# victorca25/traiNNer

Hardware: AMD Instinct MI355X
Metric: HR images/sec (G+D step), ESRGAN x4 128->512 (higher is better)
Workload: dtype f32 (bf16x3)

## Files before the change

### include/trainner_hip.h

```cpp
#ifndef TRAINNER_HIP_H
#define TRAINNER_HIP_H

#include <stdint.h>

#ifdef __cplusplus
extern "C" {
#endif

#define TNR_OK 0
#define TNR_EINVAL (-1)
#define TNR_ELAUNCH (-2)

enum { TNR_ACT_NONE = 0, TNR_ACT_LRELU = 1, TNR_ACT_RELU = 2 };

enum {
    TNR_CONV_3x3 = 0,
    TNR_CONV_3x3_UP2 = 1,
    TNR_CONV_4x4_S2 = 2,
    TNR_DGRAD_4x4_S2 = 3,
    TNR_CONV_1x1 = 4,
    TNR_CONV_3x3_C4 = 5,
    TNR_CONV_7x7_C4 = 6
};

// ... 36 lines not shown
    tnr_view m;  int32_t m_lo, m_hi; float m_slope;
    float *ws; int64_t ws_bytes;
    int32_t mma;
    int32_t pad_mode;
    float noise_sigma; int32_t noise_pos; uint32_t noise_key0, noise_key1, noise_pix0;
    const void *wq; int64_t wq_bytes;
    int32_t wq_form;
    int32_t shuffle;
} tnr_conv_desc;

typedef struct tnr_wgrad_desc {
    tnr_view x; int32_t N, H, W; int32_t Cin;
    tnr_view g; int32_t Ho, Wo; int32_t Cout;
    int32_t mode;
    float *dw; int32_t cin_total, cin_begin;
    float *db;
    float alpha, beta;
    float *ws; int64_t ws_bytes;
    int32_t mma;
    int32_t pad_mode;
    float *dw2; int32_t cout_split, cin_total2;
    float *db2;
} tnr_wgrad_desc;

typedef struct tnr_pack_item {
    const float *w;
    float *wp;
    int32_t Cout, Cin, kh, kw;
    int32_t kind;
    int32_t KoutP, KinP;
    int64_t n_out;
} tnr_pack_item;

typedef struct tnr_dense_pack_item {
    const float *w[5];
    float *wp;
    int32_t nf, gc;
    int32_t t;
    int32_t KoutP, KinP;
    float scale5;
    int64_t n_out;
} tnr_dense_pack_item;

const char *tnr_last_error(void);
#define TNR_ABI_VERSION 3
int tnr_version(void);

int tnr_pack_dims(int32_t Cout, int32_t Cin, int32_t kh, int32_t kw, int32_t kind,
                  int32_t *KoutP, int32_t *KinP, int64_t *n_out);
int tnr_pack_weights(const tnr_pack_item *items_dev, int32_t n, int64_t max_out, void *stream);
int tnr_pack_dense_dims(int32_t nf, int32_t gc, int32_t t, int32_t *KoutP, int32_t *KinP, int64_t *n_out);
int tnr_pack_dense_dgrad(const tnr_dense_pack_item *items_dev, int32_t n, int64_t max_out, void *stream);
int tnr_conv_forward(const tnr_conv_desc *d, void *stream);
int tnr_gauss_mult(tnr_view dst, tnr_view src, int64_t pixels, int32_t C, float sigma, uint32_t key0, uint32_t key1, uint32_t pix0,
                   void *stream);
int64_t tnr_conv_workspace_bytes(const tnr_conv_desc *d);
int64_t tnr_conv_wq_bytes(const tnr_conv_desc *d);
int tnr_conv_wq_pack(const tnr_conv_desc *d, void *image, int64_t image_bytes, void *stream);
int64_t tnr_conv_wino_bytes(const tnr_conv_desc *d);
int tnr_conv_wino_pack(const tnr_conv_desc *d, void *image, int64_t image_bytes, void *stream);
int tnr_im2col(tnr_view x, int32_t N, int32_t H, int32_t W, int32_t C, int32_t k, int32_t stride, int32_t pad,
               int32_t Ho, int32_t Wo, float *out, void *stream);
#define TNR_CHAIN_MAX 6
int64_t tnr_conv_chain_workspace_bytes(const tnr_conv_desc *stage0);
int tnr_conv_chain(const tnr_conv_desc *stages, const int32_t *fresh_from, int32_t n, uint32_t *ws, int64_t ws_bytes,
                   uint32_t epoch, void *stream);
int64_t tnr_conv_sweep_image_bytes(const tnr_conv_desc *stages, int32_t n);
int tnr_conv_sweep_pack(const tnr_conv_desc *stages, int32_t n, void *image, int64_t image_bytes, void *stream);
typedef struct tnr_sweep_pack_item { int32_t units; int32_t reserved; uint64_t opaque[15]; } tnr_sweep_pack_item;
int tnr_conv_sweep_pack_item(const tnr_conv_desc *stages, int32_t n, void *image, int64_t image_bytes, tnr_sweep_pack_item *item);
int tnr_conv_sweep_pack_batch(const tnr_sweep_pack_item *items_dev, int32_t n, int32_t max_units, void *stream);
int tnr_conv_sweep(const tnr_conv_desc *stages, int32_t n, const void *image, uint32_t *ws, int64_t ws_bytes, uint32_t epoch,
                   void *stream);
int64_t tnr_conv_thin_pack_floats(int32_t reduce_channels);
int tnr_conv_thin_pack(const float *w_oihw, float *wp, int32_t Cout, int32_t Cin, int32_t dgrad, void *stream);
int tnr_conv_thin(tnr_view x, int32_t N, int32_t H, int32_t W, int32_t Cin, const float *wp, tnr_view y, int32_t Cout,
                  const float *bias, float alpha, void *stream);
int64_t tnr_conv_thin7_pack_floats(int32_t reduce_channels);
int tnr_conv_thin7_pack(const float *w_oihw, float *wp, int32_t Cout, int32_t Cin, int32_t dgrad, void *stream);
int tnr_conv_thin7(tnr_view x, int32_t N, int32_t H, int32_t W, int32_t Cin, const float *wp, tnr_view y, int32_t Ho, int32_t Wo,
                   int32_t Cout, int32_t pad, int32_t reflect, const float *bias, float alpha, void *stream);
int64_t tnr_wgrad_workspace_bytes(const tnr_wgrad_desc *d);
int64_t tnr_wgrad_thin_workspace_bytes(int32_t N, int32_t H, int32_t Cbig);
int tnr_wgrad_thin(tnr_view big, tnr_view small, int32_t N, int32_t H, int32_t W, int32_t Cbig, int32_t Csmall, int32_t flip,
                   float *dw, float *db, float alpha, float beta, float *ws, int64_t ws_bytes, void *stream);
int64_t tnr_wgrad_thin7_workspace_bytes(int32_t N, int32_t Hbig_grid, int32_t Cbig);
int tnr_wgrad_thin7(tnr_view big, int32_t N, int32_t H, int32_t W, int32_t rpad, tnr_view small, int32_t Hs, int32_t Ws, int32_t off,
                    int32_t Cbig, int32_t Csmall, int32_t flip, float *dw, float *db, float alpha, float beta, float *ws, int64_t ws_bytes,
                    void *stream);
int tnr_conv_wgrad(const tnr_wgrad_desc *d, void *stream);
#define TNR_WGRAD_GROUP_MAX 12
int tnr_conv_wgrad_group(const tnr_wgrad_desc *descs, int32_t n, void *stream);
int tnr_wgrad_tile_class(const tnr_wgrad_desc *d, int32_t group_jobs, int32_t x3_occ, int32_t out[12]);

int tnr_gconv_fwd(tnr_view x, int32_t N, int32_t H, int32_t W, int32_t Cin, const float *w, const float *bias, tnr_view y, int32_t Ho,
                  int32_t Wo, int32_t Cout, int32_t k, int32_t stride, int32_t pad, int32_t reflect, int32_t act, float slope, void *stream);
int tnr_gconv_dgrad(tnr_view g, int32_t N, int32_t H, int32_t W, int32_t Cin, const float *w, tnr_view gx, int32_t Ho, int32_t Wo,
                    int32_t Cout, int32_t k, int32_t stride, int32_t pad, int32_t reflect, void *stream);
int64_t tnr_gconv_wgrad_workspace_bytes(int32_t Cout, int32_t Cin, int32_t k);
int tnr_gconv_wgrad(tnr_view x, int32_t N, int32_t H, int32_t W, int32_t Cin, tnr_view g, int32_t Ho, int32_t Wo, int32_t Cout, int32_t k,
                    int32_t stride, int32_t pad, int32_t reflect, float *dw, float *db, float alpha, float beta, double *ws,
                    int64_t ws_bytes, void *stream);
int tnr_bias_grad(tnr_view g, int64_t pixels, int32_t C, float *db, float alpha, float beta, double *ws, int64_t ws_bytes, void *stream);
int tnr_pad2d(tnr_view x, tnr_view y, int32_t N, int32_t H, int32_t W, int32_t C, int32_t pad, int32_t mode, void *stream);
int tnr_unpad2d(tnr_view xp, tnr_view y, int32_t N, int32_t H, int32_t W, int32_t C, int32_t pad, int32_t mode, void *stream);
int tnr_window2d(tnr_view src, int32_t Hs, int32_t Ws, tnr_view dst, int32_t N, int32_t Hd, int32_t Wd, int32_t C, int32_t oy,
// ... 19 lines not shown
                          float *dst, int32_t bgr2rgb, float data_range, int32_t normalize, void *stream);
int tnr_tensor2np_u8(const float *src, int32_t N, int32_t C, int32_t H, int32_t W, uint8_t *dst, int32_t rgb2bgr,
                     int32_t denormalize, void *stream);
int64_t tnr_metrics_workspace_bytes(int32_t N);
int tnr_psnr_ssim_u8(const uint8_t *a, const uint8_t *b, int32_t N, int32_t H, int32_t W, int32_t C, int32_t crop,
                     int32_t want_ssim, double *out, double *ws, int64_t ws_bytes, void *stream);
int tnr_lpips_stem_dims(int32_t H, int32_t W, int32_t crop, int32_t *Ho, int32_t *Wo);
int tnr_lpips_stem(const void *a, const void *b, int32_t src_kind, int32_t N, int32_t H, int32_t W, int32_t C, int32_t crop,
                   int32_t normalize, const float *shift, const float *scale, const float *w, const float *bias, tnr_view y,
                   void *stream);
int tnr_maxpool3s2_ceil_dims(int32_t H, int32_t W, int32_t *Ho, int32_t *Wo);
int tnr_maxpool3s2_ceil_fwd(tnr_view x, tnr_view y, int32_t N, int32_t H, int32_t W, int32_t C, void *stream);
int64_t tnr_lpips_workspace_bytes(int32_t N, int32_t L);
int tnr_lpips_head(tnr_view f0, tnr_view f1, int32_t N, int32_t H, int32_t W, int32_t C, const float *w, int32_t layer, int32_t L,
                   double *ws, int64_t ws_bytes, void *stream);
int tnr_lpips_finalize(int32_t N, int32_t L, const double *ws, int64_t ws_bytes, double *out, double *per_layer, void *stream);
int tnr_bilinear2x_fwd(tnr_view x, tnr_view y, int32_t N, int32_t H, int32_t W, int32_t C, void *stream);
int tnr_bilinear2x_bwd(tnr_view gy, tnr_view gx, tnr_view gz, tnr_view mask, float mslope, int32_t N, int32_t H, int32_t W,
                       int32_t C, void *stream);
int tnr_add2(tnr_view dst, tnr_view a, tnr_view b, int64_t pixels, int32_t C, void *stream);
int tnr_mask_copy(tnr_view dst, tnr_view src, tnr_view y, int64_t pixels, int32_t C, float mslope, void *stream);
int tnr_nchw_to_nhwc(const float *src, int32_t N, int32_t C, int32_t H, int32_t W, tnr_view dst,
                     int32_t Cpad, const float *scale, const float *shift, void *stream);
int tnr_nhwc_to_nchw(tnr_view src, int32_t N, int32_t C, int32_t H, int32_t W, float *dst,
                     const float *scale, int32_t accumulate, void *stream);
int tnr_upsample2x_bwd(tnr_view gup, tnr_view gx, int32_t N, int32_t H, int32_t W, int32_t C,
                       tnr_view mask, float mslope, void *stream);
int tnr_depth_to_space(tnr_view x, tnr_view y, int32_t N, int32_t H, int32_t W, int32_t Cout, void *stream);
int tnr_space_to_depth_bwd(tnr_view gy, tnr_view gx, int32_t N, int32_t H, int32_t W, int32_t Cout,
                           tnr_view mask, float mslope, void *stream);
int tnr_maxpool2_fwd(tnr_view x, tnr_view y, int32_t N, int32_t H, int32_t W, int32_t C, void *stream);
int tnr_maxpool2_bwd(tnr_view gy, tnr_view x, tnr_view gx, int32_t N, int32_t H, int32_t W, int32_t C,
                     void *stream);
int tnr_axpby(tnr_view dst, tnr_view src, int64_t pixels, int32_t C, float a, float b, void *stream);
int tnr_mask_mul(tnr_view g, tnr_view y, int64_t pixels, int32_t C, float mslope, void *stream);
int tnr_fill(float *p, int64_t n, float v, void *stream);

int64_t tnr_bn_workspace_bytes(int32_t C);
int tnr_bn_train_fwd(tnr_view z, tnr_view y, int64_t pixels, int32_t C, const float *gamma,
                     const float *beta, float *running_mean, float *running_var, int64_t *num_batches,
                     float momentum, float eps, float *save_mean, float *save_invstd, int32_t act,
                     float slope, void *ws, void *stream);
int tnr_bn_train_fwd_stats(tnr_view z, tnr_view y, int64_t pixels, int32_t C, const float *gamma, const float *beta,
                           float *running_mean, float *running_var, int64_t *num_batches, float momentum, float eps,
                           float *save_mean, float *save_invstd, double *stat64, int32_t act, float slope, void *ws, void *stream);
int tnr_bn_replay_running(float *running_mean, float *running_var, int64_t *num_batches, const double *stat64, int32_t C,
                          float momentum, void *stream);
int tnr_bn_train_bwd(tnr_view gy, tnr_view y, tnr_view z, tnr_view gz, int64_t pixels, int32_t C,
                     const float *gamma, const float *save_mean, const float *save_invstd, float mslope,
                     float *dgamma, float *dbeta, float acc_beta, void *ws, void *stream);
int tnr_bn_train_bwd_z(tnr_view gy, tnr_view z, tnr_view gz, int64_t pixels, int32_t C, const float *gamma, const float *beta,
                       const float *save_mean, const float *save_invstd, float mslope, float *dgamma, float *dbeta,
                       float acc_beta, void *ws, void *stream);
int64_t tnr_instnorm_workspace_bytes(int32_t N, int32_t C);
int tnr_instnorm_fwd(tnr_view z, tnr_view y, int32_t N, int64_t pixels_per_image, int32_t C, float eps, float *save_mean,
                     float *save_invstd, int32_t act, float slope, void *ws, void *stream);
int tnr_instnorm_bwd(tnr_view gy, tnr_view y, tnr_view z, tnr_view gz, int32_t N, int64_t pixels_per_image, int32_t C,
                     const float *save_mean, const float *save_invstd, float mslope, void *ws, void *stream);

int tnr_linear_fwd(const float *x, const float *w, const float *b, float *y, int32_t N, int32_t In,
                   int32_t Out, int32_t act, float slope, void *stream);
int tnr_linear_bwd(const float *x, const float *w, const float *gy, const float *yact, float mslope,
                   float *gx, float *dw, float *db, int32_t N, int32_t In, int32_t Out, float acc_beta,
                   float *gpre_ws, void *stream);

int64_t tnr_reduce_workspace_bytes(void);
int tnr_l1_mean_fwd(const float *a, const float *b, int64_t n, float scale, float *loss, void *ws,
                    void *stream);
int tnr_l1_mean_bwd(const float *a, const float *b, int64_t n, float scale, const float *gscale,
                    float *ga, int32_t accumulate, void *stream);
int tnr_ragan_phase_a(const float *pf, const float *pr, int32_t n, float *sums, void *ws, void *stream);
int tnr_ragan_phase_b(const float *pf, const float *pr, int32_t n, int32_t stage, float *sums, void *ws, void *stream);
int tnr_ragan_phase_c(const float *pf, const float *pr, int32_t n, int32_t stage, float weight,
                      const float *sums, float *loss_out, float *gf, float *gr, void *stream);
int tnr_scale_by(float *dst, const float *src, int64_t n, const float *gscale, void *stream);

int64_t tnr_ssim_workspace_bytes(int32_t N, int32_t C, int32_t H, int32_t W, int32_t shave, int32_t K);
int tnr_ssim_fwd(const float *x, const float *y, int32_t N, int32_t C, int32_t H, int32_t W, int32_t layout, int32_t shave,
                 const float *taps, int32_t K, float C1, float C2, double *sums, void *ws, int64_t ws_bytes, void *stream);
int tnr_ssim_bwd(const float *x, const float *y, int32_t N, int32_t C, int32_t H, int32_t W, int32_t layout, int32_t shave,
                 const float *taps, int32_t K, float C1, float C2, const float *coef, const float *gscale, float *gx,
                 int32_t accumulate, void *stream);
int tnr_avgpool2_pad_dims(int32_t H, int32_t W, int32_t shave, int32_t *Ho, int32_t *Wo);
int tnr_avgpool2_pad_fwd(const float *x, const float *y, int32_t N, int32_t C, int32_t H, int32_t W, int32_t layout, int32_t shave,
                         float *xo, float *yo, void *stream);
int tnr_avgpool2_pad_bwd(const float *gcoarse, float *gfine, int32_t N, int32_t C, int32_t H, int32_t W, int32_t layout,
                         int32_t shave, void *stream);
int tnr_msssim_combine(const double *sums, int32_t levels, int32_t N, const int64_t *counts, const float *weights, int32_t mode,
                       float *value, float *coef, void *stream);

enum { TNR_CRIT_L1 = 0, TNR_CRIT_L2 = 1, TNR_CRIT_CB = 2, TNR_CRIT_ELASTIC = 3, TNR_CRIT_CLIPL1 = 4 };
int64_t tnr_imgloss_workspace_bytes(int32_t N, int32_t C, int32_t H, int32_t W);
int tnr_filter_loss_fwd(const float *x, const float *y, int32_t N, int32_t C, int32_t H, int32_t W, int32_t layout, const float *taps,
                        int32_t K, int32_t crit, double scale, float *loss, float *dmap, void *ws, int64_t ws_bytes, void *stream);
int tnr_filter_loss_bwd(const float *dmap, int32_t N, int32_t C, int32_t H, int32_t W, int32_t layout, const float *taps, int32_t K,
                        double scale, const float *gscale, float *gx, int32_t accumulate, void *stream);
int tnr_fd_loss_fwd(const float *x, const float *y, int32_t N, int32_t C, int32_t H, int32_t W, int32_t layout, int32_t dirs,
                    int32_t crit, double scale, float *loss, void *ws, int64_t ws_bytes, void *stream);
int tnr_fd_loss_bwd(const float *x, const float *y, int32_t N, int32_t C, int32_t H, int32_t W, int32_t layout, int32_t dirs,
                    int32_t crit, double scale, const float *gscale, float *gx, int32_t accumulate, void *stream);
int tnr_pointwise_loss_fwd(const float *a, const float *b, int64_t n, int32_t crit, double scale, float *loss, void *ws, void *stream);
int tnr_pointwise_loss_bwd(const float *a, const float *b, int64_t n, int32_t crit, double scale, const float *gscale, float *ga,
                           int32_t accumulate, void *stream);

int tnr_overflow_loss_fwd(const float *x, int64_t n, double scale, float *loss, void *ws, void *stream);
int tnr_overflow_loss_bwd(const float *x, int64_t n, double scale, const float *gscale, float *gx, int32_t accumulate, void *stream);
// ... 63 lines not shown
```

### trainner_amd/csrc/conv_epilogue.h

```cpp
#pragma once
#include "conv_body.h"

namespace {

template <int MODE, int TW, int NT, int MT, bool COH, int DEPTH = 1, bool NOISE = true, int BIAS_STEP = 1, class PixFn>
__device__ __forceinline__ void conv_epilogue_dpp_map(const ConvK a, f32x16 (&acc)[MT][NT], const int cb, const int n, const int ty0,
                                                      const int tx0, const int par, const int li, const int half,
                                                      const __amdgpu_buffer_rsrc_t y_rs, PixFn &&pixfn) {
    constexpr bool DG2 = (MODE == TNR_DGRAD_4x4_S2);
    constexpr int NC = NT * 32;
    const int py = par >> 1, px = par & 1;
    TNR_STAMP(2);
#ifdef TNR_PRIO_EPI
    __builtin_amdgcn_s_setprio(TNR_PRIO_EPI);
#endif
    const int qa = li >> 2, qb = li & 3;
    const bool b0 = (qb & 1) != 0, b1 = (qb & 2) != 0;
    auto quad_transpose = [&](float &v0, float &v1, float &v2, float &v3) {
        auto xchg = [&](float &x, float &y, bool sel, int which) {
            const float send = sel ? x : y;
            const int r_ = which == 1 ? __builtin_amdgcn_mov_dpp(__builtin_bit_cast(int, send), 0xB1, 0xF, 0xF, true)
                                      : __builtin_amdgcn_mov_dpp(__builtin_bit_cast(int, send), 0x4E, 0xF, 0xF, true);
            const float recv = __builtin_bit_cast(float, r_);
            x = sel ? recv : x;
            y = sel ? y : recv;
        };
        xchg(v0, v1, b0, 1);
        xchg(v2, v3, b0, 1);
        xchg(v0, v2, b1, 2);
        xchg(v1, v3, b1, 2);
    };
    TNR_STAMP(5);
    TNR_STAMP(6);
    TNR_STAMP(7);
#ifdef TNR_ABL_NOMASK
    const bool has_r1 = a.r1 != nullptr, has_r2 = a.r2 != nullptr, has_m = false;
#else
    const bool has_r1 = a.r1 != nullptr, has_r2 = a.r2 != nullptr, has_m = a.m != nullptr;
#endif
    const bool has_noise = NOISE && a.noise_pos != 0;
    const bool all_full = (a.Cout & 3) == 0;
    const float ns = a.act == TNR_ACT_LRELU ? a.slope : (a.act == TNR_ACT_RELU ? 0.f : 1.f);
    int co_n[NT];
    bool co_ok[NT];
    f32x4 bv[NT];
    float b1f[NT], msf[NT];
    bool use_r1[NT], use_m[NT];
#pragma unroll
    for (int nn = 0; nn < NT; ++nn) {
        const int co = cb * NC + nn * 32 + qa * 4;
        co_n[nn] = co;
        co_ok[nn] = co < a.Cout;
        bv[nn] = f32x4{0.f, 0.f, 0.f, 0.f};
        if (a.bias != nullptr && co_ok[nn]) {
            if constexpr (BIAS_STEP != 1) {
#pragma unroll
                for (int k = 0; k < 4; ++k)
                    if (co + k < a.Cout) bv[nn][k] = a.bias[(co + k) * BIAS_STEP];
            } else if (co + 4 <= a.Cout) {
                bv[nn] = *reinterpret_cast<const f32x4 *>(a.bias + co);
            } else {
#pragma unroll
                for (int k = 0; k < 4; ++k)
                    if (co + k < a.Cout) bv[nn][k] = a.bias[co + k];
            }
        }
        use_r1[nn] = has_r1 && co < a.r1_ch;
        use_m[nn] = has_m && co >= a.m_lo && co < a.m_hi;
        b1f[nn] = use_r1[nn] ? a.beta1 : 0.f;
        msf[nn] = use_m[nn] ? a.m_slope : 1.f;
    }
    constexpr int UNITS = MT * 4;
    constexpr int AHEAD = DEPTH < UNITS ? DEPTH : UNITS, SETS = AHEAD + 1 < UNITS ? AHEAD + 1 : UNITS;
    bool ok[SETS];
    size_t pixi[SETS];
    f32x4 q1[SETS][NT], q2[SETS][NT], qm[SETS][NT];
    auto prep = [&](int u, int set) {
        const int mi = u >> 2, q = u & 3;
        int rr, cc;
        pixfn(mi, 8 * q + 4 * half + qb, rr, cc);
        const int sy = ty0 + rr, sx = tx0 + cc;
        ok[set] = sy < a.th_space && sx < a.tw_space;
        const int oy = DG2 ? 2 * sy + py : sy;
        const int ox = DG2 ? 2 * sx + px : sx;
        const size_t pix = ((size_t)n * a.Ho + oy) * a.Wo + ox;
        pixi[set] = pix;
        const f32x4 zero = {0.f, 0.f, 0.f, 0.f}, one = {1.f, 1.f, 1.f, 1.f};
#pragma unroll
        for (int nn = 0; nn < NT; ++nn) {
            const bool okc = ok[set] && co_ok[nn];
            if (has_r1) {
                q1[set][nn] = zero;
                if (okc && use_r1[nn]) q1[set][nn] = *reinterpret_cast<const f32x4 *>(a.r1 + pix * a.r1_ct + a.r1_co + co_n[nn]);
            }
            if (has_r2) {
                q2[set][nn] = zero;
                if (okc) q2[set][nn] = *reinterpret_cast<const f32x4 *>(a.r2 + pix * a.r2_ct + a.r2_co + co_n[nn]);
            }
            if (has_m) {
                qm[set][nn] = one;
                if (okc && use_m[nn]) qm[set][nn] = *reinterpret_cast<const f32x4 *>(a.m + pix * a.m_ct + a.m_co + co_n[nn]);
            }
        }
    };
    auto finish = [&](int u, int set) {
        const int mi = u >> 2, q = u & 3;
#pragma unroll
        for (int nn = 0; nn < NT; ++nn) {
            float v0 = acc[mi][nn][4 * q + 0], v1 = acc[mi][nn][4 * q + 1], v2 = acc[mi][nn][4 * q + 2], v3 = acc[mi][nn][4 * q + 3];
            quad_transpose(v0, v1, v2, v3);
            f32x4 v = f32x4{v0, v1, v2, v3} + bv[nn];
#pragma unroll
            for (int e = 0; e < 4; ++e) v[e] = __builtin_fmaf(ns, __builtin_fminf(v[e], 0.f), __builtin_fmaxf(v[e], 0.f)) * a.alpha;
            if (has_r1) v += b1f[nn] * q1[set][nn];
            if (has_noise) {
                const f32x4 nm = tnr_gauss_mult4(((unsigned)pixi[set] + a.noise_pix0) * (unsigned)(a.Cout >> 2) + (unsigned)(co_n[nn] >> 2),
                                                 a.noise_k0, a.noise_k1, a.noise_sigma);
                if (a.noise_pos == 1) v *= nm;
                if (has_r2) v = v * a.alpha2 + q2[set][nn];
                if (a.noise_pos != 1) v *= nm;
            } else if (has_r2) {
                v = v * a.alpha2 + q2[set][nn];
            }
            if (has_m) {
#pragma unroll
                for (int e = 0; e < 4; ++e) v[e] *= (qm[set][nn][e] > 0.f ? 1.f : msf[nn]);
            }
            if (!(ok[set] && co_ok[nn])) continue;
            const int co = co_n[nn];
#ifdef TNR_ABL_NOEPISTORE
            if (v[0] == 1.2345e30f) a.y[0] = v[1] + v[2] + v[3];
            continue;
#endif
            if (COH) {
                __builtin_amdgcn_raw_buffer_store_b128(__builtin_bit_cast(tnr_u32x4, v), y_rs,
                                                       (int)((unsigned)(pixi[set] * a.y_ct + a.y_co + co) * 4u), 0, TNR_COH_STORE_AUX);
            } else {
                float *yp = a.y + pixi[set] * a.y_ct + a.y_co + co;
                if (all_full) {
                    *reinterpret_cast<f32x4 *>(yp) = v;
                } else {
#pragma unroll
                    for (int e = 0; e < 4; ++e)
                        if (co + e < a.Cout) yp[e] = v[e];
                }
            }
        }
    };
#pragma unroll
    for (int u = 0; u < AHEAD; ++u) prep(u, u % SETS);
#pragma unroll
    for (int u = 0; u < UNITS; ++u) {
        if (u + AHEAD < UNITS) prep(u + AHEAD, (u + AHEAD) % SETS);
        finish(u, u % SETS);
    }
}

template <int MODE, int TW, int NT, int MT, bool COH, int DEPTH = 1, bool NOISE = true, int BIAS_STEP = 1>
__device__ __forceinline__ void conv_epilogue_dpp(const ConvK a, f32x16 (&acc)[MT][NT], const int cb, const int n, const int ty0,
                                                  const int tx0, const int par, const int wave, const int li, const int half,
                                                  const __amdgpu_buffer_rsrc_t y_rs) {
    conv_epilogue_dpp_map<MODE, TW, NT, MT, COH, DEPTH, NOISE, BIAS_STEP>(a, acc, cb, n, ty0, tx0, par, li, half, y_rs,
                                                                [&](int mi, int row, int &rr, int &cc) __attribute__((always_inline)) {
                                                                    const int p = (wave * MT + mi) * 32 + row;
                                                                    rr = p / TW;
                                                                    cc = p - rr * TW;
                                                                });
}

}
```

### trainner_amd/csrc/conv_sweep.hip

```cpp
#include <stddef.h>
#include <string.h>
#include <type_traits>
#include <utility>
#include "conv_body.h"
#include "conv_epilogue.h"
#include "conv_handoff.h"

namespace {

constexpr int SW_TH = 8, SW_TW = 32, SW_HT = SW_TH + 2, SW_WT = SW_TW + 2;
constexpr int SW_ROW = TNR_X3_ROW;
constexpr int SW_A_ROWS = SW_HT * SW_WT;
constexpr int SW_A_ALLOC_ROWS = 384;
constexpr int SW_A_FLOATS = SW_A_ALLOC_ROWS * SW_ROW;
constexpr int SW_UNIT_FLOATS = 32 * SW_ROW;
constexpr int SW_SLOT_UNITS = 9;
constexpr int SW_SLOT_FLOATS = SW_SLOT_UNITS * SW_UNIT_FLOATS;
constexpr int SW_RING = 3;
constexpr size_t SW_LDS_BYTES = (size_t)(2 * SW_A_FLOATS + SW_RING * SW_SLOT_FLOATS) * sizeof(float);
constexpr int SW_NPASS = 9, SW_NSTAGE = 5, SW_NTILE = 6;
constexpr int SW_A_IT = (SW_A_ROWS * 4 + 511) / 512;
constexpr int SW_B_PIECES = (SW_SLOT_UNITS * 3 + 7) / 8;
static_assert(SW_LDS_BYTES <= 160 * 1024, "one sweep workgroup per CU");

// ... 1012 lines not shown
                sw_static_for<0, 5>([&](auto kc) __attribute__((always_inline)) { item_step_buf(ic, kc, 0); });
            });
        }
        bool has_next = false;
        int e = 0;
        auto item_step = [&](auto ic, auto kc) __attribute__((always_inline)) {
            if (has_next) item_step_buf(ic, kc, (e + 1) & 1);
        };
        auto nop1 = [&](auto) __attribute__((always_inline)) {};
        auto nop0 = [&]() __attribute__((always_inline)) {};
        auto tick = [&](int, unsigned long long) __attribute__((always_inline)) {};
#pragma unroll 1
        for (int ck = 0; ck < c.nck; ++ck) {
            asm volatile("s_waitcnt lgkmcnt(0)\n\ts_barrier" ::: "memory");
            has_next = ck + 1 < c.nck;
            a_load(16 * (ck + 1), has_next);
            if constexpr (AMP) {
                auto item1 = [&](auto ic) __attribute__((always_inline)) {
                    if (has_next) a_item1(ic, (e + 1) & 1);
                };
                amp4_chunk<0, 2>(acc, s_a + (e & 1) * SW_A_FLOATS, apix0, half, item1, fbq, b_fetch1);
            } else {
                sweep4_chunk<0, 2, true>(acc, s_a + (e & 1) * SW_A_FLOATS, nullptr, apix0, half, nop1, item_step, nop0, tick, fbr, b_fetch);
            }
            ++e;
        }
        f32x16 t[2][2];
#pragma unroll
        for (int m = 0; m < 2; ++m) {
            t[m][0] = acc[m][0];
            t[m][1] = acc[m][1];
        }
        if constexpr (PS) {
            ConvK ap = a;
            const int nfb = c.ncb >> 2, sub = cb / nfb;
            ap.Cout = a.Cout >> 2;
            ap.Ho = 2 * a.Ho;
            ap.Wo = 2 * a.Wo;
            ap.bias = a.bias != nullptr ? a.bias + sub : nullptr;
            conv_epilogue_dpp<TNR_DGRAD_4x4_S2, SW_TW, 2, 2, false, (OCC == 1 ? 8 : 1), false, 4>(ap, t, cb - sub * nfb, n, ty0, tx0, sub, wave, li, half, y_rs);
        } else {
            conv_epilogue_dpp<TNR_CONV_3x3, SW_TW, 2, 2, false, (OCC == 1 ? 8 : 1)>(a, t, cb, n, ty0, tx0, 0, wave, li, half, y_rs);
        }
    }
}

constexpr int S2_TAPS = 4, S2_NU = S2_TAPS * 2, S2_RING = 4;
struct S2K {
    ConvK a;
    const float *wq;
    int wq_bytes;
    int nck;
    int tiles_x, tiles_y, ncb, tiles;
};
struct S2PackK {
    const float *wp;
    int KinP, KoutP, nck, ncb, units, dgrad;
    float *out;
};

__global__ void __launch_bounds__(256) s2_pack_kernel(const S2PackK a) {
    const int g = blockIdx.x * 256 + threadIdx.x;
    const int unit = g >> 6, r = (g >> 1) & 31, h = g & 1;
    if (unit >= a.units) return;
    const int j = unit & 1, tap = (unit >> 1) & 3;
    int rest = unit >> 3;
    const float *src;
    if (a.dgrad) {
        const int ck = rest % a.nck;
        rest /= a.nck;
        const int cb = rest % a.ncb, par = rest / a.ncb;
        src = a.wp + (((size_t)par * 4 + tap) * a.KoutP + cb * 64 + j * 32 + r) * a.KinP + 16 * ck + 8 * h;
    } else {
        const int ck = rest % a.nck;
        rest /= a.nck;
        const int pp = rest & 3, cb = rest >> 2;
        src = a.wp + ((size_t)tap * a.KoutP + cb * 64 + j * 32 + r) * (4 * a.KinP) + pp * a.KinP + 16 * ck + 8 * h;
    }
    const f32x4 q0 = *reinterpret_cast<const f32x4 *>(src), q1 = *reinterpret_cast<const f32x4 *>(src + 4);
    tnr_bf16x8 pl[3];
    tnr_split_bf16x3(q0, q1, pl);
    float *dst = a.out + (size_t)unit * SW_UNIT_FLOATS + (h * 32 + r) * 4;
#pragma unroll
    for (int k = 0; k < 3; ++k) *reinterpret_cast<tnr_bf16x8 *>(dst + k * 256) = pl[k];
}

template <bool AMP, class Item, class BFetch>
__device__ __forceinline__ void tap4_chunk(f32x16 (&acc)[2][2], const float *sa, const int (&aaddr)[2][4], Item &&item_step,
                                           tnr_bf16x8 (&fbr)[S2_RING][3], BFetch &&b_fetch) {
    constexpr int TA[6] = {0, 2, 1, 0, 1, 0}, TB[6] = {2, 0, 1, 1, 0, 0};
    tnr_bf16x8 fa[2][2][3];
    auto read_a = [&](auto tc, int m, int sp) __attribute__((always_inline)) {
        constexpr int t = decltype(tc)::value;
        fa[t & 1][m][sp] = *reinterpret_cast<const tnr_bf16x8 *>(sa + aaddr[m][t] + 8 * sp);
    };
#pragma unroll
    for (int k = 0; k < (AMP ? 2 : 6); ++k) read_a(std::integral_constant<int, 0>{}, AMP ? k : k / 3, AMP ? 0 : k % 3);
    sw_static_for<0, S2_NU>([&](auto uc) __attribute__((always_inline)) {
        constexpr int u = decltype(uc)::value, t = u >> 1, jj = u & 1;
        constexpr bool NEXT_TAP = jj == 1 && t + 1 < S2_TAPS;
        constexpr int ITEM = u - (S2_NU - 6);
        __builtin_amdgcn_sched_barrier(0);
        if constexpr (AMP) {
            sw_static_for<0, 2>([&](auto mc) __attribute__((always_inline)) {
                constexpr int m = decltype(mc)::value;
                acc[m][jj] = __builtin_amdgcn_mfma_f32_32x32x16_bf16(fa[t & 1][m][0], fbr[u % S2_RING][0], acc[m][jj], 0, 0, 0);
                if constexpr (m == 0) b_fetch(std::integral_constant<int, (u + 3) % S2_RING>{}, 0);
                if constexpr (NEXT_TAP) read_a(std::integral_constant<int, (t + 1 < S2_TAPS ? t + 1 : t)>{}, m, 0);
                if constexpr (m == 1 && ITEM >= 0) item_step(std::integral_constant<int, (ITEM >= 0 ? ITEM : 0)>{}, std::integral_constant<int, -1>{});
                __builtin_amdgcn_sched_barrier(0);
            });
        } else {
            sw_static_for<0, 12>([&](auto ic) __attribute__((always_inline)) {
                constexpr int i = decltype(ic)::value, p = i / 2, m = i % 2;
                acc[m][jj] = __builtin_amdgcn_mfma_f32_32x32x16_bf16(fa[t & 1][m][TA[p]], fbr[u % S2_RING][TB[p]], acc[m][jj], 0, 0, 0);
                if constexpr (i < 3) b_fetch(std::integral_constant<int, (u + 3) % S2_RING>{}, i);
                if constexpr (NEXT_TAP && i >= 3 && i < 9) read_a(std::integral_constant<int, (t + 1 < S2_TAPS ? t + 1 : t)>{}, (i - 3) / 3, (i - 3) % 3);
                if constexpr (ITEM >= 0 && i >= 4 && i < 9) item_step(std::integral_constant<int, (ITEM >= 0 ? ITEM : 0)>{}, std::integral_constant<int, (i >= 4 && i < 9 ? i - 4 : 0)>{});
                __builtin_amdgcn_sched_barrier(0);
            });
        }
    });
}

template <int MODE, bool AMP>
__global__ void __launch_bounds__(256, 2) conv_s2_d4_kernel(const S2K c) {
    constexpr bool DG = MODE == TNR_DGRAD_4x4_S2;
    constexpr int HT = DG ? SW_HT : SW_TH + 1, WT = DG ? SW_WT : SW_TW + 1, ROWS = HT * WT;
    constexpr int A_IT = (ROWS * 4 + 255) / 256;
    static_assert(A_IT <= 6 && A_IT * 256 <= SW_A_ALLOC_ROWS * 4, "staging plan");
    extern __shared__ __attribute__((aligned(16))) float smem[];
    float *s_a = smem;
    const int tid = threadIdx.x;
    const int wave = __builtin_amdgcn_readfirstlane(tid >> 6), lane = tid & 63, li = lane & 31, half = lane >> 5;
    const ConvK &a = c.a;
    const __amdgpu_buffer_rsrc_t x_rs =
        __builtin_amdgcn_make_buffer_rsrc(const_cast<float *>(a.x), 0, (int)((unsigned)a.N * a.H * a.W * a.x_ct * 4u), 0x00020000);
    const __amdgpu_buffer_rsrc_t w_rs = __builtin_amdgcn_make_buffer_rsrc(const_cast<float *>(c.wq), 0, c.wq_bytes, 0x00020000);
    const __amdgpu_buffer_rsrc_t y_rs =
        __builtin_amdgcn_make_buffer_rsrc(a.y, 0, (int)((unsigned)a.N * a.Ho * a.Wo * a.y_ct * 4u), 0x00020000);
    const int nchunks = DG ? c.nck : 4 * c.nck;

    for (int tile = blockIdx.x; tile < c.tiles; tile += gridDim.x) {
        int rest = tile;
        const int cb = rest % c.ncb;
        rest /= c.ncb;
        int par = 0;
        if constexpr (DG) {
            par = rest & 3;
            rest >>= 2;
        }
        const int tx = rest % c.tiles_x;
        rest /= c.tiles_x;
        const int ty = rest % c.tiles_y, n = rest / c.tiles_y;
        const int ty0 = ty * SW_TH, tx0 = tx * SW_TW;
        const int py = par >> 1, px = par & 1;
        int aaddr[2][4];
#pragma unroll
        for (int m = 0; m < 2; ++m)
#pragma unroll
            for (int t = 0; t < 4; ++t) {
                const int pos_y = DG ? 1 + py - (t >> 1) : (t >> 1), pos_x = DG ? 1 + px - (t & 1) : (t & 1);
                const int pp = (2 * wave + m + pos_y) * WT + li + pos_x;
                aaddr[m][t] = pp * SW_ROW + 4 * (half ^ ((pp >> TNR_X3_SWZ) & 1));
            }
        int in_off[A_IT], a_dst[A_IT];
        auto plan = [&](int pp) __attribute__((always_inline)) {
#pragma unroll
            for (int it = 0; it < A_IT; ++it) {
                const int i = tid + it * 256, row = i >> 2, q = i & 3;
                const int hr = row / WT, hc = row - hr * WT;
                const int Y = DG ? ty0 + hr - 1 : 2 * (ty0 + hr) - 1 + (pp >> 1), X = DG ? tx0 + hc - 1 : 2 * (tx0 + hc) - 1 + (pp & 1);
                const bool in = (row < ROWS) & (Y >= 0) & (Y < a.H) & (X >= 0) & (X < a.W);
                in_off[it] = in ? (((n * a.H + Y) * a.W + X) * a.x_ct + a.x_co + q * 4) : -1;
                a_dst[it] = row * SW_ROW + 4 * ((q >> 1) ^ ((row >> TNR_X3_SWZ) & 1)) + 2 * (q & 1);
            }
        };
        plan(0);
        f32x4 rin[A_IT];
// ... 33 lines not shown
        for (int m = 0; m < 2; ++m)
#pragma unroll
            for (int j = 0; j < 2; ++j)
#pragma unroll
                for (int r = 0; r < 16; ++r) acc[m][j][r] = 0.f;

        a_load(0, true);
        __syncthreads();
        tnr_bf16x8 fbr[S2_RING][3];
        int bq = (DG ? (par * c.ncb + cb) * c.nck : cb * 4 * c.nck) * S2_NU;
        auto b_fetch = [&](auto rc, int sp) __attribute__((always_inline)) {
            constexpr int r = decltype(rc)::value;
            if constexpr (AMP) {
                fbr[r][0] = __builtin_bit_cast(tnr_bf16x8, __builtin_amdgcn_raw_buffer_load_b128(w_rs, lane * 16, bq * 3072, 0));
                ++bq;
            } else {
                fbr[r][sp] = __builtin_bit_cast(tnr_bf16x8, __builtin_amdgcn_raw_buffer_load_b128(w_rs, lane * 16, (bq * 3 + sp) * 1024, 0));
                if (sp == 2) ++bq;
            }
        };
        sw_static_for<0, 3>([&](auto rc) __attribute__((always_inline)) {
#pragma unroll
            for (int sp = 0; sp < (AMP ? 1 : 3); ++sp) b_fetch(rc, sp);
        });
        sw_static_for<0, 6>([&](auto ic) __attribute__((always_inline)) {
            if constexpr (AMP) item_step_buf(ic, std::integral_constant<int, -1>{}, 0);
            else sw_static_for<0, 5>([&](auto kc) __attribute__((always_inline)) { item_step_buf(ic, kc, 0); });
        });
        bool has_next = false;
        int e = 0;
        auto item_step = [&](auto ic, auto kc) __attribute__((always_inline)) {
            if (has_next) item_step_buf(ic, kc, (e + 1) & 1);
        };
#pragma unroll 1
        for (int ck = 0; ck < nchunks; ++ck) {
            asm volatile("s_waitcnt lgkmcnt(0)\n\ts_barrier" ::: "memory");
            has_next = ck + 1 < nchunks;
            int ch_next = 16 * (ck + 1);
            if constexpr (!DG) {
                const int nx = ck + 1, ppn = nx / c.nck;
                ch_next = 16 * (nx - ppn * c.nck);
                if (has_next && ppn != ck / c.nck) plan(ppn);
            }
            a_load(ch_next, has_next);
            tap4_chunk<AMP>(acc, s_a + (e & 1) * SW_A_FLOATS, aaddr, item_step, fbr, b_fetch);
            ++e;
        }
        f32x16 t2[2][2];
#pragma unroll
        for (int m = 0; m < 2; ++m) {
            t2[m][0] = acc[m][0];
            t2[m][1] = acc[m][1];
        }
        conv_epilogue_dpp<MODE, SW_TW, 2, 2, false, 1>(a, t2, cb, n, ty0, tx0, par, wave, li, half, y_rs);
    }
}

bool s2_ok(const tnr_conv_desc *d) {
    if (d->mode != TNR_CONV_4x4_S2 && d->mode != TNR_DGRAD_4x4_S2) return false;
    const bool dg = d->mode == TNR_DGRAD_4x4_S2;
    const int tw = dg ? d->W : d->Wo, th = dg ? d->H : d->Ho;
    return (d->mma == TNR_MMA_BF16X3 || d->mma == TNR_MMA_BF16) && d->pad_mode == 0 && d->shuffle == 0 && (d->Cout % 64) == 0 && d->KoutP == d->Cout &&
           d->Cin == d->KinP && (d->Cin % 16) == 0 && d->Cin >= 32 && tw >= 32 && th >= 8 &&
           (dg ? (d->Ho == 2 * d->H && d->Wo == 2 * d->W) : (d->H == 2 * d->Ho && d->W == 2 * d->Wo)) &&
           buffers_addressable(*d) &&
           (int64_t)(d->Cout / 64) * (d->Cin / 16) * 4 * S2_NU * SW_UNIT_FLOATS * (int64_t)sizeof(float) < (1LL << 31);
}

bool d4_ok(const tnr_conv_desc *d) {
    if (d->shuffle != 0 && !(d->shuffle == 2 && (d->Cout % 256) == 0 && d->r1.ptr == nullptr && d->r2.ptr == nullptr && d->m.ptr == nullptr &&
                             d->noise_pos == 0 && d->pad_mode == 0 && (d->y.ctot % 4) == 0 &&
                             (int64_t)d->N * d->H * d->W * 4 * d->y.ctot < (1LL << 30)))
        return false;
    return d->mode == TNR_CONV_3x3 && (d->mma == TNR_MMA_BF16X3 || d->mma == TNR_MMA_BF16) && (d->pad_mode == 0 || (d->pad_mode == 1 && d->H >= 2 && d->W >= 2)) &&
           (d->Cout % 64) == 0 && d->KoutP == d->Cout &&
           d->Cin == d->KinP && (d->Cin % 16) == 0 && d->Cin >= 32 && d->Ho == d->H && d->Wo == d->W && d->W >= 32 && d->H >= 8 &&
           buffers_addressable(*d) &&
           (int64_t)(d->Cout / 64) * (d->Cin / 16) * 18 * SW_UNIT_FLOATS * (int64_t)sizeof(float) < (1LL << 31);
}

bool sweep_pattern(const tnr_conv_desc *st, int n, const char **why) {
    auto no = [&](const char *w) { if (why) *why = w; return false; };
    if (st == nullptr || (n != SW_NSTAGE && n != SW4_NSTAGE)) return no("not 5 (or 4) stages");
    if (n == SW4_NSTAGE && st[0].mma != TNR_MMA_BF16X3) return no("the four-stage form exists in bf16x3 only");
    const tnr_conv_desc &d0 = st[0];
    if (d0.Cin < 32 || (d0.Cin % 16) != 0) return no("block input channels must be a multiple of 16, >= 32");
    for (int i = 0; i < n; ++i) {
        const tnr_conv_desc &d = st[i];
        if (d.mode != TNR_CONV_3x3 || (d.mma != TNR_MMA_BF16X3 && d.mma != TNR_MMA_BF16) || d.mma != d0.mma || d.pad_mode != 0)
            return no("stage is not a zero-padded 3x3 in bf16x3 (or all stages with bf16 operands)");
        if (d.N != d0.N || d.H != d0.H || d.W != d0.W || d.Ho != d0.H || d.Wo != d0.W) return no("pixel grids differ");
        if (d.x.ptr != d0.x.ptr || d.x.ctot != d0.x.ctot || d.x.coff != d0.x.coff) return no("stages read different buffers");
        if (d.Cin != d0.Cin + 32 * i || d.KinP != d.Cin) return no("input channels do not grow by 32 per stage");
        if (d.Cout != (i < 4 ? 32 : 64) || d.KoutP != d.Cout) return no("output channels are not 32, 32, 32, 32, 64");
        if (i < 4 && (d.y.ptr != d0.x.ptr || d.y.ctot != d0.x.ctot || d.y.coff != d0.x.coff + d.Cin)) return no("stage output is not the next channel group");
        if (!views_aligned(d)) return no("x / y / r1 / r2 / mask views must be 4-channel aligned");
        if (d.noise_pos < 0 || d.noise_pos > 2 || (i < 4 && d.noise_pos != 0)) return no("the noise multiplier belongs to the last stage");
        if (!buffers_addressable(d)) return no("buffer above 4 GiB");
        if (!d.x.ptr || !d.y.ptr || !d.wp) return no("null pointer");
    }
    const tnr_conv_desc &dl = st[n - 1];
    if (n == SW_NSTAGE && dl.y.ptr == d0.x.ptr && dl.y.coff < d0.x.coff + dl.Cin && dl.y.coff + dl.Cout > d0.x.coff) return no("last stage overwrites its own input");
    return true;
}

int sweep_form() {
    static const int form = [] {
// ... 116 lines not shown
    c.wq_bytes = sw_total_units(c.nck0, n) * SW_UNIT_FLOATS * (int)sizeof(float);
    for (int i = 0; i < SW_NSTAGE; ++i) {
        const tnr_conv_desc *d = &stages[i < n ? i : n - 1];
        ConvK &k = c.st[i] = conv_k_from_desc(*d);
        k.tiles_x = c.tiles_x; k.tiles_y = c.tiles_y; k.ncb = d->KoutP / 32;
    }
    const int per_round = (cus / c.tpi) * c.tpi;
    const int grid = c.tiles < per_round ? c.tiles : per_round;
    const int form = sweep_form();
    if (n == SW4_NSTAGE) {
        TNR_REQUIRE(form == 5, "conv_sweep: four stages run in the direct four-wave form only");
        hipLaunchKernelGGL((conv_sweep4_kernel<true, false, SwPlan4>), dim3((unsigned)grid), dim3(256), S4D_LDS_BYTES, (hipStream_t)stream, c);
        return tnr_check_launch("conv_sweep");
    }
    if (stages[0].mma == TNR_MMA_BF16) {
        TNR_REQUIRE(form == 5, "conv_sweep: bf16 operands (use_amp) run in the direct four-wave form only");
        hipLaunchKernelGGL((conv_sweep4_kernel<true, true>), dim3((unsigned)grid), dim3(256), S4D_LDS_BYTES, (hipStream_t)stream, c);
        return tnr_check_launch("conv_sweep");
    }
    if (form == 8) hipLaunchKernelGGL(conv_sweep_kernel, dim3((unsigned)grid), dim3(512), SW_LDS_BYTES, (hipStream_t)stream, c);
    else if (form == 4) hipLaunchKernelGGL(conv_sweep4_kernel<false>, dim3((unsigned)grid), dim3(256), SW_LDS_BYTES, (hipStream_t)stream, c);
    else hipLaunchKernelGGL(conv_sweep4_kernel<true>, dim3((unsigned)grid), dim3(256), S4D_LDS_BYTES, (hipStream_t)stream, c);
    return tnr_check_launch("conv_sweep");
}

extern "C" int64_t tnr_conv_wq_bytes(const tnr_conv_desc *d) {
    if (d != nullptr && s2_ok(d)) return (int64_t)(d->Cout / 64) * (d->Cin / 16) * 4 * S2_NU * SW_UNIT_FLOATS * (int64_t)sizeof(float);
    if (d == nullptr || !d4_ok(d)) return 0;
    return (int64_t)(d->Cout / 64) * (d->Cin / 16) * 18 * SW_UNIT_FLOATS * (int64_t)sizeof(float);
}

extern "C" int tnr_conv_wq_pack(const tnr_conv_desc *d, void *image, int64_t image_bytes, void *stream) {
    if (d != nullptr && image != nullptr && d->wp != nullptr && s2_ok(d)) {
        S2PackK a;
        a.wp = d->wp; a.KinP = d->KinP; a.KoutP = d->KoutP; a.nck = d->Cin / 16; a.ncb = d->Cout / 64;
        a.dgrad = d->mode == TNR_DGRAD_4x4_S2;
        a.units = a.ncb * 4 * a.nck * S2_NU;
        TNR_REQUIRE((int64_t)a.units * SW_UNIT_FLOATS * (int64_t)sizeof(float) <= image_bytes, "conv_wq_pack: image buffer too small");
        a.out = static_cast<float *>(image);
        hipLaunchKernelGGL(s2_pack_kernel, dim3((unsigned)tnr_cdiv(a.units * 64, 256)), dim3(256), 0, (hipStream_t)stream, a);
        return tnr_check_launch("conv_wq_pack (four-tap form)");
    }
    TNR_REQUIRE(d != nullptr && image != nullptr && d->wp != nullptr && d4_ok(d), "conv_wq_pack: the launch cannot use a pre-split weight stream");
    D4PackK a;
    a.wp = d->wp; a.KinP = d->KinP; a.KoutP = d->KoutP; a.nck = d->Cin / 16; a.ncb = d->Cout / 64;
    a.units = a.ncb * a.nck * 18;
    a.shuffle = d->shuffle;
    TNR_REQUIRE((int64_t)a.units * SW_UNIT_FLOATS * (int64_t)sizeof(float) <= image_bytes, "conv_wq_pack: image buffer too small");
    a.out = static_cast<float *>(image);
    hipLaunchKernelGGL(d4_pack_kernel, dim3((unsigned)tnr_cdiv(a.units * 64, 256)), dim3(256), 0, (hipStream_t)stream, a);
    return tnr_check_launch("conv_wq_pack");
}

int tnr_launch_conv_s2_d4(const tnr_conv_desc *d, void *stream) {
    if (!s2_ok(d) || d->wq == nullptr || d->wq_bytes < tnr_conv_wq_bytes(d) || d->noise_pos != 0) return 1;
    static int cus = 0;
    if (const int rc = tnr_kernel_setup(&cus, "conv_s2_d4", {{conv_s2_d4_kernel<TNR_CONV_4x4_S2, false>, S4D_LDS_BYTES}, {conv_s2_d4_kernel<TNR_CONV_4x4_S2, true>, S4D_LDS_BYTES},
                                                             {conv_s2_d4_kernel<TNR_DGRAD_4x4_S2, false>, S4D_LDS_BYTES}, {conv_s2_d4_kernel<TNR_DGRAD_4x4_S2, true>, S4D_LDS_BYTES}}))
        return rc;
    const bool dg = d->mode == TNR_DGRAD_4x4_S2;
    S2K c;
    if (!stream_k_from_desc(c, *d, tnr_conv_wq_bytes(d), SW_TW, SW_TH, dg ? 4 : 1)) return 1;
    const unsigned grid = (unsigned)(c.tiles < 2 * cus ? c.tiles : 2 * cus);
    const bool amp = d->mma == TNR_MMA_BF16;
    if (dg) {
        if (amp) hipLaunchKernelGGL((conv_s2_d4_kernel<TNR_DGRAD_4x4_S2, true>), dim3(grid), dim3(256), S4D_LDS_BYTES, (hipStream_t)stream, c);
        else hipLaunchKernelGGL((conv_s2_d4_kernel<TNR_DGRAD_4x4_S2, false>), dim3(grid), dim3(256), S4D_LDS_BYTES, (hipStream_t)stream, c);
    } else {
        if (amp) hipLaunchKernelGGL((conv_s2_d4_kernel<TNR_CONV_4x4_S2, true>), dim3(grid), dim3(256), S4D_LDS_BYTES, (hipStream_t)stream, c);
        else hipLaunchKernelGGL((conv_s2_d4_kernel<TNR_CONV_4x4_S2, false>), dim3(grid), dim3(256), S4D_LDS_BYTES, (hipStream_t)stream, c);
    }
    return tnr_check_launch("conv_s2_d4");
}

int tnr_launch_conv3x3_d4(const tnr_conv_desc *d, void *stream) {
    if (!d4_ok(d) || d->wq == nullptr || d->wq_bytes < tnr_conv_wq_bytes(d) || d->noise_pos < 0 || d->noise_pos > 2) return 1;
    static int occ = [] { const char *e = getenv("TNR_D4_OCC"); return e ? atoi(e) : 2; }();
    static int cus = 0;
    if (const int rc = tnr_kernel_setup(&cus, "conv3x3_d4", {{conv3x3_d4_kernel<1>, S4D_LDS_BYTES}, {conv3x3_d4_kernel<2>, S4D_LDS_BYTES}, {conv3x3_d4_kernel<2, true>, S4D_LDS_BYTES},
                                                             {conv3x3_d4_kernel<2, false, true>, S4D_LDS_BYTES}, {conv3x3_d4_kernel<2, true, true>, S4D_LDS_BYTES}}))
        return rc;
    D4K c;
    if (!stream_k_from_desc(c, *d, tnr_conv_wq_bytes(d), SW_TW, SW_TH, 1)) return 1;
    const int slots = cus * (occ == 1 ? 1 : 2);
    const int grid = c.tiles < slots ? c.tiles : slots;
    if (d->shuffle == 2) {
        const unsigned g2 = (unsigned)(c.tiles < 2 * cus ? c.tiles : 2 * cus);
        if (d->mma == TNR_MMA_BF16) hipLaunchKernelGGL((conv3x3_d4_kernel<2, true, true>), dim3(g2), dim3(256), S4D_LDS_BYTES, (hipStream_t)stream, c);
        else hipLaunchKernelGGL((conv3x3_d4_kernel<2, false, true>), dim3(g2), dim3(256), S4D_LDS_BYTES, (hipStream_t)stream, c);
        return tnr_check_launch("conv3x3_d4 (pixel-shuffle store)");
    }
    if (d->mma == TNR_MMA_BF16) hipLaunchKernelGGL((conv3x3_d4_kernel<2, true>), dim3((unsigned)(c.tiles < 2 * cus ? c.tiles : 2 * cus)), dim3(256), S4D_LDS_BYTES, (hipStream_t)stream, c);
    else if (occ == 1) hipLaunchKernelGGL(conv3x3_d4_kernel<1>, dim3((unsigned)grid), dim3(256), S4D_LDS_BYTES, (hipStream_t)stream, c);
    else hipLaunchKernelGGL(conv3x3_d4_kernel<2>, dim3((unsigned)grid), dim3(256), S4D_LDS_BYTES, (hipStream_t)stream, c);
    return tnr_check_launch("conv3x3_d4");
}
```

### trainner_amd/csrc/conv_tile.hip

```cpp
#include "conv_body.h"
#include "conv_x3w8.h"
#include <cstdlib>
#ifdef TNR_CONV_DL_EXPERIMENT
#include "conv_body_dl.h"
#endif

namespace {

template <int MODE, int TW, int NT, int MT, int BF>
__global__ void __launch_bounds__(256, 2) conv_tile_kernel(const ConvK a) {
    TNR_STAMP_CALL(0);
    extern __shared__ __attribute__((aligned(16))) float smem[];
    int bid = blockIdx.x;
    const int split = bid % a.ksplit;
    bid /= a.ksplit;
    const int cb = bid % a.ncb;
    bid /= a.ncb;
    const int tx = bid % a.tiles_x;
    bid /= a.tiles_x;
    const int ty = bid % a.tiles_y;
    bid /= a.tiles_y;
    int par = 0;
    if (MODE == TNR_DGRAD_4x4_S2) {
        par = bid & 3;
// ... 64 lines not shown
    if (tw == 32) return nt == 2 ? launch_conv<MODE, 32, 2>(k, tiles, s) : launch_conv<MODE, 32, 1>(k, tiles, s);
    if (tw == 16) return nt == 2 ? launch_conv<MODE, 16, 2>(k, tiles, s) : launch_conv<MODE, 16, 1>(k, tiles, s);
    return nt == 2 ? launch_conv<MODE, 8, 2>(k, tiles, s) : launch_conv<MODE, 8, 1>(k, tiles, s);
}

int conv_pick_tw(int sw, int sh) {
    int best = 0;
    int64_t best_area = 0;
    for (int tw = 32; tw >= 8; tw >>= 1) {
        if (tw > 8 && sw < tw) continue;
        const int th = 256 / tw;
        const int64_t area = (int64_t)tnr_cdiv(sw, tw) * tw * tnr_cdiv(sh, th) * th;
        if (best == 0 || area < best_area) { best = tw; best_area = area; }
    }
    return best;
}

struct ConvTileGeom {
    int tw, th, nt;
    bool big_m;
    int tiles_x, tiles_y, ncb;
    int64_t tiles;
};
ConvTileGeom conv_tile_geom(const tnr_conv_desc *d) {
    const bool dg = d->mode == TNR_DGRAD_4x4_S2;
    const int sh = dg ? d->H : d->Ho, sw = dg ? d->W : d->Wo;
    ConvTileGeom g;
    g.tw = conv_pick_tw(sw, sh);
    g.nt = d->Cout > 32 ? 2 : 1;
    g.big_m = (d->mode == TNR_CONV_3x3) && g.nt == 1 && g.tw == 32 && sh >= 16;
    g.th = (g.big_m ? 512 : 256) / g.tw;
    g.tiles_x = tnr_cdiv(sw, g.tw);
    g.tiles_y = tnr_cdiv(sh, g.th);
    g.ncb = tnr_cdiv(d->Cout, g.nt * 32);
    g.tiles = (int64_t)g.tiles_x * g.tiles_y * g.ncb * d->N * (dg ? 4 : 1);
    return g;
}

int conv_ksplit(const tnr_conv_desc *d, int64_t tiles) {
    if (d->r1.ptr || d->r2.ptr || d->m.ptr || d->noise_pos || (d->Cout % 4) != 0 || d->mode == TNR_DGRAD_4x4_S2) return 1;
    const int nchunks = (d->KinP / TNR_CK) * (d->mode == TNR_CONV_4x4_S2 ? 4 : 1);
    if (tiles >= 192 || nchunks < 32) return 1;
    int want = (int)((512 + tiles - 1) / tiles);
    const int max_split = nchunks / 8;
    if (want > max_split) want = max_split;
    if (want < 2) return 1;
    const int per = (nchunks + want - 1) / want;
    return (nchunks + per - 1) / per;
}

}

int tnr_launch_conv3x3_d4(const tnr_conv_desc *d, void *stream);
int tnr_launch_conv3x3_wino(const tnr_conv_desc *d, void *stream);
int tnr_launch_conv_s2_d4(const tnr_conv_desc *d, void *stream);

extern "C" int tnr_conv_forward(const tnr_conv_desc *d, void *stream) {
    TNR_REQUIRE(d != nullptr && d->x.ptr && d->y.ptr && d->wp, "conv: null pointer");
    TNR_REQUIRE(d->mode >= TNR_CONV_3x3 && d->mode <= TNR_CONV_7x7_C4, "conv: bad mode %d", d->mode);
    if (d->mode == TNR_CONV_3x3_C4)
        TNR_REQUIRE(d->x.ctot == 4 && d->x.coff == 0 && d->Cin == 4 && d->KinP == 48, "conv3x3_c4: needs an NHWC4 input view and a C4 packing");
    if (d->mode == TNR_CONV_7x7_C4)
        TNR_REQUIRE(d->x.ctot == 4 && d->x.coff == 0 && d->Cin == 4 && d->KinP == 208 && d->wq == nullptr && d->ws == nullptr && d->shuffle == 0,
                    "conv7x7_c4: needs an NHWC4 input view and a 7x7 C4 packing (no weight stream, no split-K)");
    TNR_REQUIRE(views_aligned(*d) && (d->Cin % 4) == 0,
                "conv: x / y / r1 (+ r1_ch) / r2 / mask (+ range) views and Cin must be 4-channel aligned (x: ctot %d coff %d Cin %d)", d->x.ctot, d->x.coff, d->Cin);
    TNR_REQUIRE((d->KinP % TNR_CK) == 0 && (d->KoutP % 32) == 0, "conv: bad packed dims %d %d", d->KinP, d->KoutP);
    TNR_REQUIRE(d->Cin <= d->KinP && d->Cout <= d->KoutP, "conv: Cin/Cout exceed the packing");
    TNR_REQUIRE((int64_t)d->N * d->H * d->W * d->x.ctot < (1LL << 31), "conv: input buffer above 2^31 elements needs 64-bit offsets");
    TNR_REQUIRE(d->Cout % 4 == 0 || (d->r1.ptr == nullptr && d->r2.ptr == nullptr && d->m.ptr == nullptr && d->noise_pos == 0),
                "conv: residual / mask / noise epilogues need Cout %% 4 == 0");
    TNR_REQUIRE(d->noise_pos >= 0 && d->noise_pos <= 2, "conv: bad noise_pos %d", d->noise_pos);
    switch (d->mode) {
        case TNR_CONV_3x3:
        case TNR_CONV_1x1:
        case TNR_CONV_3x3_C4:
        case TNR_CONV_7x7_C4:
            TNR_REQUIRE(d->Ho == d->H && d->Wo == d->W, "conv3x3 / conv1x1 / conv7x7_c4: output must match input size");
            break;
        case TNR_CONV_3x3_UP2:
            TNR_REQUIRE(d->Ho == 2 * d->H && d->Wo == 2 * d->W, "conv3x3_up2: output must be 2x input");
            break;
        case TNR_CONV_4x4_S2:
            TNR_REQUIRE(2 * d->Ho == d->H && 2 * d->Wo == d->W, "conv4x4s2: output must be input/2");
            break;
        default:
            TNR_REQUIRE(d->Ho == 2 * d->H && d->Wo == 2 * d->W, "dgrad4x4s2: output must be 2x gout size");
            break;
    }
    ConvK k = conv_k_from_desc(*d);
    const ConvTileGeom g = conv_tile_geom(d);
    const int tw = g.tw, nt = g.nt, sh = k.th_space;
    const bool big_m = g.big_m;
    k.tiles_x = g.tiles_x; k.tiles_y = g.tiles_y; k.ncb = g.ncb;
    int64_t tiles = g.tiles;
    TNR_REQUIRE(tiles > 0 && tiles < (1LL << 31), "conv: grid too large");
    hipStream_t s = (hipStream_t)stream;
    const int ksplit = conv_ksplit(d, tiles);
    TNR_REQUIRE(d->mma >= TNR_MMA_F32 && d->mma <= TNR_MMA_BF16X3, "conv: bad mma %d", d->mma);
    TNR_REQUIRE(d->pad_mode == 0 || (d->pad_mode == 1 && d->mode == TNR_CONV_3x3 && d->H >= 2 && d->W >= 2) ||
                (d->pad_mode == 1 && d->mode == TNR_CONV_7x7_C4 && d->H >= 4 && d->W >= 4), "conv: pad_mode 1 (reflection) is for TNR_CONV_3x3 and TNR_CONV_7x7_C4");
    SplitRedK red;
    if (ksplit > 1 && d->ws != nullptr) {
        const int64_t plane = (int64_t)d->N * d->Ho * d->Wo * k.KoutP;
        TNR_REQUIRE(plane * ksplit * (int64_t)sizeof(float) <= d->ws_bytes, "conv: split-K workspace too small");
        red.ws = d->ws; red.split_stride = (size_t)plane; red.ksplit = ksplit;
        red.y = k.y; red.y_ct = k.y_ct; red.y_co = k.y_co; red.Cout = k.Cout; red.CoutP = k.KoutP;
        red.pixels = (long long)d->N * d->Ho * d->Wo;
        red.bias = k.bias; red.act = k.act; red.slope = k.slope; red.alpha = k.alpha;
        k.y = d->ws; k.y_ct = k.KoutP; k.y_co = 0; k.Cout = k.KoutP;
        k.bias = nullptr; k.act = TNR_ACT_NONE; k.alpha = 1.f;
        k.ksplit = ksplit; k.split_stride = (size_t)plane;
        tiles *= ksplit;
    }
    int rc;
    if (d->wq != nullptr && d->wq_form == 1) {
        TNR_REQUIRE(k.ksplit == 1, "conv: a Winograd weight stream cannot be combined with a split-K workspace");
        rc = tnr_launch_conv3x3_wino(d, (void *)s);
        TNR_REQUIRE(rc != 1, "conv: wq_form = 1 but the launch does not qualify for the Winograd kernel (tnr_conv_wino_bytes() == 0)");
        return rc;
    }
    if (d->wq != nullptr && k.ksplit == 1) {
        static const bool d4 = [] { const char *e = std::getenv("TNR_X3_D4"); return e == nullptr || e[0] != '0'; }();
        if (d4 || d->shuffle != 0) {
            rc = (d->mode == TNR_CONV_4x4_S2 || d->mode == TNR_DGRAD_4x4_S2) ? tnr_launch_conv_s2_d4(d, (void *)s) : tnr_launch_conv3x3_d4(d, (void *)s);
            if (rc <= 0) return rc;
        }
    }
    TNR_REQUIRE(d->shuffle == 0, "conv: a pixel-shuffle store (shuffle = %d) exists in the weight-stream kernel only (tnr_conv_wq_bytes() == 0 for this launch)", d->shuffle);
    {
        static const bool w8 = [] { const char *e = std::getenv("TNR_X3_W8"); return e == nullptr || e[0] != '0'; }();
        if (w8 && d->mode == TNR_CONV_3x3 && nt == 2 && tw == 32 && sh >= 16 && conv3x3_x3w8_ok(k)) return launch_conv3x3_x3w8(k, s);
    }
#ifdef TNR_CONV_DL_EXPERIMENT
    const char *dl_env = std::getenv("TNR_CONV_DL");
    const int dl = dl_env != nullptr ? dl_env[0] - '0' : 0;
    if (dl == 1 && d->mode == TNR_CONV_3x3 && nt == 2 && tw == 32 && sh >= 16 && conv3x3_dl_ok(k)) return launch_conv3x3_dl<0>(k, s);
    if (dl == 4 && d->mode == TNR_CONV_3x3 && nt == 2 && tw == 32 && sh >= 16 && conv3x3_dl_ok(k)) return launch_conv3x3_dl<2>(k, s);
    if (dl == 5 && d->mode == TNR_CONV_3x3 && nt == 2 && tw == 32 && sh >= 16 && conv3x3_dl_ok(k)) return launch_conv3x3_dl<4>(k, s);
    if (dl == 2 && d->mode == TNR_CONV_3x3 && tw == 32 && conv3x3_dl_ok(k)) {
        if (big_m) return launch_conv3x3_dk8<1, 4>(k, tiles, s);
        if (nt == 2) return launch_conv3x3_dk8<2, 2>(k, tiles, s);
    }
#endif
    if (big_m) {
        rc = launch_conv<TNR_CONV_3x3, 32, 1, 4>(k, (int)tiles, s);
    } else {
        switch (d->mode) {
            case TNR_CONV_3x3: rc = dispatch_conv<TNR_CONV_3x3>(k, tw, nt, (int)tiles, s); break;
            case TNR_CONV_3x3_UP2: rc = dispatch_conv<TNR_CONV_3x3_UP2>(k, tw, nt, (int)tiles, s); break;
            case TNR_CONV_4x4_S2: rc = dispatch_conv<TNR_CONV_4x4_S2>(k, tw, nt, (int)tiles, s); break;
            case TNR_CONV_1x1: rc = dispatch_conv<TNR_CONV_1x1>(k, tw, nt, (int)tiles, s); break;
            case TNR_CONV_3x3_C4: rc = dispatch_conv<TNR_CONV_3x3_C4>(k, tw, nt, (int)tiles, s); break;
            case TNR_CONV_7x7_C4: rc = dispatch_conv<TNR_CONV_7x7_C4>(k, tw, nt, (int)tiles, s); break;
            default: rc = dispatch_conv<TNR_DGRAD_4x4_S2>(k, tw, nt, (int)tiles, s); break;
        }
    }
    if (rc != TNR_OK || k.ksplit == 1) return rc;
    const long long work = red.pixels * (red.CoutP >> 2);
    long long blocks = (work + 255) / 256;
    if (blocks > 4096) blocks = 4096;
    hipLaunchKernelGGL(conv_splitk_reduce_kernel, dim3((unsigned)blocks), dim3(256), 0, s, red);
    return tnr_check_launch("conv_splitk_reduce");
}

extern "C" int64_t tnr_conv_workspace_bytes(const tnr_conv_desc *d) {
    if (d == nullptr) return 0;
    const int ks = conv_ksplit(d, conv_tile_geom(d).tiles);
    return ks > 1 ? (int64_t)ks * d->N * d->Ho * d->Wo * tnr_round_up(d->Cout, 32) * (int64_t)sizeof(float) : 0;
}
```

### trainner_amd/csrc/conv_wino.hip

```cpp
#include <stddef.h>
#include <stdlib.h>
#include <type_traits>
#include <utility>
#include "conv_body.h"
#include "conv_epilogue.h"

namespace {

constexpr int WN_T = 16;
constexpr int WN_PT = WN_T / 2;
constexpr int WN_NP = WN_PT * WN_PT;
constexpr int WN_RAW_W = WN_T + 2;
constexpr int WN_RAW_PIX = WN_RAW_W * WN_RAW_W;
constexpr int WN_RAW_STRIDE = 24;
constexpr int WN_RAW_FLOATS = WN_RAW_PIX * WN_RAW_STRIDE;
constexpr int WN_ROW = TNR_X3_ROW;
constexpr int WN_VH_ROWS = 8 * WN_NP;
constexpr int WN_VH_FLOATS = WN_VH_ROWS * WN_ROW;
constexpr size_t WN_LDS_BYTES = (size_t)(2 * WN_VH_FLOATS + 2 * WN_RAW_FLOATS) * sizeof(float);
constexpr int WN_UNIT_FLOATS = 32 * WN_ROW;
constexpr int WN_STAGE_ITEMS = WN_RAW_PIX * 4;
constexpr int WN_STAGE_IT = (WN_STAGE_ITEMS / 2 + 255) / 256;
static_assert(WN_LDS_BYTES <= 160 * 1024, "one Winograd workgroup per CU");
static_assert(8 * 4 * 16 * 64 * sizeof(float) <= WN_LDS_BYTES, "the inverse transform's exchange fits the LDS");
static_assert(WN_STAGE_IT * 256 * 2 >= WN_STAGE_ITEMS, "staging plan covers the patch");

#ifndef WN_PRIO
#define WN_PRIO 3
#endif
#ifdef WN_TIMELINE
__device__ unsigned long long wn_tl[2][16];
#define WN_T(v) const unsigned long long v = __builtin_amdgcn_s_memtime()
#define WN_ADD(i, d) do { if (lane == 0 && (wave & 3) == 0) tl[i] += (d); } while (0)
#else
#define WN_T(v) do { } while (0)
#define WN_ADD(i, d) do { } while (0)
#endif

struct WinoK {
    ConvK a;
    const float *wq;
    int wq_bytes;
    int nck;
    int tiles_x, tiles_y, ncb, tiles;
};

struct WinoPackK {
    const float *wp;
    int KinP, KoutP, nck, ncb, units;
    float *out;
};

__global__ void __launch_bounds__(256) wino_pack_kernel(const WinoPackK a) {
    const int g = blockIdx.x * 256 + threadIdx.x;
    const int unit = g >> 6, r = (g >> 1) & 31, oh = g & 1;
    if (unit >= a.units) return;
    const int j = unit & 3;
    int rest = unit >> 2;
    const int ck = rest % a.nck;
    rest /= a.nck;
    const int i = rest & 3, nt = (rest >> 2) & 1, cb = rest >> 3;
    const int co = cb * 64 + nt * 32 + r;
    const double G[4][3] = {{1.0, 0.0, 0.0}, {0.5, 0.5, 0.5}, {0.5, -0.5, 0.5}, {0.0, 0.0, 1.0}};
    f32x4 q[2];
#pragma unroll
    for (int e = 0; e < 8; ++e) {
        const int ch = 16 * ck + 8 * oh + e;
        double u = 0.0;
#pragma unroll
        for (int ky = 0; ky < 3; ++ky)
#pragma unroll
            for (int kx = 0; kx < 3; ++kx)
                u += G[i][ky] * G[j][kx] * (double)a.wp[((size_t)(ky * 3 + kx) * a.KoutP + co) * a.KinP + ch];
        q[e >> 2][e & 3] = (float)u;
    }
    tnr_bf16x8 pl[3];
    tnr_split_bf16x3(q[0], q[1], pl);
    float *dst = a.out + (size_t)unit * WN_UNIT_FLOATS + (oh * 32 + r) * 4;
#pragma unroll
    for (int k = 0; k < 3; ++k) *reinterpret_cast<tnr_bf16x8 *>(dst + k * 256) = pl[k];
}

template <int B, class F, int... I>
__device__ __forceinline__ void wn_static_for_seq(F &f, std::integer_sequence<int, I...>) {
    (f(std::integral_constant<int, B + I>{}), ...);
}
template <int B, int E, class F>
__device__ __forceinline__ void wn_static_for(F &&f) {
    wn_static_for_seq<B>(f, std::make_integer_sequence<int, (E > B ? E - B : 0)>{});
}

__global__ void __launch_bounds__(512, 2) conv3x3_wino_kernel(const WinoK c) {
    extern __shared__ __attribute__((aligned(16))) float smem[];
    float *s_v = smem;
    float *s_raw = smem + 2 * WN_VH_FLOATS;
    const int tid = threadIdx.x;
    const int wave = __builtin_amdgcn_readfirstlane(tid >> 6), lane = tid & 63, li = lane & 31, half = lane >> 5;
    const int wil = wave & 1, wn = (wave >> 1) & 1, wh = wave >> 2;
    const int wi = 2 * wh + wil;
    const int tt = tid & 255;
    const ConvK &a = c.a;
    const __amdgpu_buffer_rsrc_t x_rs =
        __builtin_amdgcn_make_buffer_rsrc(const_cast<float *>(a.x), 0, (int)((unsigned)a.N * a.H * a.W * a.x_ct * 4u), 0x00020000);
    const __amdgpu_buffer_rsrc_t w_rs = __builtin_amdgcn_make_buffer_rsrc(const_cast<float *>(c.wq), 0, c.wq_bytes, 0x00020000);
    const __amdgpu_buffer_rsrc_t y_rs =
        __builtin_amdgcn_make_buffer_rsrc(a.y, 0, (int)((unsigned)a.N * a.Ho * a.Wo * a.y_ct * 4u), 0x00020000);
    float *s_vh = s_v + wh * WN_VH_FLOATS;

    const int tp = tt >> 2, tq = tt & 3;
    const int tpy = tp >> 3, tpx = tp & 7;
    const int raw_off = ((2 * tpy + wh) * WN_RAW_W + 2 * tpx) * WN_RAW_STRIDE + 4 * tq;
    static_assert(TNR_X3_SWZ < 4, "the swizzle bit must not depend on the transform position or the M-tile");
    const int v_dst0 = tp * WN_ROW + 4 * ((tq >> 1) ^ ((tp >> TNR_X3_SWZ) & 1)) + 2 * (tq & 1);
    const int a_src0 = (wil * 4 * WN_NP + li) * WN_ROW + 4 * (half ^ ((li >> TNR_X3_SWZ) & 1));
    constexpr int XL_STRIDE = WN_NP * WN_ROW;

#ifdef WN_TIMELINE
    unsigned long long tl[16] = {0, 0, 0, 0, 0, 0, 0, 0, 0, 0, 0, 0, 0, 0, 0, 0};
    const unsigned long long tl_begin = __builtin_amdgcn_s_memtime();
#endif
    for (int tile = blockIdx.x; tile < c.tiles; tile += gridDim.x) {
        const int cb = tile % c.ncb;
        int rest = tile / c.ncb;
        const int tx = rest % c.tiles_x;
        rest /= c.tiles_x;
        const int ty = rest % c.tiles_y, n = rest / c.tiles_y;
        const int ty0 = ty * WN_T, tx0 = tx * WN_T;
        int in_off[WN_STAGE_IT], r_dst[WN_STAGE_IT];
#pragma unroll
        for (int it = 0; it < WN_STAGE_IT; ++it) {
            const int il = tt + it * 256;
            const int i = wh * (WN_STAGE_ITEMS / 2) + il, pix = i >> 2, q = i & 3;
            const int pr = pix / WN_RAW_W, pc = pix - pr * WN_RAW_W;
            int Y = ty0 + pr - 1, X = tx0 + pc - 1;
            if (a.reflect) {
                Y = Y == -1 ? 1 : (Y == a.H ? a.H - 2 : Y);
                X = X == -1 ? 1 : (X == a.W ? a.W - 2 : X);
            }
            const bool mine = il < WN_STAGE_ITEMS / 2;
            const bool in = mine & (Y >= 0) & (Y < a.H) & (X >= 0) & (X < a.W);
            in_off[it] = in ? (((n * a.H + Y) * a.W + X) * a.x_ct + a.x_co + q * 4) : -1;
            r_dst[it] = mine ? pix * WN_RAW_STRIDE + 4 * q : -1;
        }
        f32x4 rin[WN_STAGE_IT];
// ... 200 lines not shown
            WN_T(t1);
            __syncthreads();
            WN_T(t2);
#ifndef WN_X_NOB
            b_fetch(ck, std::integral_constant<int, 2>{});
#endif
#ifndef WN_X_NORAW
            raw_load(16 * (ck + 2), ck + 2 < c.nck);
#endif
#ifndef WN_X_NOM
            multiply();
#endif
            WN_T(t3);
            __syncthreads();
            WN_T(t4);
            WN_ADD(0, t1 - t0); WN_ADD(1, t2 - t1); WN_ADD(2, t3 - t2); WN_ADD(3, t4 - t3); WN_ADD(7, 1ull);
        }
        if (wh == 0) __syncthreads();
        WN_T(t_loop1);
        WN_ADD(4, t_loop1 - t_loop0);

#ifdef WN_X_NOEPI
        if (a.alpha == 1.2345e30f)
#endif
        {
        {
            float *xch = smem + wave * (4 * 16 * 64);
#pragma unroll
            for (int l = 0; l < 2; ++l)
#pragma unroll
                for (int m = 0; m < 2; ++m) {
                    const f32x16 rr = l == 0 ? (acc[0][m] + acc[1][m]) + acc[2][m] : (acc[1][m] - acc[2][m]) - acc[3][m];
#pragma unroll
                    for (int r = 0; r < 16; ++r) xch[((l * 2 + m) * 16 + r) * 64 + lane] = rr[r];
                }
        }
        __syncthreads();
        f32x16 keep[2][1];
        {
            const int k = wil, m = wh;
            auto slot = [&](int ip, int l) __attribute__((always_inline)) {
                return smem + (((ip >> 1) * 4 + wn * 2 + (ip & 1)) * 4 + l * 2 + m) * (16 * 64) + lane;
            };
#pragma unroll
            for (int l = 0; l < 2; ++l) {
                const float *p0 = slot(k, l), *p1 = slot(k + 1, l), *p2 = slot(k + 2, l);
#pragma unroll
                for (int r = 0; r < 16; ++r) {
                    const float x0 = p0[r * 64], x1 = p1[r * 64], x2 = p2[r * 64];
                    keep[l][0][r] = k == 0 ? (x0 + x1) + x2 : (x0 - x1) - x2;
                }
            }
        }
        conv_epilogue_dpp_map<TNR_CONV_3x3, WN_T, 1, 2, false, 1>(a, keep, cb * 2 + wn, n, ty0, tx0, 0, li, half, y_rs,
                                                                  [&](int mi, int row, int &rr, int &cc) __attribute__((always_inline)) {
                                                                      const int p = 32 * wh + row;
                                                                      rr = 2 * (p >> 3) + wil;
                                                                      cc = 2 * (p & 7) + mi;
                                                                  });
        }
    }
#ifdef WN_TIMELINE
    if (lane == 0 && (wave & 3) == 0) {
        tl[5] = __builtin_amdgcn_s_memtime() - tl_begin;
        for (int i = 0; i < 16; ++i) atomicAdd(&wn_tl[wh][i], tl[i]);
    }
#endif
}

constexpr int W16_STAGE_IT = (WN_STAGE_ITEMS / 2 + 511) / 512;

__global__ void __launch_bounds__(1024, 4) conv3x3_wino16_kernel(const WinoK c) {
    extern __shared__ __attribute__((aligned(16))) float smem[];
    float *s_v = smem;
    float *s_raw = smem + 2 * WN_VH_FLOATS;
    const int tid = threadIdx.x;
    const int wave = __builtin_amdgcn_readfirstlane(tid >> 6), lane = tid & 63, li = lane & 31, half = lane >> 5;
    const int wh = (wave >> 2) & 1, role = (wave & 3) | ((wave >> 3) << 2);
    const int wil = role & 1, wn = (role >> 1) & 1, wjp = role >> 2;
    const int wi = 2 * wh + wil;
    const int tt = role * 64 + lane;
    const ConvK &a = c.a;
    const __amdgpu_buffer_rsrc_t x_rs =
        __builtin_amdgcn_make_buffer_rsrc(const_cast<float *>(a.x), 0, (int)((unsigned)a.N * a.H * a.W * a.x_ct * 4u), 0x00020000);
    const __amdgpu_buffer_rsrc_t w_rs = __builtin_amdgcn_make_buffer_rsrc(const_cast<float *>(c.wq), 0, c.wq_bytes, 0x00020000);
    const __amdgpu_buffer_rsrc_t y_rs =
        __builtin_amdgcn_make_buffer_rsrc(a.y, 0, (int)((unsigned)a.N * a.Ho * a.Wo * a.y_ct * 4u), 0x00020000);
    float *s_vh = s_v + wh * WN_VH_FLOATS;

    const int tp = (tt >> 2) & 63, tq = tt & 3, rs = tt >> 8;
    const int tpy = tp >> 3, tpx = tp & 7;
    const int it_ = 2 * wh + rs;
    const int pa = it_ == 0 ? 0 : (it_ == 2 ? 2 : 1), pb = it_ == 0 ? 2 : (it_ == 1 ? 2 : (it_ == 2 ? 1 : 3));
    const bool plus = it_ == 1;
    const int raw_a = ((2 * tpy + pa) * WN_RAW_W + 2 * tpx) * WN_RAW_STRIDE + 4 * tq;
    const int raw_b = ((2 * tpy + pb) * WN_RAW_W + 2 * tpx) * WN_RAW_STRIDE + 4 * tq;
    static_assert(TNR_X3_SWZ < 4, "the swizzle bit must not depend on the transform position or the M-tile");
    const int v_dst0 = (rs * 4 * WN_NP + tp) * WN_ROW + 4 * ((tq >> 1) ^ ((tp >> TNR_X3_SWZ) & 1)) + 2 * (tq & 1);
    const int a_src0 = ((wil * 4 + 2 * wjp) * WN_NP + li) * WN_ROW + 4 * (half ^ ((li >> TNR_X3_SWZ) & 1));
    constexpr int XL_STRIDE = WN_NP * WN_ROW;

    for (int tile = blockIdx.x; tile < c.tiles; tile += gridDim.x) {
        const int cb = tile % c.ncb;
        int rest = tile / c.ncb;
        const int tx = rest % c.tiles_x;
        rest /= c.tiles_x;
        const int ty = rest % c.tiles_y, n = rest / c.tiles_y;
        const int ty0 = ty * WN_T, tx0 = tx * WN_T;
        int in_off[W16_STAGE_IT], r_dst[W16_STAGE_IT];
#pragma unroll
        for (int it = 0; it < W16_STAGE_IT; ++it) {
            const int il = tt + it * 512;
// ... 157 lines not shown
            };
            const float *p0 = slot(k), *p1 = slot(k + 1), *p2 = slot(k + 2);
#pragma unroll
            for (int r = 0; r < 16; ++r) {
                const float x0 = p0[r * 64], x1 = p1[r * 64], x2 = p2[r * 64];
                keep[0][0][r] = k == 0 ? (x0 + x1) + x2 : (x0 - x1) - x2;
            }
        }
        conv_epilogue_dpp_map<TNR_CONV_3x3, WN_T, 1, 1, false, 1>(a, keep, cb * 2 + wn, n, ty0, tx0, 0, li, half, y_rs,
                                                                  [&](int, int row, int &rr, int &cc) __attribute__((always_inline)) {
                                                                      const int p = 32 * wh + row;
                                                                      rr = 2 * (p >> 3) + wil;
                                                                      cc = 2 * (p & 7) + wjp;
                                                                  });
    }
}

bool wino_ok(const tnr_conv_desc *d) {
    return d->mode == TNR_CONV_3x3 && d->mma == TNR_MMA_BF16X3 && (d->pad_mode == 0 || (d->pad_mode == 1 && d->H >= 2 && d->W >= 2)) &&
           (d->Cout % 64) == 0 && d->KoutP == d->Cout && d->Cin == d->KinP && (d->Cin % 16) == 0 && d->Cin >= 32 && d->Ho == d->H &&
           d->Wo == d->W && d->W >= 8 && d->H >= 8 && buffers_addressable(*d) &&
           (int64_t)(d->Cout / 64) * (d->Cin / 16) * 32 * WN_UNIT_FLOATS * (int64_t)sizeof(float) < (1LL << 31);
}

}

#ifdef WN_TIMELINE
extern "C" int tnr_debug_wino_timeline(unsigned long long *out16, int reset) {
    if (out16 != nullptr && hipMemcpyFromSymbol(out16, HIP_SYMBOL(wn_tl), sizeof(wn_tl)) != hipSuccess) return TNR_ELAUNCH;
    if (reset) {
        unsigned long long z[32] = {0};
        if (hipMemcpyToSymbol(HIP_SYMBOL(wn_tl), z, sizeof(z)) != hipSuccess) return TNR_ELAUNCH;
    }
    return TNR_OK;
}
#endif

extern "C" int64_t tnr_conv_wino_bytes(const tnr_conv_desc *d) {
    if (d == nullptr || !wino_ok(d)) return 0;
    return (int64_t)(d->Cout / 64) * (d->Cin / 16) * 32 * WN_UNIT_FLOATS * (int64_t)sizeof(float);
}

extern "C" int tnr_conv_wino_pack(const tnr_conv_desc *d, void *image, int64_t image_bytes, void *stream) {
    TNR_REQUIRE(d != nullptr && image != nullptr && d->wp != nullptr && wino_ok(d), "conv_wino_pack: the launch cannot run in the Winograd form");
    WinoPackK a;
    a.wp = d->wp; a.KinP = d->KinP; a.KoutP = d->KoutP; a.nck = d->Cin / 16; a.ncb = d->Cout / 64;
    a.units = a.ncb * a.nck * 32;
    TNR_REQUIRE((int64_t)a.units * WN_UNIT_FLOATS * (int64_t)sizeof(float) <= image_bytes, "conv_wino_pack: image buffer too small");
    a.out = static_cast<float *>(image);
    hipLaunchKernelGGL(wino_pack_kernel, dim3((unsigned)tnr_cdiv(a.units * 64, 256)), dim3(256), 0, (hipStream_t)stream, a);
    return tnr_check_launch("conv_wino_pack");
}

int tnr_launch_conv3x3_wino(const tnr_conv_desc *d, void *stream) {
    if (!wino_ok(d) || d->wq == nullptr || d->wq_bytes < tnr_conv_wino_bytes(d) || d->noise_pos < 0 || d->noise_pos > 2) return 1;
    static int cus = 0;
    if (const int rc = tnr_kernel_setup(&cus, "conv3x3_wino", {{conv3x3_wino_kernel, WN_LDS_BYTES}, {conv3x3_wino16_kernel, WN_LDS_BYTES}})) return rc;
    WinoK c;
    if (!stream_k_from_desc(c, *d, tnr_conv_wino_bytes(d), WN_T, WN_T, 1)) return 1;
    const int grid = c.tiles < cus ? c.tiles : cus;
    static const bool w16 = [] { const char *e = getenv("TNR_WINO_WAVES"); return e != nullptr && atoi(e) == 16; }();
    if (w16) {
        hipLaunchKernelGGL(conv3x3_wino16_kernel, dim3((unsigned)grid), dim3(1024), WN_LDS_BYTES, (hipStream_t)stream, c);
        return tnr_check_launch("conv3x3_wino16");
    }
    hipLaunchKernelGGL(conv3x3_wino_kernel, dim3((unsigned)grid), dim3(512), WN_LDS_BYTES, (hipStream_t)stream, c);
    return tnr_check_launch("conv3x3_wino");
}
```

### trainner_amd/csrc/norm_loss_optim.hip

```cpp
#include "common.h"

namespace {

constexpr int RED_BLOCKS = 512;

struct BnMaskK { const float *invstd, *gamma, *beta; };
template <int MODE>
__global__ void bn_partial_kernel(const float *z, int z_ct, int z_co, const float *gy, int g_ct, int g_co, const float *y,
                                  int y_ct, int y_co, const float *mean, float mslope, int64_t pixels, int C,
                                  int64_t pix_per_block, double *partial, BnMaskK mk = BnMaskK{nullptr, nullptr, nullptr}) {
    extern __shared__ double sh_d[];
    {
        const size_t go = (size_t)blockIdx.y * (size_t)pixels;
        z += go * z_ct;
        if (MODE >= 1) {
            gy += go * g_ct;
            if (MODE == 1) y += go * y_ct;
            mean += (size_t)blockIdx.y * C;
        }
        partial += (size_t)blockIdx.y * gridDim.x * C * 2;
    }
    const int G = C / 4;
    const int lanes = 256 / G;
    const int tid = threadIdx.x;
// ... 581 lines not shown
}
}

extern "C" int tnr_bn_replay_running(float *running_mean, float *running_var, int64_t *num_batches, const double *stat64, int32_t C,
                                     float momentum, void *stream) {
    TNR_REQUIRE(running_mean && running_var && stat64 && C > 0, "bn_replay_running: bad arguments");
    hipLaunchKernelGGL(bn_replay_kernel, dim3(tnr_cdiv(C, 256)), dim3(256), 0, (hipStream_t)stream, running_mean, running_var, num_batches,
                       stat64, C, momentum);
    return tnr_check_launch("bn_replay_running");
}

extern "C" int tnr_bn_train_bwd(tnr_view gy, tnr_view y, tnr_view z, tnr_view gz, int64_t pixels, int32_t C,
                                const float *gamma, const float *save_mean, const float *save_invstd, float mslope,
                                float *dgamma, float *dbeta, float acc_beta, void *ws, void *stream) {
    TNR_REQUIRE(gy.ptr && y.ptr && z.ptr && gz.ptr && gamma && save_mean && save_invstd && ws, "bn_bwd: null pointer");
    TNR_REQUIRE((C % 4) == 0 && C / 4 <= 256, "bn_bwd: unsupported C %d", C);
    TNR_REQUIRE((dgamma == nullptr) == (dbeta == nullptr), "bn_bwd: dgamma and dbeta go together");
    int nblocks; int64_t ppb; size_t lds;
    bn_plan(pixels, C, nblocks, ppb, lds);
    hipStream_t s = (hipStream_t)stream;
    double *partial = (double *)ws;
    double *sums = partial + (size_t)RED_BLOCKS * C * 2;
    hipLaunchKernelGGL(bn_partial_kernel<1>, dim3(nblocks), dim3(256), lds, s, z.ptr, z.ctot, z.coff, gy.ptr, gy.ctot, gy.coff,
                       y.ptr, y.ctot, y.coff, save_mean, mslope, pixels, C, ppb, partial);
    hipLaunchKernelGGL(bn_bwd_finalize_kernel, dim3(tnr_cdiv(C, 32)), dim3(256), 0, s, partial, nblocks, C, save_invstd, sums,
                       dgamma, dbeta, acc_beta);
    hipLaunchKernelGGL(bn_bwd_apply_kernel<false>, dim3(grid_for(pixels * (C / 4))), dim3(256), 0, s, gy.ptr, gy.ctot, gy.coff, y.ptr,
                       y.ctot, y.coff, z.ptr, z.ctot, z.coff, gz.ptr, gz.ctot, gz.coff, pixels, C, gamma, save_mean,
                       save_invstd, sums, mslope, (const float *)nullptr);
    return tnr_check_launch("bn_train_bwd");
}

extern "C" int tnr_bn_train_bwd_z(tnr_view gy, tnr_view z, tnr_view gz, int64_t pixels, int32_t C, const float *gamma, const float *beta,
                                  const float *save_mean, const float *save_invstd, float mslope, float *dgamma, float *dbeta,
                                  float acc_beta, void *ws, void *stream) {
    TNR_REQUIRE(gy.ptr && z.ptr && gz.ptr && gamma && beta && save_mean && save_invstd && ws, "bn_bwd_z: null pointer");
    TNR_REQUIRE((C % 4) == 0 && C / 4 <= 256, "bn_bwd_z: unsupported C %d", C);
    TNR_REQUIRE((dgamma == nullptr) == (dbeta == nullptr), "bn_bwd_z: dgamma and dbeta go together");
    int nblocks; int64_t ppb; size_t lds;
    bn_plan(pixels, C, nblocks, ppb, lds);
    hipStream_t s = (hipStream_t)stream;
    double *partial = (double *)ws;
    double *sums = partial + (size_t)RED_BLOCKS * C * 2;
    hipLaunchKernelGGL(bn_partial_kernel<2>, dim3(nblocks), dim3(256), lds, s, z.ptr, z.ctot, z.coff, gy.ptr, gy.ctot, gy.coff,
                       (const float *)nullptr, 0, 0, save_mean, mslope, pixels, C, ppb, partial, BnMaskK{save_invstd, gamma, beta});
    hipLaunchKernelGGL(bn_bwd_finalize_kernel, dim3(tnr_cdiv(C, 32)), dim3(256), 0, s, partial, nblocks, C, save_invstd, sums,
                       dgamma, dbeta, acc_beta);
    hipLaunchKernelGGL(bn_bwd_apply_kernel<true>, dim3(grid_for(pixels * (C / 4))), dim3(256), 0, s, gy.ptr, gy.ctot, gy.coff,
                       (const float *)nullptr, 0, 0, z.ptr, z.ctot, z.coff, gz.ptr, gz.ctot, gz.coff, pixels, C, gamma, save_mean,
                       save_invstd, sums, mslope, beta);
    return tnr_check_launch("bn_train_bwd_z");
}

extern "C" int64_t tnr_instnorm_workspace_bytes(int32_t N, int32_t C) {
    return (int64_t)N * ((int64_t)RED_BLOCKS * C * 2 + 2 * (int64_t)C) * (int64_t)sizeof(double);
}

extern "C" int tnr_instnorm_fwd(tnr_view z, tnr_view y, int32_t N, int64_t pixels, int32_t C, float eps, float *save_mean,
                                float *save_invstd, int32_t act, float slope, void *ws, void *stream) {
    TNR_REQUIRE(z.ptr && y.ptr && save_mean && save_invstd && ws && N > 0 && N <= 65535 && pixels > 0, "instnorm_fwd: bad arguments");
    TNR_REQUIRE((C % 4) == 0 && C / 4 <= 256, "instnorm_fwd: unsupported C %d", C);
    int nblocks; int64_t ppb; size_t lds;
    bn_plan(pixels, C, nblocks, ppb, lds);
    hipStream_t s = (hipStream_t)stream;
    double *partial = (double *)ws;
    hipLaunchKernelGGL(bn_partial_kernel<0>, dim3(nblocks, N), dim3(256), lds, s, z.ptr, z.ctot, z.coff, nullptr, 0, 0, nullptr, 0,
                       0, nullptr, 0.f, pixels, C, ppb, partial);
    hipLaunchKernelGGL(bn_fwd_finalize_kernel, dim3(tnr_cdiv(C, 32), N), dim3(256), 0, s, partial, nblocks, C, pixels,
                       nullptr, nullptr, nullptr, 0.f, eps, save_mean, save_invstd, nullptr);
    int64_t gx = tnr_cdiv64(pixels * (C / 4), 256);
    if (gx > 4096) gx = 4096;
    hipLaunchKernelGGL(bn_fwd_apply_kernel, dim3((unsigned)gx, N), dim3(256), 0, s, z.ptr, z.ctot, z.coff, y.ptr,
                       y.ctot, y.coff, pixels, C, nullptr, nullptr, save_mean, save_invstd, act, slope);
    return tnr_check_launch("instnorm_fwd");
}

extern "C" int tnr_instnorm_bwd(tnr_view gy, tnr_view y, tnr_view z, tnr_view gz, int32_t N, int64_t pixels, int32_t C,
                                const float *save_mean, const float *save_invstd, float mslope, void *ws, void *stream) {
    TNR_REQUIRE(gy.ptr && y.ptr && z.ptr && gz.ptr && save_mean && save_invstd && ws && N > 0 && N <= 65535 && pixels > 0,
                "instnorm_bwd: bad arguments");
    TNR_REQUIRE((C % 4) == 0 && C / 4 <= 256, "instnorm_bwd: unsupported C %d", C);
    int nblocks; int64_t ppb; size_t lds;
    bn_plan(pixels, C, nblocks, ppb, lds);
    hipStream_t s = (hipStream_t)stream;
    double *partial = (double *)ws;
    double *sums = partial + (size_t)N * RED_BLOCKS * C * 2;
    hipLaunchKernelGGL(bn_partial_kernel<1>, dim3(nblocks, N), dim3(256), lds, s, z.ptr, z.ctot, z.coff, gy.ptr, gy.ctot, gy.coff,
                       y.ptr, y.ctot, y.coff, save_mean, mslope, pixels, C, ppb, partial);
    hipLaunchKernelGGL(bn_bwd_finalize_kernel, dim3(tnr_cdiv(C, 32), N), dim3(256), 0, s, partial, nblocks, C, save_invstd, sums,
                       nullptr, nullptr, 0.f);
    int64_t gx = tnr_cdiv64(pixels * (C / 4), 256);
    if (gx > 4096) gx = 4096;
    hipLaunchKernelGGL(bn_bwd_apply_kernel<false>, dim3((unsigned)gx, N), dim3(256), 0, s, gy.ptr, gy.ctot, gy.coff, y.ptr,
                       y.ctot, y.coff, z.ptr, z.ctot, z.coff, gz.ptr, gz.ctot, gz.coff, pixels, C, nullptr, save_mean,
                       save_invstd, sums, mslope, (const float *)nullptr);
    return tnr_check_launch("instnorm_bwd");
}

extern "C" int tnr_linear_fwd(const float *x, const float *w, const float *b, float *y, int32_t N, int32_t In, int32_t Out,
                              int32_t act, float slope, void *stream) {
    TNR_REQUIRE(x && w && y && N > 0 && In > 0 && Out > 0, "linear_fwd: bad arguments");
    hipLaunchKernelGGL(linear_fwd_kernel, dim3(N * Out), dim3(256), 0, (hipStream_t)stream, x, w, b, y, N, In, Out, act, slope);
    return tnr_check_launch("linear_fwd");
}

extern "C" int tnr_linear_bwd(const float *x, const float *w, const float *gy, const float *yact, float mslope, float *gx,
// ... 108 lines not shown
```

### trainner_amd/engine.py

```python
import torch

from . import hip, ops
from .flat import FlatParams


class ConvOp:

    def __init__(self, mod, packer, need_dgrad=True, ups=False):
        self.mod, self.packer = mod, packer
        k, s = mod.kernel_size, mod.stride
        if k == 3 and s == 1:
            self.mode_f = ops.CONV_3x3_UP2 if ups else ops.CONV_3x3
            self.mode_d = ops.CONV_3x3
            pf, pd = ops.PACK_FWD, ops.PACK_DGRAD_3x3
        elif k == 4 and s == 2 and not ups:
            self.mode_f, self.mode_d = ops.CONV_4x4_S2, ops.DGRAD_4x4_S2
            pf, pd = ops.PACK_FWD_S2D, ops.PACK_DGRAD_S2
        else:
            raise NotImplementedError("conv k=%d s=%d is not on the SR hot path" % (k, s))
        self.i_f = packer.add(mod.weight, pf)
        self.i_d = packer.add(mod.weight, pd) if need_dgrad else None
        deep = mod.in_channels * k * k >= 2048 and not ups
        i_fc = packer.add(mod.weight, ops.PACK_COL_FWD) if deep else None
        i_dc = packer.add(mod.weight, ops.PACK_COL_DGRAD3) if (deep and need_dgrad and k == 3) else None
        img = k == 3 and s == 1 and not ups
        self.thin = img
        i_f4 = packer.add(mod.weight, ops.PACK_C4_FWD) if (img and mod.in_channels <= 4) else None
        i_d4 = packer.add(mod.weight, ops.PACK_C4_DGRAD3) if (img and need_dgrad and mod.out_channels <= 4) else None
        cin, cout = mod.in_channels, mod.out_channels
        self.dirs = {False: (self.mode_f, ops.ConvLayer(k, s, cin, cout, False, ups, direct=self.i_f, c4=i_f4, col=i_fc)),
                     True: (self.mode_d, ops.ConvLayer(k, s, cin, cout, True, ups, direct=self.i_d, c4=i_d4, col=i_dc))}

    def _run(self, dgrad, x, y, epi):
        mode, layer = self.dirs[dgrad]
        wp = self.packer.get(layer.direct)
        form = ops.conv_plan(x, wp, y, mode, epi, layer=layer)[0]
        if form == "thin":
            ops.conv_thin(x, self.mod.weight, y, bias=None if dgrad else self.mod.bias, alpha=epi.get("alpha", 1.0), dgrad=dgrad)
        elif form == "c4":
            ops.conv(x if x.C == 4 else ops.View(x.buf), self.packer.get(layer.c4), y, mode=ops.CONV_3x3_C4, **epi)
        elif form == "im2col":
            ops.conv_small(x, self.packer.get(layer.col), y, layer.k, layer.stride, **epi)
        else:
            ops.conv(x, wp, y, mode=mode, **epi)

    def fwd(self, x, y, **epi):
        epi["bias"] = self.mod.bias
        self._run(False, x, y, epi)

    def fwd_shuffle2(self, x, y, **epi):
        return ops.conv_shuffle2(x, self.packer.get(self.i_f), y, layer=self.dirs[False][1], bias=self.mod.bias, **epi)

    def dgrad(self, g, gx, **epi):
        self._run(True, g, gx, epi)

    def fwd_stage(self, x, y, fresh_from=None, **epi):
        return dict(x=x, wp=self.packer.get(self.i_f), y=y, mode=self.mode_f, bias=self.mod.bias, fresh_from=fresh_from, **epi)

    def wgrad_item(self, x, g, alpha=1.0, cin_begin=0, with_bias=True, reflect=False):
        w = self.mod.weight
        db = self.mod.bias.grad if (with_bias and self.mod.bias is not None and cin_begin == 0) else None
        return dict(x=x, g=g, dw=w.grad, db=db, cin_begin=cin_begin, alpha=alpha, beta=1.0, reflect=reflect)

    def wgrad(self, x, g, alpha=1.0, cin_begin=0, with_bias=True, reflect=False):
        if reflect:
            ops.wgrad_group([self.wgrad_item(x, g, alpha, cin_begin, with_bias, reflect=True)], mode=self.mode_f)
            return
        if self.thin and ops.IMAGE_C4 and cin_begin == 0 and x.N == g.N and (x.H, x.W) == (g.H, g.W):
            m = self.mod
            db = m.bias.grad if (with_bias and m.bias is not None) else None
            if m.in_channels <= 3 and x.ctot == 4 and x.coff == 0 and g.C in (16, 32, 64):
                ops.wgrad_thin(g, ops.View(x.buf), m.weight.grad, db, flip=False, alpha=alpha)
                return
            if m.out_channels <= 3 and g.ctot == 4 and g.coff == 0 and x.C in (16, 32, 64):
                ops.wgrad_thin(x, ops.View(g.buf), m.weight.grad, db, flip=True, alpha=alpha)
                return
        ops.wgrad_group([self.wgrad_item(x, g, alpha, cin_begin, with_bias)], mode=self.mode_f)


class _NetFn(torch.autograd.Function):

    @staticmethod
    def forward(ctx, net, x, *params):
        need_param_grad = any(ctx.needs_input_grad[2:])
        need_graph = ctx.needs_input_grad[1] or need_param_grad
        memo = net._memo_lookup(x) if (net.memoize and net.training) else None
        if memo is not None and memo[1] is not None:
            out, saved = memo
            net.replay_forward_side_effects(saved)
            out = out.detach()
        else:
            out, saved = net.engine_forward(x, save=need_graph or (net.memoize and net.training))
            if net.memoize and net.training:
                net._memo_store(x, out, saved)
        ctx.net, ctx.saved, ctx.need_param_grad = net, (saved if need_graph else None), need_param_grad
        return out

    @staticmethod
    def backward(ctx, gout):
        saved = ctx.saved
        if saved is None:
            raise RuntimeError("HIP engine: backward through a forward that saved no activations")
        ctx.saved = None
        sched = getattr(ctx.net, "_bucket_schedule", None)
        if sched is not None and ctx.need_param_grad:
            sched.begin_pass()
        gx = ctx.net.engine_backward(saved, gout, need_input_grad=ctx.needs_input_grad[1],
# ... 74 lines not shown
```

### trainner_amd/hip.py

```python
import ctypes as C
import os

import torch

from . import build as _build

c_f = C.c_float
c_i = C.c_int32
c_l = C.c_int64
c_p = C.c_void_p

ACT_NONE, ACT_LRELU, ACT_RELU = 0, 1, 2
MMA_F32, MMA_BF16, MMA_BF16X3 = 0, 1, 2
CONV_3x3, CONV_3x3_UP2, CONV_4x4_S2, DGRAD_4x4_S2, CONV_1x1, CONV_3x3_C4, CONV_7x7_C4 = 0, 1, 2, 3, 4, 5, 6
PACK_FWD, PACK_DGRAD_3x3, PACK_FWD_S2D, PACK_DGRAD_S2, PACK_COL_FWD, PACK_COL_DGRAD3 = 0, 1, 2, 3, 4, 5
PACK_C4_FWD, PACK_C4_DGRAD3 = 6, 7
PACK_DENSE_DGRAD = 16


class CView(C.Structure):
    _fields_ = [("ptr", c_p), ("ctot", c_i), ("coff", c_i)]


class ConvDesc(C.Structure):
    _fields_ = [
        ("x", CView), ("N", c_i), ("H", c_i), ("W", c_i), ("Cin", c_i),
        ("wp", c_p), ("KinP", c_i), ("KoutP", c_i),
        ("y", CView), ("Ho", c_i), ("Wo", c_i), ("Cout", c_i),
        ("mode", c_i), ("bias", c_p), ("act", c_i), ("slope", c_f), ("alpha", c_f),
        ("r1", CView), ("r1_ch", c_i), ("beta1", c_f),
        ("r2", CView), ("alpha2", c_f),
        ("m", CView), ("m_lo", c_i), ("m_hi", c_i), ("m_slope", c_f),
        ("ws", c_p), ("ws_bytes", c_l), ("mma", c_i), ("pad_mode", c_i),
        ("noise_sigma", c_f), ("noise_pos", c_i), ("noise_key0", C.c_uint32), ("noise_key1", C.c_uint32), ("noise_pix0", C.c_uint32),
        ("wq", c_p), ("wq_bytes", c_l), ("wq_form", c_i), ("shuffle", c_i),
    ]


class WgradDesc(C.Structure):
    _fields_ = [
        ("x", CView), ("N", c_i), ("H", c_i), ("W", c_i), ("Cin", c_i),
        ("g", CView), ("Ho", c_i), ("Wo", c_i), ("Cout", c_i),
        ("mode", c_i),
        ("dw", c_p), ("cin_total", c_i), ("cin_begin", c_i),
        ("db", c_p), ("alpha", c_f), ("beta", c_f),
        ("ws", c_p), ("ws_bytes", c_l), ("mma", c_i), ("pad_mode", c_i),
        ("dw2", c_p), ("cout_split", c_i), ("cin_total2", c_i), ("db2", c_p),
    ]


class SweepPackItem(C.Structure):
    _fields_ = [("units", c_i), ("reserved", c_i), ("opaque", C.c_uint64 * 15)]


class PackItem(C.Structure):
    _fields_ = [("w", c_p), ("wp", c_p), ("Cout", c_i), ("Cin", c_i), ("kh", c_i), ("kw", c_i),
                ("kind", c_i), ("KoutP", c_i), ("KinP", c_i), ("n_out", c_l)]


class DensePackItem(C.Structure):
    _fields_ = [("w", c_p * 5), ("wp", c_p), ("nf", c_i), ("gc", c_i), ("t", c_i), ("KoutP", c_i), ("KinP", c_i),
                ("scale5", c_f), ("n_out", c_l)]


_SIGS = {
    "tnr_last_error": (C.c_char_p, []),
    "tnr_version": (c_i, []),
    "tnr_pack_dims": (c_i, [c_i, c_i, c_i, c_i, c_i, C.POINTER(c_i), C.POINTER(c_i), C.POINTER(c_l)]),
    "tnr_pack_weights": (c_i, [c_p, c_i, c_l, c_p]),
    "tnr_pack_dense_dims": (c_i, [c_i, c_i, c_i, C.POINTER(c_i), C.POINTER(c_i), C.POINTER(c_l)]),
    "tnr_pack_dense_dgrad": (c_i, [c_p, c_i, c_l, c_p]),
    "tnr_conv_forward": (c_i, [C.POINTER(ConvDesc), c_p]),
    "tnr_conv_workspace_bytes": (c_l, [C.POINTER(ConvDesc)]),
    "tnr_conv_wq_bytes": (c_l, [C.POINTER(ConvDesc)]),
    "tnr_conv_wq_pack": (c_i, [C.POINTER(ConvDesc), c_p, c_l, c_p]),
    "tnr_conv_wino_bytes": (c_l, [C.POINTER(ConvDesc)]),
    "tnr_conv_wino_pack": (c_i, [C.POINTER(ConvDesc), c_p, c_l, c_p]),
    "tnr_gauss_mult": (c_i, [CView, CView, c_l, c_i, c_f, C.c_uint32, C.c_uint32, C.c_uint32, c_p]),
    "tnr_im2col": (c_i, [CView, c_i, c_i, c_i, c_i, c_i, c_i, c_i, c_i, c_i, c_p, c_p]),
    "tnr_conv_chain_workspace_bytes": (c_l, [C.POINTER(ConvDesc)]),
    "tnr_conv_chain": (c_i, [C.POINTER(ConvDesc), C.POINTER(C.c_int32), c_i, c_p, c_l, C.c_uint32, c_p]),
    "tnr_conv_sweep_image_bytes": (c_l, [C.POINTER(ConvDesc), c_i]),
    "tnr_conv_sweep_pack_item": (c_i, [C.POINTER(ConvDesc), c_i, c_p, c_l, C.POINTER(SweepPackItem)]),
    "tnr_conv_sweep_pack_batch": (c_i, [c_p, c_i, c_i, c_p]),
    "tnr_conv_sweep_pack": (c_i, [C.POINTER(ConvDesc), c_i, c_p, c_l, c_p]),
    "tnr_conv_sweep": (c_i, [C.POINTER(ConvDesc), c_i, c_p, c_p, c_l, C.c_uint32, c_p]),
    "tnr_conv_thin_pack_floats": (c_l, [c_i]),
    "tnr_conv_thin_pack": (c_i, [c_p, c_p, c_i, c_i, c_i, c_p]),
    "tnr_conv_thin": (c_i, [CView, c_i, c_i, c_i, c_i, c_p, CView, c_i, c_p, c_f, c_p]),
    "tnr_wgrad_workspace_bytes": (c_l, [C.POINTER(WgradDesc)]),
    "tnr_conv_thin7_pack_floats": (c_l, [c_i]),
    "tnr_conv_thin7_pack": (c_i, [c_p, c_p, c_i, c_i, c_i, c_p]),
    "tnr_conv_thin7": (c_i, [CView, c_i, c_i, c_i, c_i, c_p, CView, c_i, c_i, c_i, c_i, c_i, c_p, c_f, c_p]),
    "tnr_wgrad_thin7_workspace_bytes": (c_l, [c_i, c_i, c_i]),
    "tnr_wgrad_thin7": (c_i, [CView, c_i, c_i, c_i, c_i, CView, c_i, c_i, c_i, c_i, c_i, c_i, c_p, c_p, c_f, c_f, c_p, c_l, c_p]),
    "tnr_wgrad_thin_workspace_bytes": (c_l, [c_i, c_i, c_i]),
    "tnr_wgrad_thin": (c_i, [CView, CView, c_i, c_i, c_i, c_i, c_i, c_i, c_p, c_p, c_f, c_f, c_p, c_l, c_p]),
    "tnr_conv_wgrad": (c_i, [C.POINTER(WgradDesc), c_p]),
    "tnr_conv_wgrad_group": (c_i, [C.POINTER(WgradDesc), c_i, c_p]),
    "tnr_wgrad_tile_class": (c_i, [C.POINTER(WgradDesc), c_i, c_i, C.POINTER(c_i * 12)]),
    "tnr_nchw_to_nhwc": (c_i, [c_p, c_i, c_i, c_i, c_i, CView, c_i, c_p, c_p, c_p]),
    "tnr_nhwc_to_nchw": (c_i, [CView, c_i, c_i, c_i, c_i, c_p, c_p, c_i, c_p]),
    "tnr_upsample2x_bwd": (c_i, [CView, CView, c_i, c_i, c_i, c_i, CView, c_f, c_p]),
    "tnr_depth_to_space": (c_i, [CView, CView, c_i, c_i, c_i, c_i, c_p]),
    "tnr_space_to_depth_bwd": (c_i, [CView, CView, c_i, c_i, c_i, c_i, CView, c_f, c_p]),
    "tnr_maxpool2_fwd": (c_i, [CView, CView, c_i, c_i, c_i, c_i, c_p]),
    "tnr_maxpool2_bwd": (c_i, [CView, CView, CView, c_i, c_i, c_i, c_i, c_p]),
    "tnr_gconv_fwd": (c_i, [CView, c_i, c_i, c_i, c_i, c_p, c_p, CView, c_i, c_i, c_i, c_i, c_i, c_i, c_i, c_i, c_f, c_p]),
    "tnr_gconv_dgrad": (c_i, [CView, c_i, c_i, c_i, c_i, c_p, CView, c_i, c_i, c_i, c_i, c_i, c_i, c_i, c_p]),
    "tnr_gconv_wgrad_workspace_bytes": (c_l, [c_i, c_i, c_i]),
    "tnr_gconv_wgrad": (c_i, [CView, c_i, c_i, c_i, c_i, CView, c_i, c_i, c_i, c_i, c_i, c_i, c_i, c_p, c_p, c_f, c_f, c_p, c_l, c_p]),
    "tnr_bias_grad": (c_i, [CView, c_l, c_i, c_p, c_f, c_f, c_p, c_l, c_p]),
    "tnr_pad2d": (c_i, [CView, CView, c_i, c_i, c_i, c_i, c_i, c_i, c_p]),
    "tnr_unpad2d": (c_i, [CView, CView, c_i, c_i, c_i, c_i, c_i, c_i, c_p]),
    "tnr_window2d": (c_i, [CView, c_i, c_i, CView, c_i, c_i, c_i, c_i, c_i, c_i, c_i, c_p]),
    "tnr_tanh_fwd": (c_i, [c_p, c_p, c_l, c_p]),
    "tnr_tanh_bwd": (c_i, [c_p, c_p, c_p, c_l, c_p]),
    "tnr_gan_loss": (c_i, [c_p, c_l, c_i, c_f, c_p, c_p, c_p]),
    "tnr_dp_unique_id": (c_i, [c_p]),
    "tnr_dp_init": (c_i, [c_p, c_i, c_i, C.POINTER(c_p)]),
    "tnr_dp_allreduce_bucket": (c_i, [c_p, c_p, c_l, c_i, c_p]),
    "tnr_dp_broadcast": (c_i, [c_p, c_p, c_l, c_i, c_p]),
    "tnr_dp_comm_count": (c_i, [c_p, C.POINTER(c_i)]),
    "tnr_dp_finalize": (c_i, [c_p]),
    "tnr_filter2d": (c_i, [c_p, c_p, c_p, c_i, c_i, c_i, c_i, c_p]),
    "tnr_resize": (c_i, [c_p, c_p, c_i, c_i, c_i, c_i, c_i, c_i, c_p]),
    "tnr_noise_gaussian": (c_i, [c_p, c_i, c_i, c_i, c_i, c_p, c_p, C.c_uint64, c_i, c_p]),
    "tnr_noise_poisson": (c_i, [c_p, c_i, c_i, c_i, c_i, c_p, c_p, c_p, C.c_uint64, c_i, c_p]),
    "tnr_jpeg_workspace_bytes": (c_l, [c_i, c_i, c_i]),
    "tnr_jpeg_sim": (c_i, [c_p, c_i, c_i, c_i, c_p, c_p, c_l, c_p]),
    "tnr_feed_u8_to_tensor": (c_i, [c_p, c_i, c_i, c_i, c_i, c_p, c_i, c_p, c_i, c_f, c_i, c_p]),
    "tnr_tensor2np_u8": (c_i, [c_p, c_i, c_i, c_i, c_i, c_p, c_i, c_i, c_p]),
    "tnr_metrics_workspace_bytes": (c_l, [c_i]),
    "tnr_psnr_ssim_u8": (c_i, [c_p, c_p, c_i, c_i, c_i, c_i, c_i, c_i, c_p, c_p, c_l, c_p]),
    "tnr_lpips_stem_dims": (c_i, [c_i, c_i, c_i, C.POINTER(c_i), C.POINTER(c_i)]),
    "tnr_lpips_stem": (c_i, [c_p, c_p, c_i, c_i, c_i, c_i, c_i, c_i, c_i, c_p, c_p, c_p, c_p, CView, c_p]),
    "tnr_maxpool3s2_ceil_dims": (c_i, [c_i, c_i, C.POINTER(c_i), C.POINTER(c_i)]),
    "tnr_maxpool3s2_ceil_fwd": (c_i, [CView, CView, c_i, c_i, c_i, c_i, c_p]),
    "tnr_lpips_workspace_bytes": (c_l, [c_i, c_i]),
    "tnr_lpips_head": (c_i, [CView, CView, c_i, c_i, c_i, c_i, c_p, c_i, c_i, c_p, c_l, c_p]),
    "tnr_lpips_finalize": (c_i, [c_i, c_i, c_p, c_l, c_p, c_p, c_p]),
    "tnr_bilinear2x_fwd": (c_i, [CView, CView, c_i, c_i, c_i, c_i, c_p]),
    "tnr_bilinear2x_bwd": (c_i, [CView, CView, CView, CView, c_f, c_i, c_i, c_i, c_i, c_p]),
    "tnr_add2": (c_i, [CView, CView, CView, c_l, c_i, c_p]),
    "tnr_mask_copy": (c_i, [CView, CView, CView, c_l, c_i, c_f, c_p]),
    "tnr_axpby": (c_i, [CView, CView, c_l, c_i, c_f, c_f, c_p]),
    "tnr_mask_mul": (c_i, [CView, CView, c_l, c_i, c_f, c_p]),
    "tnr_fill": (c_i, [c_p, c_l, c_f, c_p]),
    "tnr_bn_workspace_bytes": (c_l, [c_i]),
    "tnr_bn_train_fwd": (c_i, [CView, CView, c_l, c_i, c_p, c_p, c_p, c_p, c_p, c_f, c_f, c_p, c_p, c_i, c_f, c_p, c_p]),
    "tnr_bn_train_fwd_stats": (c_i, [CView, CView, c_l, c_i, c_p, c_p, c_p, c_p, c_p, c_f, c_f, c_p, c_p, c_p, c_i, c_f, c_p, c_p]),
    "tnr_bn_replay_running": (c_i, [c_p, c_p, c_p, c_p, c_i, c_f, c_p]),
    "tnr_bn_train_bwd": (c_i, [CView, CView, CView, CView, c_l, c_i, c_p, c_p, c_p, c_f, c_p, c_p, c_f, c_p, c_p]),
    "tnr_bn_train_bwd_z": (c_i, [CView, CView, CView, c_l, c_i, c_p, c_p, c_p, c_p, c_f, c_p, c_p, c_f, c_p, c_p]),
    "tnr_instnorm_workspace_bytes": (c_l, [c_i, c_i]),
    "tnr_instnorm_fwd": (c_i, [CView, CView, c_i, c_l, c_i, c_f, c_p, c_p, c_i, c_f, c_p, c_p]),
    "tnr_instnorm_bwd": (c_i, [CView, CView, CView, CView, c_i, c_l, c_i, c_p, c_p, c_f, c_p, c_p]),
    "tnr_linear_fwd": (c_i, [c_p, c_p, c_p, c_p, c_i, c_i, c_i, c_i, c_f, c_p]),
    "tnr_linear_bwd": (c_i, [c_p, c_p, c_p, c_p, c_f, c_p, c_p, c_p, c_i, c_i, c_i, c_f, c_p, c_p]),
    "tnr_reduce_workspace_bytes": (c_l, []),
    "tnr_l1_mean_fwd": (c_i, [c_p, c_p, c_l, c_f, c_p, c_p, c_p]),
    "tnr_l1_mean_bwd": (c_i, [c_p, c_p, c_l, c_f, c_p, c_p, c_i, c_p]),
    "tnr_ragan_phase_a": (c_i, [c_p, c_p, c_i, c_p, c_p, c_p]),
    "tnr_ragan_phase_b": (c_i, [c_p, c_p, c_i, c_i, c_p, c_p, c_p]),
    "tnr_ragan_phase_c": (c_i, [c_p, c_p, c_i, c_i, c_f, c_p, c_p, c_p, c_p, c_p]),
    "tnr_scale_by": (c_i, [c_p, c_p, c_l, c_p, c_p]),
    "tnr_ssim_workspace_bytes": (c_l, [c_i, c_i, c_i, c_i, c_i, c_i]),
    "tnr_ssim_fwd": (c_i, [c_p, c_p, c_i, c_i, c_i, c_i, c_i, c_i, C.POINTER(c_f), c_i, c_f, c_f, c_p, c_p, c_l, c_p]),
    "tnr_ssim_bwd": (c_i, [c_p, c_p, c_i, c_i, c_i, c_i, c_i, c_i, C.POINTER(c_f), c_i, c_f, c_f, c_p, c_p, c_p, c_i, c_p]),
    "tnr_avgpool2_pad_dims": (c_i, [c_i, c_i, c_i, C.POINTER(c_i), C.POINTER(c_i)]),
    "tnr_avgpool2_pad_fwd": (c_i, [c_p, c_p, c_i, c_i, c_i, c_i, c_i, c_i, c_p, c_p, c_p]),
    "tnr_avgpool2_pad_bwd": (c_i, [c_p, c_p, c_i, c_i, c_i, c_i, c_i, c_i, c_p]),
    "tnr_msssim_combine": (c_i, [c_p, c_i, c_i, C.POINTER(c_l), C.POINTER(c_f), c_i, c_p, c_p, c_p]),
    "tnr_imgloss_workspace_bytes": (c_l, [c_i, c_i, c_i, c_i]),
    "tnr_filter_loss_fwd": (c_i, [c_p, c_p, c_i, c_i, c_i, c_i, c_i, C.POINTER(c_f), c_i, c_i, C.c_double, c_p, c_p, c_p, c_l, c_p]),
    "tnr_filter_loss_bwd": (c_i, [c_p, c_i, c_i, c_i, c_i, c_i, C.POINTER(c_f), c_i, C.c_double, c_p, c_p, c_i, c_p]),
    "tnr_fd_loss_fwd": (c_i, [c_p, c_p, c_i, c_i, c_i, c_i, c_i, c_i, c_i, C.c_double, c_p, c_p, c_l, c_p]),
    "tnr_fd_loss_bwd": (c_i, [c_p, c_p, c_i, c_i, c_i, c_i, c_i, c_i, c_i, C.c_double, c_p, c_p, c_i, c_p]),
    "tnr_pointwise_loss_fwd": (c_i, [c_p, c_p, c_l, c_i, C.c_double, c_p, c_p, c_p]),
    "tnr_pointwise_loss_bwd": (c_i, [c_p, c_p, c_l, c_i, C.c_double, c_p, c_p, c_i, c_p]),
    "tnr_overflow_loss_fwd": (c_i, [c_p, c_l, C.c_double, c_p, c_p, c_p]),
    "tnr_overflow_loss_bwd": (c_i, [c_p, c_l, C.c_double, c_p, c_p, c_i, c_p]),
    "tnr_spl_workspace_bytes": (c_l, [c_i, c_i, c_i, c_i, c_i]),
    "tnr_spl_coef_bytes": (c_l, [c_i, c_i, c_i, c_i, c_i]),
    "tnr_spl_loss_fwd": (c_i, [c_p, c_p, c_i, c_i, c_i, c_i, c_i, c_i, c_i, c_p, c_p, c_p, c_l, c_p]),
    "tnr_spl_loss_bwd": (c_i, [c_p, c_p, c_i, c_i, c_i, c_i, c_i, c_i, c_i, c_p, c_p, c_p, c_i, c_p]),
    "tnr_freqsep_low": (c_i, [c_p, c_i, c_i, c_i, c_i, c_i, C.POINTER(c_f), c_p, c_p, c_i, c_p]),
    "tnr_freqsep_high_fwd": (c_i, [c_p, c_i, c_i, c_i, c_i, c_i, C.POINTER(c_f), c_p, c_p]),
    "tnr_freqsep_high_bwd": (c_i, [c_p, c_p, c_i, c_i, c_i, c_i, c_i, C.POINTER(c_f), c_p, c_p, c_i, c_p]),
    "tnr_diffaug_workspace_bytes": (c_l, [c_i]),
    "tnr_diffaug_mean": (c_i, [c_p, c_i, c_i, c_i, c_i, c_i, c_p, C.POINTER(c_i), c_i, c_p, c_l, c_p]),
    "tnr_diffaug_fwd": (c_i, [c_p, c_i, c_i, c_i, c_i, c_i, c_p, C.POINTER(c_i), c_p, c_p, c_p]),
    "tnr_diffaug_bwd": (c_i, [c_p, c_i, c_i, c_i, c_i, c_i, c_p, C.POINTER(c_i), c_p, c_p, c_p]),
    "tnr_batchaug_mix": (c_i, [c_p, c_p, c_p, c_p, c_i, c_i, c_i, c_i, c_i, C.POINTER(c_i), c_f, c_f, c_p, c_p]),
    "tnr_batchaug_mask": (c_i, [c_p, c_p, c_i, c_i, c_i, c_i, c_i, c_i, c_p, c_p]),
    "tnr_gram_workspace_bytes": (c_l, [c_i, c_i, c_i, c_i]),
    "tnr_gram_fwd": (c_i, [CView, c_i, c_i, c_i, c_i, c_f, c_i, c_p, c_p, c_l, c_p]),
    "tnr_gram_bwd": (c_i, [CView, c_p, c_i, c_i, c_i, c_i, c_f, c_i, CView, c_i, c_p]),
    "tnr_cx_sums_workspace_bytes": (c_l, [c_i, c_i, c_i]),
    "tnr_cx_sums": (c_i, [CView, c_i, c_i, c_i, c_i, c_p, c_i, c_p, c_p, c_l, c_p]),
    "tnr_cx_prepare": (c_i, [CView, c_i, c_i, c_i, c_i, c_p, c_i, c_p, c_p, c_p, c_p]),
    "tnr_cx_matrix_bytes": (c_l, [c_i, c_i]),
    "tnr_cx_distance": (c_i, [c_p, c_p, c_i, c_i, c_i, c_i, c_p, c_p]),
    "tnr_cx_rows": (c_i, [c_p, c_i, c_i, c_f, c_f, c_p, c_p, c_p, c_p, c_p]),
    "tnr_cx_finalize": (c_i, [c_p, c_i, c_i, c_p, c_p, c_p, c_p, c_p, c_p]),
    "tnr_cx_grad_rows": (c_i, [c_p, c_p, c_p, c_i, c_i, c_i, c_f, c_p, c_p, c_p, c_p, c_p, c_p, c_p]),
    "tnr_cx_grad_gemm": (c_i, [c_p, c_p, c_i, c_i, c_i, c_i, c_p, c_p]),
# ... 75 lines not shown
```

### trainner_amd/models/modules/architectures/discriminators.py

```python
import torch
import torch.nn as nn

from .... import ops
from ....engine import ConvOp, HipNet
from ....ops import View, new_act
from . import block as B


class Discriminator_VGG(HipNet):
    def __init__(self, size, in_nc, base_nf, norm_type="batch", act_type="leakyrelu", mode="CNA", convtype="Conv2D",
                 arch="ESRGAN"):
        super().__init__()
        if norm_type != "batch" or mode != "CNA" or convtype != "Conv2D":
            raise NotImplementedError("Discriminator_VGG option outside the ESRGAN recipe is not implemented by the HIP engine")
        if in_nc > 4 or base_nf % 4:
            raise NotImplementedError("HIP Discriminator_VGG needs <= 4 image channels and base_nf %% 4 == 0")
        self.size, self.in_nc = size, in_nc
        self.act, self.slope = B.act_code(act_type)
        blocks = [B.conv_block(in_nc, base_nf, 3, 1, None, act_type), B.conv_block(base_nf, base_nf, 4, 2, "batch", act_type)]
        cur, nc = size // 2, base_nf
        while cur > 4:
            out = nc * 2 if nc < 512 else nc
            blocks.append(B.conv_block(nc, out, 3, 1, "batch", act_type))
            blocks.append(B.conv_block(out, out, 4, 2, "batch", act_type))
            nc, cur = out, cur // 2
        self.features = B.flat_sequential(*blocks)
        self.final_nc, self.final_size = nc, cur
        hidden = 128 if arch == "PPON" else 100
        self.classifier = nn.Sequential(B.LinearHIP(nc * cur * cur, hidden), B.Marker("act:leakyrelu"), B.LinearHIP(hidden, 1))
        self._init_engine()

    def _build_ops(self, packer):
        layers = []
        mods = list(self.features)
        i = 0
        while i < len(mods):
            conv = mods[i]
            bn = mods[i + 1] if isinstance(mods[i + 1], B.BatchNorm2dHIP) else None
            layers.append((ConvOp(conv, packer, need_dgrad=True), bn))
            i += 3 if bn is not None else 2
        self._ops = layers

    def engine_forward(self, x, save):
        N, Cc, S, _ = x.shape
        if S != self.size or x.shape[3] != self.size:
            raise ValueError("Discriminator_VGG built for %dx%d inputs, got %s" % (self.size, self.size, tuple(x.shape)))
        dev, sl, act = x.device, self.slope, self.act
        x4 = View(new_act(N, S, S, 4, dev))
        ops.nchw_to_nhwc(x, x4, Cpad=4)
        cur, acts, bn_stats = x4, [], []
        for conv, bn in self._ops:
            m = conv.mod
            Ho = cur.H // m.stride
            if bn is None:
                y = View(new_act(N, Ho, Ho, m.out_channels, dev))
                conv.fwd(cur, y, act=act, slope=sl)
                acts.append((cur, None, y, None, None))
            else:
                z = View(new_act(N, Ho, Ho, m.out_channels, dev))
                conv.fwd(cur, z)
                y = View(new_act(N, Ho, Ho, m.out_channels, dev))
                mean = torch.empty(m.out_channels, dtype=torch.float32, device=dev)
                invstd = torch.empty(m.out_channels, dtype=torch.float32, device=dev)
                st = torch.empty(2 * m.out_channels, dtype=torch.float64, device=dev) if (save and self.memoize) else None
                ops.bn_train_fwd(z, y, bn.weight, bn.bias, bn.running_mean, bn.running_var, bn.num_batches_tracked,
                                 mean, invstd, momentum=bn.momentum, eps=bn.eps, act=act, slope=sl, stat64=st)
                acts.append((cur, z, y, mean, invstd))
                bn_stats.append((bn, st))
            cur = y
        feat = torch.empty((N, self.final_nc, cur.H, cur.W), dtype=torch.float32, device=dev)
        ops.nhwc_to_nchw(cur, feat)
        l0, l1 = self.classifier[0], self.classifier[2]
        hid = torch.empty((N, l0.out_features), dtype=torch.float32, device=dev)
        ops.linear_fwd(feat.view(N, -1), l0.weight, l0.bias, hid, act=ops.ACT_LRELU, slope=0.2)
        out = torch.empty((N, 1), dtype=torch.float32, device=dev)
        ops.linear_fwd(hid, l1.weight, l1.bias, out)
        saved = dict(acts=acts, feat=feat, hid=hid, last=cur, bn_stats=bn_stats) if save else None
        return out, saved

    def replay_forward_side_effects(self, saved):
        for bn, st in saved["bn_stats"]:
            if st is None:
                raise RuntimeError("memoized forward without recorded BatchNorm statistics")
            ops.bn_replay_running(bn.running_mean, bn.running_var, bn.num_batches_tracked, st, momentum=bn.momentum)

    def engine_backward(self, sv, gout, need_input_grad, need_param_grad):
        W, sl = need_param_grad, self.slope
        gout = gout.contiguous()
        dev = gout.device
        acts, feat, hid, last = sv["acts"], sv["feat"], sv["hid"], sv["last"]
        N = feat.shape[0]
        l0, l1 = self.classifier[0], self.classifier[2]
        ghid = torch.empty_like(hid)
        ops.linear_bwd(hid, l1.weight, gout, None, gx=ghid, dw=l1.weight.grad if W else None,
                       db=l1.bias.grad if W else None)
        gfeat = torch.empty_like(feat)
        ops.linear_bwd(feat.view(N, -1), l0.weight, ghid, hid, gx=gfeat.view(N, -1), dw=l0.weight.grad if W else None,
                       db=l0.bias.grad if W else None, mslope=0.2)
        gy = View(new_act(N, last.H, last.W, last.C, dev))
        ops.nchw_to_nhwc(gfeat, gy, Cpad=last.C)
        sched = getattr(self, "_bucket_schedule", None) if W else None
        if sched is not None:
            sched.mark_done(l0.weight)
        for li in range(len(self._ops) - 1, -1, -1):
            conv, bn = self._ops[li]
            xin, z, y, mean, invstd = acts[li]
            if bn is not None:
                gz = View(new_act(N, y.H, y.W, y.C, dev))
                ops.bn_train_bwd(gy, y, z, gz, bn.weight, mean, invstd, dgamma=bn.weight.grad if W else None,
                                 dbeta=bn.bias.grad if W else None, mslope=sl, beta=bn.bias)
            else:
                gz = gy
            if W:
                conv.wgrad(View(xin.buf, 0, conv.mod.in_channels) if li == 0 else xin, gz)
                if sched is not None:
                    sched.mark_done(conv.mod.weight)
            if li == 0:
                if not need_input_grad:
                    return None
                gx4 = View(new_act(N, xin.H, xin.W, 4, dev))
                conv.dgrad(gz, gx4)
                gx = torch.empty((N, self.in_nc, xin.H, xin.W), dtype=torch.float32, device=dev)
                ops.nhwc_to_nchw(View(gx4.buf, 0, self.in_nc), gx)
                return gx
            prev_bn = self._ops[li - 1][1]
            gprev = View(new_act(N, xin.H, xin.W, xin.C, dev))
            if prev_bn is None:
                conv.dgrad(gz, gprev, mask=xin, m_slope=sl)
            else:
                conv.dgrad(gz, gprev)
            gy = gprev
        return None


class UNetDiscriminator(HipNet):

    def __init__(self, input_nc, nf=64, skip_connection=True, spectral_norm=False):
        super().__init__()
        if spectral_norm:
            raise NotImplementedError("spectral norm in UNetDiscriminator is not implemented by the HIP engine")
        if input_nc > 4 or nf % 4:
            raise NotImplementedError("HIP UNetDiscriminator needs <= 4 image channels and nf %% 4 == 0")
        self.input_nc, self.nf, self.skip_connection = input_nc, nf, bool(skip_connection)
        self.slope = 0.2
        C = B.Conv2dHIP
        self.conv0 = C(input_nc, nf, 3, 1)
        self.conv1 = C(nf, nf * 2, 4, 2, bias=False)
        self.conv2 = C(nf * 2, nf * 4, 4, 2, bias=False)
        self.conv3 = C(nf * 4, nf * 8, 4, 2, bias=False)
        self.conv4 = C(nf * 8, nf * 4, 3, 1, bias=False)
        self.conv5 = C(nf * 4, nf * 2, 3, 1, bias=False)
        self.conv6 = C(nf * 2, nf, 3, 1, bias=False)
        self.conv7 = C(nf, nf, 3, 1, bias=False)
        self.conv8 = C(nf, nf, 3, 1, bias=False)
        self.conv9 = C(nf, 1, 3, 1)
        self._init_engine()

    def _build_ops(self, packer):
        self._ops = [ConvOp(getattr(self, "conv%d" % i), packer, need_dgrad=True) for i in range(10)]

    def engine_forward(self, x, save):
        N, Cc, H, W = x.shape
        if H % 8 or W % 8:
            raise ValueError("UNetDiscriminator needs input sizes divisible by 8, got %s" % (tuple(x.shape),))
        dev, sl, o, nf = x.device, self.slope, self._ops, self.nf
        act = dict(act=ops.ACT_LRELU, slope=sl)
        x4 = View(new_act(N, H, W, 4, dev))
        ops.nchw_to_nhwc(x, x4, Cpad=4)
        x0 = View(new_act(N, H, W, nf, dev))
        o[0].fwd(x4, x0, **act)
        x1 = View(new_act(N, H // 2, W // 2, nf * 2, dev))
        o[1].fwd(x0, x1, **act)
        x2 = View(new_act(N, H // 4, W // 4, nf * 4, dev))
        o[2].fwd(x1, x2, **act)
        x3 = View(new_act(N, H // 8, W // 8, nf * 8, dev))
        o[3].fwd(x2, x3, **act)
        ups, ys, xs = [], [], []
        prev = x3
        for conv, skip in ((o[4], x2), (o[5], x1), (o[6], x0)):
            up = View(new_act(N, prev.H * 2, prev.W * 2, prev.C, dev))
            ops.bilinear2x_fwd(prev, up)
# ... 314 lines not shown
```

### trainner_amd/ops.py

```python
import collections
import ctypes as C

import os

import torch

from . import hip
from .hip import (ACT_LRELU, ACT_NONE, ACT_RELU, CONV_1x1, CONV_3x3, CONV_3x3_C4, CONV_3x3_UP2, CONV_4x4_S2, CONV_7x7_C4, DGRAD_4x4_S2,
                  PACK_C4_DGRAD3, PACK_C4_FWD, PACK_COL_DGRAD3, PACK_COL_FWD, PACK_DENSE_DGRAD, PACK_DGRAD_3x3, PACK_DGRAD_S2, PACK_FWD, PACK_FWD_S2D, CView,
                  ConvDesc,
                  DensePackItem, PackItem, WgradDesc)


def round_up(a, b):
    return (a + b - 1) // b * b


class View:
    __slots__ = ("buf", "coff", "C")

    def __init__(self, buf, coff=0, C=None):
        assert buf.dim() == 4 and buf.dtype == torch.float32 and buf.is_contiguous()
        self.buf, self.coff = buf, coff
        self.C = buf.shape[3] - coff if C is None else C
# ... 315 lines not shown
def conv_plan(x, wp, y, mode=CONV_3x3, epi=None, shuffle=0, layer=None, wino=None, mma=_LIVE, splitk=True, wino_ok=True, stream_ok=True):
    mma = MMA if mma is _LIVE else mma
    epi = epi or {}
    if shuffle:
        no = ((not (SHUFFLE_FOLD and X3_D4 and x.buf.is_cuda) and "switch")
              or (mma not in _STREAM_MMA and "arithmetic")
              or (layer is not None and (layer.k != 3 or layer.stride != 1 or layer.ups or layer.cout != 4 * y.C) and "shape")
              or ((wp.KoutP != 4 * y.C or y.H != 2 * x.H or y.W != 2 * x.W) and "shape")
              or (not stream_ok and "declined"))
        return ("tile", no) if no else ("stream", None)
    why = None
    if layer is not None:
        if layer.k == 3 and layer.stride == 1 and not layer.ups and (layer.cin if layer.dgrad else layer.cout) <= 4 and y.C <= 4:
            why = ((not IMAGE_C4 and "switch")
                   or ((any(epi.get(n) is not None for n in _FUSED) or epi.get("act", ACT_NONE) != ACT_NONE) and "epilogue"))
            if not why:
                return "thin", None
        if layer.c4 is not None and x.ctot == 4 and x.coff == 0:
            if IMAGE_C4:
                return "c4", why
            why = why or "switch"
        if layer.col is not None:
            no = ((not SMALL_GEMM and "switch")
                  or ((y.pixels > 4096 or y.pixels % 8 or x.C % 4) and "shape")
                  or ((any(epi.get(n) is not None for n in _FUSED) or epi.get("reflect")) and "epilogue"))
            if not no:
                return "im2col", why
            why = why or no
    if splitk and wp.KinP >= 512 and y.pixels <= 16384:
        return "tile", "splitk"
    if mode in (CONV_3x3_C4, CONV_7x7_C4):
        return "c4", why
    if mode == CONV_3x3:
        no = ((wino is False and "forbidden")
              or (wino is None and not WINO and "switch")
              or (wino is None and (x.C < WINO_MIN_CIN or y.pixels < WINO_MIN_PIXELS) and "shape")
              or (mma != hip.MMA_BF16X3 and "arithmetic")
              or (y.C % 64 and "shape")
              or (not wino_ok and "declined"))
        if not no:
            return "wino", why or ("forced" if wino else None)
        why = why or no
    if mode in (CONV_3x3, CONV_4x4_S2, DGRAD_4x4_S2):
        no = ((not (X3_D4 and (S2_D4 or mode == CONV_3x3)) and "switch")
              or (mma not in _STREAM_MMA and "arithmetic")
              or (y.C % 64 and "shape")
              or (not stream_ok and "declined"))
        if not no:
            return "stream", why
        why = why or no
    return "tile", why


def _conv_launch(x, wp, y, mode, wino, shuffle, epi, layer=None):
    d, said = None, {}
    while True:
        form, why = conv_plan(x, wp, y, mode, epi, shuffle, layer, wino, **said)
        if shuffle and form != "stream":
            return None
        if d is None:
            lib, d = hip.load(), ConvDesc()
            _conv_desc(d, x, wp, y, mode, **epi)
            if shuffle:
                d.Ho, d.Wo, d.Cout, d.shuffle, d.m_hi = x.H, x.W, 4 * y.C, shuffle, 0
        if why == "splitk":
            need = lib.tnr_conv_workspace_bytes(C.byref(d))
            if need > 0:
                ws = WS.get("splitk@%x" % hip.stream(), need, x.buf.device)
                d.ws, d.ws_bytes = ws.data_ptr(), ws.numel() * 8
                break
            said["splitk"] = False
        elif form == "wino":
            img = _wino_image(lib, d, wp, x.buf.device)
            if img is not None:
                d.wq, d.wq_bytes, d.wq_form = img.data_ptr(), img.numel() * 4, 1
                break
            assert wino is not True, "this launch cannot run in the Winograd form"
            said["wino_ok"] = False
        elif form == "stream":
            img = _wq_image(lib, d, wp, x.buf.device, tag="shuffle2" if shuffle else None)
            if img is not None:
                d.wq, d.wq_bytes = img.data_ptr(), img.numel() * 4
                break
            said["stream_ok"] = False
        else:
            break
    t0 = PROFILE.begin() if PROFILE is not None else None
    hip.check(lib.tnr_conv_forward(C.byref(d), hip.stream()), "conv_forward")
    if PROFILE is not None:
        fam, taps = _CONV_FAMILY[mode]
        PROFILE.end("conv_wino_3x3" if form == "wino" else fam, 2.0 * d.N * d.Ho * d.Wo * taps * min(x.C, wp.KinP) * d.Cout, t0, (x.C, d.Cout, d.Ho, wp.kind))
    return form


def conv_shuffle2(x, wp, y, layer=None, **epi):
    return _conv_launch(x, wp, y, CONV_3x3, None, 2, epi, layer) is not None


def conv(x, wp, y, mode=CONV_3x3, wino=None, **epi):
    _conv_launch(x, wp, y, mode, wino, 0, epi)


CHAIN_MAX = 6
CONV_CHAIN = os.environ.get("TNR_CONV_CHAIN", "1") != "0"
CONV_SWEEP = os.environ.get("TNR_CONV_SWEEP", "1") != "0"
CHAIN_X3 = os.environ.get("TNR_CHAIN_X3", "1") == "1"
AMP_SWEEP = os.environ.get("TNR_AMP_SWEEP", "1") != "0"
SWEEP_DISPENSED = os.environ.get("TNR_SWEEP_WAVES", "4") != "8"
CHAIN_WITH_COLLECTIVES = os.environ.get("TNR_CHAIN_WITH_COLLECTIVES", "0") == "1"
SWEEP_AUTO = os.environ.get("TNR_SWEEP_AUTO", "1") != "0"
SWEEP_AUTO_STATE = {"choice": None, "sweep_us": None, "layers_us": None}
DENSE_SPLIT = os.environ.get("TNR_DENSE_SPLIT", "1") != "0"
_SWEEP_FORM_DMA = os.environ.get("TNR_SWEEP_FORM", "")[:2] == "dm"
COLLECTIVES_IN_FLIGHT = False
COUNTERS = {"one_launch_next_to_collectives": 0, "per_layer_next_to_collectives": 0}
_cu_counts = {}


def _cus(dev):
    if dev not in _cu_counts:
        _cu_counts[dev] = torch.cuda.get_device_properties(dev).multi_processor_count
    return _cu_counts[dev]


def _on_device(buf):
    return buf.is_cuda


def _crowded(in_flight):
    return in_flight and not CHAIN_WITH_COLLECTIVES


def _chain_mma(mma):
    return hip.MMA_F32 if mma == hip.MMA_BF16X3 and not CHAIN_X3 else mma


def _eligible(stages):
    return all(st.get("mode", CONV_3x3) == CONV_3x3 and st["y"].C % 32 == 0 and st["wp"].KoutP == st["y"].C for st in stages)


def _split_shape(stages):
    x0 = stages[0]["x"]
    if not all(st.get("mode", CONV_3x3) == CONV_3x3 and not st.get("reflect") and st["wp"].KoutP == st["y"].C and st["wp"].KinP == st["x"].C for st in stages) \
            or stages[4]["y"].C != 64 or any(st["y"].C != 32 for st in stages[:4]) or x0.C % 16 or x0.C < 32 or stages[4]["x"].C != x0.C + 128:
        return False
    return x0.H >= 8 and x0.W >= 8 and -(-x0.W // 32) * -(-x0.H // 8) <= _cus(x0.buf.device)


def dense_block_plan(stages, crowded=_LIVE, mma=_LIVE, choice=_LIVE, sweepable=True):
    n = 5 if stages is None else len(stages)
    mma = _chain_mma(MMA if mma is _LIVE else mma)
    x3 = mma == hip.MMA_BF16X3
    if not CONV_CHAIN:
# ... 427 lines not shown


def bias_grad(g, db, alpha=1.0, beta=1.0):
    ws = WS.get("bias_grad@%x" % hip.stream(), 512 * g.C * 8, g.buf.device)
    hip.check(hip.load().tnr_bias_grad(g.c(), g.pixels, g.C, db.data_ptr(), alpha, beta, ws.data_ptr(), ws.numel() * 8, hip.stream()), "bias_grad")


def pad2d(x, y, pad, reflect):
    hip.check(hip.load().tnr_pad2d(x.c(), y.c(), x.N, x.H, x.W, x.C, pad, int(reflect), hip.stream()), "pad2d")


def unpad2d(xp, y, pad, fold):
    hip.check(hip.load().tnr_unpad2d(xp.c(), y.c(), y.N, y.H, y.W, y.C, pad, int(fold), hip.stream()), "unpad2d")


def window2d(src, dst, oy, ox, acc=False):
    hip.check(hip.load().tnr_window2d(src.c(), src.H, src.W, dst.c(), dst.N, dst.H, dst.W, dst.C, oy, ox, int(acc), hip.stream()), "window2d")


def tanh_fwd(x, y):
    hip.check(hip.load().tnr_tanh_fwd(x.data_ptr(), y.data_ptr(), x.numel(), hip.stream()), "tanh_fwd")


def tanh_bwd(g, y, gx):
    hip.check(hip.load().tnr_tanh_bwd(g.data_ptr(), y.data_ptr(), gx.data_ptr(), g.numel(), hip.stream()), "tanh_bwd")


def gan_loss(pred, kind, target, out, grad=None):
    hip.check(hip.load().tnr_gan_loss(pred.data_ptr(), pred.numel(), kind, float(target), out.data_ptr(), hip.ptr(grad), hip.stream()), "gan_loss")


def axpby(dst, src, a=1.0, b=1.0):
    hip.check(hip.load().tnr_axpby(dst.c(), src.c(), dst.pixels, dst.C, a, b, hip.stream()), "axpby")


def mask_mul(g, y, mslope=0.2):
    hip.check(hip.load().tnr_mask_mul(g.c(), y.c(), g.pixels, g.C, mslope, hip.stream()), "mask_mul")


def fill(t, value=0.0):
    hip.check(hip.load().tnr_fill(t.data_ptr(), t.numel(), value, hip.stream()), "fill")


def bn_train_fwd(z, y, gamma, beta, running_mean, running_var, num_batches, save_mean, save_invstd,
                 momentum=0.1, eps=1e-5, act=ACT_LRELU, slope=0.2, stat64=None):
    lib = hip.load()
    ws = WS.get("bn", lib.tnr_bn_workspace_bytes(z.C), z.buf.device)
    hip.check(lib.tnr_bn_train_fwd_stats(z.c(), y.c(), z.pixels, z.C, gamma.data_ptr(), beta.data_ptr(),
                                         hip.ptr(running_mean), hip.ptr(running_var), hip.ptr(num_batches), momentum, eps,
                                         save_mean.data_ptr(), save_invstd.data_ptr(), hip.ptr(stat64), act, slope, ws.data_ptr(),
                                         hip.stream()), "bn_train_fwd")


def bn_replay_running(running_mean, running_var, num_batches, stat64, momentum=0.1):
    hip.check(hip.load().tnr_bn_replay_running(running_mean.data_ptr(), running_var.data_ptr(), hip.ptr(num_batches), stat64.data_ptr(),
                                               running_mean.numel(), momentum, hip.stream()), "bn_replay_running")


BN_MASK_FROM_Z = os.environ.get("TNR_BN_MASK_FROM_Z", "1") != "0"


def bn_train_bwd(gy, y, z, gz, gamma, save_mean, save_invstd, dgamma=None, dbeta=None, acc_beta=1.0, mslope=0.2, beta=None):
    lib = hip.load()
    ws = WS.get("bn", lib.tnr_bn_workspace_bytes(z.C), z.buf.device)
    if beta is not None and BN_MASK_FROM_Z:
        hip.check(lib.tnr_bn_train_bwd_z(gy.c(), z.c(), gz.c(), z.pixels, z.C, gamma.data_ptr(), beta.data_ptr(), save_mean.data_ptr(),
                                         save_invstd.data_ptr(), mslope, hip.ptr(dgamma), hip.ptr(dbeta), acc_beta, ws.data_ptr(),
                                         hip.stream()), "bn_train_bwd_z")
        return
    hip.check(lib.tnr_bn_train_bwd(gy.c(), y.c(), z.c(), gz.c(), z.pixels, z.C, gamma.data_ptr(),
                                   save_mean.data_ptr(), save_invstd.data_ptr(), mslope, hip.ptr(dgamma),
                                   hip.ptr(dbeta), acc_beta, ws.data_ptr(), hip.stream()), "bn_train_bwd")


def instnorm_fwd(z, y, save_mean, save_invstd, eps=1e-5, act=ACT_NONE, slope=0.0):
    lib = hip.load()
    ws = WS.get("instnorm", lib.tnr_instnorm_workspace_bytes(z.N, z.C), z.buf.device)
    hip.check(lib.tnr_instnorm_fwd(z.c(), y.c(), z.N, z.H * z.W, z.C, eps, save_mean.data_ptr(), save_invstd.data_ptr(), act, slope,
                                   ws.data_ptr(), hip.stream()), "instnorm_fwd")


def instnorm_bwd(gy, y, z, gz, save_mean, save_invstd, mslope=1.0):
    lib = hip.load()
    ws = WS.get("instnorm", lib.tnr_instnorm_workspace_bytes(z.N, z.C), z.buf.device)
    hip.check(lib.tnr_instnorm_bwd(gy.c(), y.c(), z.c(), gz.c(), z.N, z.H * z.W, z.C, save_mean.data_ptr(), save_invstd.data_ptr(),
                                   mslope, ws.data_ptr(), hip.stream()), "instnorm_bwd")


def linear_fwd(x, w, b, y, act=ACT_NONE, slope=0.2):
    N, In = x.shape
    Out = w.shape[0]
    hip.check(hip.load().tnr_linear_fwd(x.data_ptr(), w.data_ptr(), hip.ptr(b), y.data_ptr(), N, In, Out, act, slope,
                                        hip.stream()), "linear_fwd")


def linear_bwd(x, w, gy, yact=None, gx=None, dw=None, db=None, acc_beta=1.0, mslope=0.2):
    N, In = x.shape
    Out = w.shape[0]
    gpre = WS.get("lin", N * Out * 4, x.device)
    hip.check(hip.load().tnr_linear_bwd(x.data_ptr(), w.data_ptr(), gy.data_ptr(), hip.ptr(yact), mslope, hip.ptr(gx),
                                        hip.ptr(dw), hip.ptr(db), N, In, Out, acc_beta, gpre.data_ptr(), hip.stream()),
              "linear_bwd")


def _reduce_ws(dev):
    return WS.get("reduce@%x" % hip.stream(), hip.load().tnr_reduce_workspace_bytes(), dev)


def _floats(seq, n=None):
    return (C.c_float * (len(seq) if n is None else n))(*seq)


def l1_mean_fwd(a, b, scale, out):
    hip.check(hip.load().tnr_l1_mean_fwd(a.data_ptr(), b.data_ptr(), a.numel(), scale, out.data_ptr(),
                                         _reduce_ws(a.device).data_ptr(), hip.stream()), "l1_mean_fwd")


def l1_mean_bwd(a, b, scale, gscale, ga, accumulate=False):
    hip.check(hip.load().tnr_l1_mean_bwd(a.data_ptr(), b.data_ptr(), a.numel(), scale, hip.ptr(gscale), ga.data_ptr(),
                                         int(accumulate), hip.stream()), "l1_mean_bwd")


def ssim_fwd(x, y, layout, shave, taps, C1, C2, sums):
    lib = hip.load()
    N, Ch, H, W = x.shape
# ... 283 lines not shown
```

Baseline: 74.50.

## Fuse BatchNorm statistics reduction into discriminator conv epilogues

Adds a statistics hook to the conv epilogue. In forward mode it accumulates per-channel sum and sum-of-squares. In backward mode it accumulates the BN gradient reductions (sum of masked gy and gy times centered z) and writes per-tile double partials. New BN forward and backward entry points consume these partials instead of re-reading the activation tensor to reduce it, which removes a full pass over z per BN layer in the VGG-style discriminator. In exchange the epilogue does extra register-heavy double accumulation, DPP shuffles and an LDS reduction, which may lower occupancy or slow the conv kernels.

```diff
diff --git a/include/trainner_hip.h b/include/trainner_hip.h
--- a/include/trainner_hip.h
+++ b/include/trainner_hip.h
@@ -112,6 +112,18 @@
 int tnr_pack_dense_dims(int32_t nf, int32_t gc, int32_t t, int32_t *KoutP, int32_t *KinP, int64_t *n_out);
 int tnr_pack_dense_dgrad(const tnr_dense_pack_item *items_dev, int32_t n, int64_t max_out, void *stream);
 int tnr_conv_forward(const tnr_conv_desc *d, void *stream);
+#define TNR_STATS_FWD 1
+#define TNR_STATS_BWD 2
+typedef struct tnr_conv_stats {
+    int32_t mode;
+    int32_t slots;
+    double *partial;
+    tnr_view z;
+    const float *mean, *invstd, *gamma, *beta;
+    float slope;
+} tnr_conv_stats;
+int32_t tnr_conv_stats_slots(const tnr_conv_desc *d, int32_t mode);
+int tnr_conv_forward_stats(const tnr_conv_desc *d, const tnr_conv_stats *st, void *stream);
 int tnr_gauss_mult(tnr_view dst, tnr_view src, int64_t pixels, int32_t C, float sigma, uint32_t key0, uint32_t key1, uint32_t pix0,
                    void *stream);
 int64_t tnr_conv_workspace_bytes(const tnr_conv_desc *d);
@@ -237,6 +249,12 @@
 int tnr_bn_train_bwd_z(tnr_view gy, tnr_view z, tnr_view gz, int64_t pixels, int32_t C, const float *gamma, const float *beta,
                        const float *save_mean, const float *save_invstd, float mslope, float *dgamma, float *dbeta,
                        float acc_beta, void *ws, void *stream);
+int tnr_bn_train_fwd_partials(const double *partial, int32_t slots, tnr_view z, tnr_view y, int64_t pixels, int32_t C, const float *gamma,
+                              const float *beta, float *running_mean, float *running_var, int64_t *num_batches, float momentum, float eps,
+                              float *save_mean, float *save_invstd, double *stat64, int32_t act, float slope, void *ws, void *stream);
+int tnr_bn_train_bwd_z_partials(const double *partial, int32_t slots, tnr_view gy, tnr_view z, tnr_view gz, int64_t pixels, int32_t C,
+                                const float *gamma, const float *beta, const float *save_mean, const float *save_invstd, float mslope,
+                                float *dgamma, float *dbeta, float acc_beta, void *ws, void *stream);
 int64_t tnr_instnorm_workspace_bytes(int32_t N, int32_t C);
 int tnr_instnorm_fwd(tnr_view z, tnr_view y, int32_t N, int64_t pixels_per_image, int32_t C, float eps, float *save_mean,
                      float *save_invstd, int32_t act, float slope, void *ws, void *stream);
diff --git a/trainner_amd/csrc/conv_epilogue.h b/trainner_amd/csrc/conv_epilogue.h
--- a/trainner_amd/csrc/conv_epilogue.h
+++ b/trainner_amd/csrc/conv_epilogue.h
@@ -3,10 +3,20 @@
 
 namespace {
 
-template <int MODE, int TW, int NT, int MT, bool COH, int DEPTH = 1, bool NOISE = true, int BIAS_STEP = 1, class PixFn>
+struct ConvStatK {
+    double *partial;
+    const float *z; int z_ct, z_co;
+    const float *mean, *invstd, *gamma, *beta;
+    float slope;
+};
+inline ConvStatK conv_stat_k(const tnr_conv_stats &s) {
+    return ConvStatK{s.partial, s.z.ptr, s.z.ctot, s.z.coff, s.mean, s.invstd, s.gamma, s.beta, s.slope};
+}
+template <int MODE, int TW, int NT, int MT, bool COH, int DEPTH = 1, bool NOISE = true, int BIAS_STEP = 1, int STAT = 0, class PixFn>
 __device__ __forceinline__ void conv_epilogue_dpp_map(const ConvK a, f32x16 (&acc)[MT][NT], const int cb, const int n, const int ty0,
                                                       const int tx0, const int par, const int li, const int half,
-                                                      const __amdgpu_buffer_rsrc_t y_rs, PixFn &&pixfn) {
+                                                      const __amdgpu_buffer_rsrc_t y_rs, PixFn &&pixfn, double (*st)[4][2] = nullptr,
+                                                      const ConvStatK *sk = nullptr) {
     constexpr bool DG2 = (MODE == TNR_DGRAD_4x4_S2);
     constexpr int NC = NT * 32;
     const int py = par >> 1, px = par & 1;
@@ -70,11 +80,23 @@
         b1f[nn] = use_r1[nn] ? a.beta1 : 0.f;
         msf[nn] = use_m[nn] ? a.m_slope : 1.f;
     }
+    constexpr int SNT = STAT == 2 ? NT : 1;
+    f32x4 s_mu[SNT], s_is[SNT], s_ga[SNT], s_be[SNT];
+    if constexpr (STAT == 2) {
+#pragma unroll
+        for (int nn = 0; nn < NT; ++nn) {
+            const int co = co_ok[nn] ? co_n[nn] : 0;
+            s_mu[nn] = *reinterpret_cast<const f32x4 *>(sk->mean + co);
+            s_is[nn] = *reinterpret_cast<const f32x4 *>(sk->invstd + co);
+            s_ga[nn] = *reinterpret_cast<const f32x4 *>(sk->gamma + co);
+            s_be[nn] = *reinterpret_cast<const f32x4 *>(sk->beta + co);
+        }
+    }
     constexpr int UNITS = MT * 4;
     constexpr int AHEAD = DEPTH < UNITS ? DEPTH : UNITS, SETS = AHEAD + 1 < UNITS ? AHEAD + 1 : UNITS;
     bool ok[SETS];
     size_t pixi[SETS];
-    f32x4 q1[SETS][NT], q2[SETS][NT], qm[SETS][NT];
+    f32x4 q1[SETS][NT], q2[SETS][NT], qm[SETS][NT], qz[SETS][SNT];
     auto prep = [&](int u, int set) {
         const int mi = u >> 2, q = u & 3;
         int rr, cc;
@@ -101,6 +123,10 @@
                 qm[set][nn] = one;
                 if (okc && use_m[nn]) qm[set][nn] = *reinterpret_cast<const f32x4 *>(a.m + pix * a.m_ct + a.m_co + co_n[nn]);
             }
+            if constexpr (STAT == 2) {
+                qz[set][nn] = zero;
+                if (okc) qz[set][nn] = *reinterpret_cast<const f32x4 *>(sk->z + pix * sk->z_ct + sk->z_co + co_n[nn]);
+            }
         }
     };
     auto finish = [&](int u, int set) {
@@ -128,6 +154,22 @@
             }
             if (!(ok[set] && co_ok[nn])) continue;
             const int co = co_n[nn];
+            if constexpr (STAT == 1) {
+#pragma unroll
+                for (int e = 0; e < 4; ++e) {
+                    st[nn][e][0] += (double)v[e];
+                    st[nn][e][1] += (double)v[e] * (double)v[e];
+                }
+            } else if constexpr (STAT == 2) {
+#pragma unroll
+                for (int e = 0; e < 4; ++e) {
+                    const float zc = qz[set][nn][e] - s_mu[nn][e];
+                    const float yv = ((qz[set][nn][e] - s_mu[nn][e]) * s_is[nn][e]) * s_ga[nn][e] + s_be[nn][e];
+                    const float gm = v[e] * (yv > 0.f ? 1.f : sk->slope);
+                    st[nn][e][0] += (double)gm;
+                    st[nn][e][1] += (double)gm * (double)zc;
+                }
+            }
 #ifdef TNR_ABL_NOEPISTORE
             if (v[0] == 1.2345e30f) a.y[0] = v[1] + v[2] + v[3];
             continue;
@@ -156,16 +198,47 @@
     }
 }
 
-template <int MODE, int TW, int NT, int MT, bool COH, int DEPTH = 1, bool NOISE = true, int BIAS_STEP = 1>
+template <int MODE, int TW, int NT, int MT, bool COH, int DEPTH = 1, bool NOISE = true, int BIAS_STEP = 1, int STAT = 0>
 __device__ __forceinline__ void conv_epilogue_dpp(const ConvK a, f32x16 (&acc)[MT][NT], const int cb, const int n, const int ty0,
                                                   const int tx0, const int par, const int wave, const int li, const int half,
-                                                  const __amdgpu_buffer_rsrc_t y_rs) {
-    conv_epilogue_dpp_map<MODE, TW, NT, MT, COH, DEPTH, NOISE, BIAS_STEP>(a, acc, cb, n, ty0, tx0, par, li, half, y_rs,
+                                                  const __amdgpu_buffer_rsrc_t y_rs, double (*st)[4][2] = nullptr,
+                                                  const ConvStatK *sk = nullptr) {
+    conv_epilogue_dpp_map<MODE, TW, NT, MT, COH, DEPTH, NOISE, BIAS_STEP, STAT>(a, acc, cb, n, ty0, tx0, par, li, half, y_rs,
                                                                 [&](int mi, int row, int &rr, int &cc) __attribute__((always_inline)) {
                                                                     const int p = (wave * MT + mi) * 32 + row;
                                                                     rr = p / TW;
                                                                     cc = p - rr * TW;
-                                                                });
-}
-
-}
+                                                                }, st, sk);
+}
+
+constexpr int CONV_STATS_WAVE_DOUBLES(int NT) { return 2 * NT * 8 * 4 * 2; }
+template <int CTRL>
+__device__ __forceinline__ double conv_stats_dpp(const double x) {
+    const unsigned long long b = __builtin_bit_cast(unsigned long long, x);
+    const unsigned lo = (unsigned)__builtin_amdgcn_mov_dpp((int)(unsigned)b, CTRL, 0xF, 0xF, true);
+    const unsigned hi = (unsigned)__builtin_amdgcn_mov_dpp((int)(unsigned)(b >> 32), CTRL, 0xF, 0xF, true);
+    return __builtin_bit_cast(double, ((unsigned long long)hi << 32) | lo);
+}
+template <int NT>
+__device__ __forceinline__ void conv_stats_to_lds(double (&st)[NT][4][2], double *sh, const int wave, const int li, const int half) {
+    double *row = sh + ((size_t)(wave * 2 + half) * NT * 8 + (li >> 2)) * 8;
+#pragma unroll
+    for (int nn = 0; nn < NT; ++nn)
+#pragma unroll
+        for (int e = 0; e < 4; ++e)
+#pragma unroll
+            for (int k = 0; k < 2; ++k) {
+                double s = st[nn][e][k];
+                s += conv_stats_dpp<0xB1>(s);
+                s += conv_stats_dpp<0x4E>(s);
+                if ((li & 3) == 0) row[nn * 64 + e * 2 + k] = s;
+            }
+}
+template <int NT>
+__device__ __forceinline__ void conv_stats_add(const double *sh, const int wave, const int half, const int ch, double &s0, double &s1) {
+    const double *p = sh + ((size_t)((wave * 2 + half) * NT + (ch >> 5)) * 8 + ((ch & 31) >> 2)) * 8 + (ch & 3) * 2;
+    s0 += p[0];
+    s1 += p[1];
+}
+
+}
diff --git a/trainner_amd/csrc/conv_sweep.hip b/trainner_amd/csrc/conv_sweep.hip
--- a/trainner_amd/csrc/conv_sweep.hip
+++ b/trainner_amd/csrc/conv_sweep.hip
@@ -1088,6 +1088,7 @@
     int wq_bytes;
     int nck;
     int tiles_x, tiles_y, ncb, tiles;
+    ConvStatK st;
 };
 struct S2PackK {
     const float *wp;
@@ -1159,8 +1160,9 @@
     });
 }
 
-template <int MODE, bool AMP>
+template <int MODE, bool AMP, int STAT = 0>
 __global__ void __launch_bounds__(256, 2) conv_s2_d4_kernel(const S2K c) {
+    static_assert(STAT == 0 || (STAT == 1 && MODE == TNR_CONV_4x4_S2 && !AMP), "the statistics hook exists for the fp32 forward layer only");
     constexpr bool DG = MODE == TNR_DGRAD_4x4_S2;
     constexpr int HT = DG ? SW_HT : SW_TH + 1, WT = DG ? SW_WT : SW_TW + 1, ROWS = HT * WT;
     constexpr int A_IT = (ROWS * 4 + 255) / 256;
@@ -1300,7 +1302,24 @@
             t2[m][0] = acc[m][0];
             t2[m][1] = acc[m][1];
         }
-        conv_epilogue_dpp<MODE, SW_TW, 2, 2, false, 1>(a, t2, cb, n, ty0, tx0, par, wave, li, half, y_rs);
+        double st[2][4][2] = {{{0.0, 0.0}, {0.0, 0.0}, {0.0, 0.0}, {0.0, 0.0}}, {{0.0, 0.0}, {0.0, 0.0}, {0.0, 0.0}, {0.0, 0.0}}};
+        conv_epilogue_dpp<MODE, SW_TW, 2, 2, false, 1, true, 1, STAT>(a, t2, cb, n, ty0, tx0, par, wave, li, half, y_rs, st, &c.st);
+        if constexpr (STAT != 0) {
+            double *sh = reinterpret_cast<double *>(s_a + (nchunks & 1) * SW_A_FLOATS);
+            static_assert(4 * CONV_STATS_WAVE_DOUBLES(2) * sizeof(double) <= SW_A_FLOATS * sizeof(float), "statistics rows fit an input buffer");
+            conv_stats_to_lds<2>(st, sh, wave, li, half);
+            __syncthreads();
+            if (tid < 64) {
+                double s0 = 0.0, s1 = 0.0;
+#pragma unroll
+                for (int w = 0; w < 4; ++w)
+#pragma unroll
+                    for (int hh = 0; hh < 2; ++hh) conv_stats_add<2>(sh, w, hh, tid, s0, s1);
+                double *dst = c.st.partial + ((size_t)((n * c.tiles_y + ty) * c.tiles_x + tx) * a.Cout + cb * 64 + tid) * 2;
+                dst[0] = s0;
+                dst[1] = s1;
+            }
+        }
     }
 }
 
@@ -1523,17 +1542,32 @@
     return tnr_check_launch("conv_wq_pack");
 }
 
-int tnr_launch_conv_s2_d4(const tnr_conv_desc *d, void *stream) {
+int tnr_conv_s2_d4_stats_slots(const tnr_conv_desc *d, int mode) {
+    if (!s2_ok(d) || d->wq == nullptr || d->wq_bytes < tnr_conv_wq_bytes(d) || d->noise_pos != 0 || d->mma != TNR_MMA_BF16X3) return 0;
+    if (d->mode != TNR_CONV_4x4_S2 || mode != TNR_STATS_FWD) return 0;
+    const int64_t slots = (int64_t)d->N * tnr_cdiv(d->Ho, SW_TH) * tnr_cdiv(d->Wo, SW_TW);
+    return slots < (1LL << 31) / d->Cout ? (int)slots : 0;
+}
+
+int tnr_launch_conv_s2_d4(const tnr_conv_desc *d, void *stream, const tnr_conv_stats *st) {
     if (!s2_ok(d) || d->wq == nullptr || d->wq_bytes < tnr_conv_wq_bytes(d) || d->noise_pos != 0) return 1;
     static int cus = 0;
     if (const int rc = tnr_kernel_setup(&cus, "conv_s2_d4", {{conv_s2_d4_kernel<TNR_CONV_4x4_S2, false>, S4D_LDS_BYTES}, {conv_s2_d4_kernel<TNR_CONV_4x4_S2, true>, S4D_LDS_BYTES},
-                                                             {conv_s2_d4_kernel<TNR_DGRAD_4x4_S2, false>, S4D_LDS_BYTES}, {conv_s2_d4_kernel<TNR_DGRAD_4x4_S2, true>, S4D_LDS_BYTES}}))
+                                                             {conv_s2_d4_kernel<TNR_DGRAD_4x4_S2, false>, S4D_LDS_BYTES}, {conv_s2_d4_kernel<TNR_DGRAD_4x4_S2, true>, S4D_LDS_BYTES},
+                                                             {conv_s2_d4_kernel<TNR_CONV_4x4_S2, false, 1>, S4D_LDS_BYTES}}))
         return rc;
     const bool dg = d->mode == TNR_DGRAD_4x4_S2;
     S2K c;
     if (!stream_k_from_desc(c, *d, tnr_conv_wq_bytes(d), SW_TW, SW_TH, dg ? 4 : 1)) return 1;
     const unsigned grid = (unsigned)(c.tiles < 2 * cus ? c.tiles : 2 * cus);
     const bool amp = d->mma == TNR_MMA_BF16;
+    c.st = ConvStatK{};
+    if (st != nullptr) {
+        if (tnr_conv_s2_d4_stats_slots(d, st->mode) <= 0) return 1;
+        c.st = conv_stat_k(*st);
+        hipLaunchKernelGGL((conv_s2_d4_kernel<TNR_CONV_4x4_S2, false, 1>), dim3(grid), dim3(256), S4D_LDS_BYTES, (hipStream_t)stream, c);
+        return tnr_check_launch("conv_s2_d4 (statistics)");
+    }
     if (dg) {
         if (amp) hipLaunchKernelGGL((conv_s2_d4_kernel<TNR_DGRAD_4x4_S2, true>), dim3(grid), dim3(256), S4D_LDS_BYTES, (hipStream_t)stream, c);
         else hipLaunchKernelGGL((conv_s2_d4_kernel<TNR_DGRAD_4x4_S2, false>), dim3(grid), dim3(256), S4D_LDS_BYTES, (hipStream_t)stream, c);
diff --git a/trainner_amd/csrc/conv_tile.hip b/trainner_amd/csrc/conv_tile.hip
--- a/trainner_amd/csrc/conv_tile.hip
+++ b/trainner_amd/csrc/conv_tile.hip
@@ -140,10 +140,44 @@
 }
 
 int tnr_launch_conv3x3_d4(const tnr_conv_desc *d, void *stream);
-int tnr_launch_conv3x3_wino(const tnr_conv_desc *d, void *stream);
-int tnr_launch_conv_s2_d4(const tnr_conv_desc *d, void *stream);
-
-extern "C" int tnr_conv_forward(const tnr_conv_desc *d, void *stream) {
+int tnr_launch_conv3x3_wino(const tnr_conv_desc *d, void *stream, const tnr_conv_stats *st);
+int tnr_launch_conv_s2_d4(const tnr_conv_desc *d, void *stream, const tnr_conv_stats *st);
+int tnr_conv3x3_wino_stats_slots(const tnr_conv_desc *d, int mode);
+int tnr_conv_s2_d4_stats_slots(const tnr_conv_desc *d, int mode);
+
+namespace {
+bool conv_x3_d4_on() {
+    static const bool d4 = [] { const char *e = std::getenv("TNR_X3_D4"); return e == nullptr || e[0] != '0'; }();
+    return d4;
+}
+int conv_forward_impl(const tnr_conv_desc *d, const tnr_conv_stats *st, void *stream);
+}
+
+extern "C" int tnr_conv_forward(const tnr_conv_desc *d, void *stream) { return conv_forward_impl(d, nullptr, stream); }
+
+extern "C" int32_t tnr_conv_stats_slots(const tnr_conv_desc *d, int32_t mode) {
+    if (d == nullptr || d->wq == nullptr || (mode != TNR_STATS_FWD && mode != TNR_STATS_BWD)) return 0;
+    if (d->ws != nullptr && conv_ksplit(d, conv_tile_geom(d).tiles) > 1) return 0;
+    if (d->wq_form == 1) return tnr_conv3x3_wino_stats_slots(d, mode);
+    if (!(conv_x3_d4_on() || d->shuffle != 0) || (d->mode != TNR_CONV_4x4_S2 && d->mode != TNR_DGRAD_4x4_S2)) return 0;
+    return tnr_conv_s2_d4_stats_slots(d, mode);
+}
+
+extern "C" int tnr_conv_forward_stats(const tnr_conv_desc *d, const tnr_conv_stats *st, void *stream) {
+    TNR_REQUIRE(d != nullptr && st != nullptr && st->partial != nullptr, "conv_forward_stats: null pointer");
+    const int32_t need = tnr_conv_stats_slots(d, st->mode);
+    TNR_REQUIRE(need > 0, "conv_forward_stats: the form this descriptor launches has no statistics hook (tnr_conv_stats_slots() == 0)");
+    TNR_REQUIRE(st->slots >= need, "conv_forward_stats: partial holds %d slots, the launch writes %d", st->slots, need);
+    if (st->mode == TNR_STATS_BWD) {
+        TNR_REQUIRE(st->z.ptr && st->mean && st->invstd && st->gamma && st->beta, "conv_forward_stats: TNR_STATS_BWD needs z, mean, invstd, gamma, beta");
+        TNR_REQUIRE((st->z.ctot % 4) == 0 && (st->z.coff % 4) == 0 && (int64_t)d->N * d->Ho * d->Wo * st->z.ctot < (1LL << 31),
+                    "conv_forward_stats: z view must be 4-channel aligned and below 2^31 elements");
+    }
+    return conv_forward_impl(d, st, stream);
+}
+
+namespace {
+int conv_forward_impl(const tnr_conv_desc *d, const tnr_conv_stats *st, void *stream) {
     TNR_REQUIRE(d != nullptr && d->x.ptr && d->y.ptr && d->wp, "conv: null pointer");
     TNR_REQUIRE(d->mode >= TNR_CONV_3x3 && d->mode <= TNR_CONV_7x7_C4, "conv: bad mode %d", d->mode);
     if (d->mode == TNR_CONV_3x3_C4)
@@ -204,17 +238,17 @@
     int rc;
     if (d->wq != nullptr && d->wq_form == 1) {
         TNR_REQUIRE(k.ksplit == 1, "conv: a Winograd weight stream cannot be combined with a split-K workspace");
-        rc = tnr_launch_conv3x3_wino(d, (void *)s);
+        rc = tnr_launch_conv3x3_wino(d, (void *)s, st);
         TNR_REQUIRE(rc != 1, "conv: wq_form = 1 but the launch does not qualify for the Winograd kernel (tnr_conv_wino_bytes() == 0)");
         return rc;
     }
     if (d->wq != nullptr && k.ksplit == 1) {
-        static const bool d4 = [] { const char *e = std::getenv("TNR_X3_D4"); return e == nullptr || e[0] != '0'; }();
-        if (d4 || d->shuffle != 0) {
-            rc = (d->mode == TNR_CONV_4x4_S2 || d->mode == TNR_DGRAD_4x4_S2) ? tnr_launch_conv_s2_d4(d, (void *)s) : tnr_launch_conv3x3_d4(d, (void *)s);
+        if (conv_x3_d4_on() || d->shuffle != 0) {
+            rc = (d->mode == TNR_CONV_4x4_S2 || d->mode == TNR_DGRAD_4x4_S2) ? tnr_launch_conv_s2_d4(d, (void *)s, st) : tnr_launch_conv3x3_d4(d, (void *)s);
             if (rc <= 0) return rc;
         }
     }
+    TNR_REQUIRE(st == nullptr, "conv: the statistics hook exists in the Winograd and four-tap weight-stream kernels only");
     TNR_REQUIRE(d->shuffle == 0, "conv: a pixel-shuffle store (shuffle = %d) exists in the weight-stream kernel only (tnr_conv_wq_bytes() == 0 for this launch)", d->shuffle);
     {
         static const bool w8 = [] { const char *e = std::getenv("TNR_X3_W8"); return e == nullptr || e[0] != '0'; }();
@@ -251,6 +285,7 @@
     hipLaunchKernelGGL(conv_splitk_reduce_kernel, dim3((unsigned)blocks), dim3(256), 0, s, red);
     return tnr_check_launch("conv_splitk_reduce");
 }
+}
 
 extern "C" int64_t tnr_conv_workspace_bytes(const tnr_conv_desc *d) {
     if (d == nullptr) return 0;
diff --git a/trainner_amd/csrc/conv_wino.hip b/trainner_amd/csrc/conv_wino.hip
--- a/trainner_amd/csrc/conv_wino.hip
+++ b/trainner_amd/csrc/conv_wino.hip
@@ -43,6 +43,7 @@
     int wq_bytes;
     int nck;
     int tiles_x, tiles_y, ncb, tiles;
+    ConvStatK st;
 };
 
 struct WinoPackK {
@@ -90,6 +91,7 @@
     wn_static_for_seq<B>(f, std::make_integer_sequence<int, (E > B ? E - B : 0)>{});
 }
 
+template <int STAT>
 __global__ void __launch_bounds__(512, 2) conv3x3_wino_kernel(const WinoK c) {
     extern __shared__ __attribute__((aligned(16))) float smem[];
     float *s_v = smem;
@@ -396,12 +398,30 @@
                 }
             }
         }
-        conv_epilogue_dpp_map<TNR_CONV_3x3, WN_T, 1, 2, false, 1>(a, keep, cb * 2 + wn, n, ty0, tx0, 0, li, half, y_rs,
+        double st[1][4][2] = {{{0.0, 0.0}, {0.0, 0.0}, {0.0, 0.0}, {0.0, 0.0}}};
+        conv_epilogue_dpp_map<TNR_CONV_3x3, WN_T, 1, 2, false, 1, true, 1, STAT>(a, keep, cb * 2 + wn, n, ty0, tx0, 0, li, half, y_rs,
                                                                   [&](int mi, int row, int &rr, int &cc) __attribute__((always_inline)) {
                                                                       const int p = 32 * wh + row;
                                                                       rr = 2 * (p >> 3) + wil;
                                                                       cc = 2 * (p & 7) + mi;
-                                                                  });
+                                                                  }, st, &c.st);
+        if constexpr (STAT != 0) {
+            double *sh = reinterpret_cast<double *>(smem + 8 * (4 * 16 * 64));
+            static_assert(8 * (4 * 16 * 64) * sizeof(float) + 8 * CONV_STATS_WAVE_DOUBLES(1) * sizeof(double) <= WN_LDS_BYTES, "statistics rows fit behind the exchange");
+            conv_stats_to_lds<1>(st, sh, wave, li, half);
+            __syncthreads();
+            if (tid < 64) {
+                const int nt = tid >> 5;
+                double s0 = 0.0, s1 = 0.0;
+#pragma unroll
+                for (int k = 0; k < 4; ++k)
+#pragma unroll
+                    for (int hh = 0; hh < 2; ++hh) conv_stats_add<1>(sh, (k >> 1) * 4 + nt * 2 + (k & 1), hh, tid & 31, s0, s1);
+                double *dst = c.st.partial + ((size_t)((n * c.tiles_y + ty) * c.tiles_x + tx) * a.Cout + cb * 64 + tid) * 2;
+                dst[0] = s0;
+                dst[1] = s1;
+            }
+        }
         }
     }
 #ifdef WN_TIMELINE
@@ -665,18 +685,37 @@
     return tnr_check_launch("conv_wino_pack");
 }
 
-int tnr_launch_conv3x3_wino(const tnr_conv_desc *d, void *stream) {
+static bool wino_w16() {
+    static const bool w16 = [] { const char *e = getenv("TNR_WINO_WAVES"); return e != nullptr && atoi(e) == 16; }();
+    return w16;
+}
+
+int tnr_conv3x3_wino_stats_slots(const tnr_conv_desc *d, int mode) {
+    if (!wino_ok(d) || d->wq == nullptr || d->wq_bytes < tnr_conv_wino_bytes(d) || d->noise_pos < 0 || d->noise_pos > 2 || wino_w16()) return 0;
+    const int64_t slots = (int64_t)d->N * tnr_cdiv(d->Ho, WN_T) * tnr_cdiv(d->Wo, WN_T);
+    return slots < (1LL << 31) / d->Cout ? (int)slots : 0;
+}
+
+int tnr_launch_conv3x3_wino(const tnr_conv_desc *d, void *stream, const tnr_conv_stats *st) {
     if (!wino_ok(d) || d->wq == nullptr || d->wq_bytes < tnr_conv_wino_bytes(d) || d->noise_pos < 0 || d->noise_pos > 2) return 1;
     static int cus = 0;
-    if (const int rc = tnr_kernel_setup(&cus, "conv3x3_wino", {{conv3x3_wino_kernel, WN_LDS_BYTES}, {conv3x3_wino16_kernel, WN_LDS_BYTES}})) return rc;
+    if (const int rc = tnr_kernel_setup(&cus, "conv3x3_wino", {{conv3x3_wino_kernel<0>, WN_LDS_BYTES}, {conv3x3_wino_kernel<1>, WN_LDS_BYTES},
+                                                               {conv3x3_wino_kernel<2>, WN_LDS_BYTES}, {conv3x3_wino16_kernel, WN_LDS_BYTES}})) return rc;
     WinoK c;
     if (!stream_k_from_desc(c, *d, tnr_conv_wino_bytes(d), WN_T, WN_T, 1)) return 1;
     const int grid = c.tiles < cus ? c.tiles : cus;
-    static const bool w16 = [] { const char *e = getenv("TNR_WINO_WAVES"); return e != nullptr && atoi(e) == 16; }();
-    if (w16) {
+    c.st = ConvStatK{};
+    if (st != nullptr) {
+        if (tnr_conv3x3_wino_stats_slots(d, st->mode) <= 0) return 1;
+        c.st = conv_stat_k(*st);
+        if (st->mode == TNR_STATS_FWD) hipLaunchKernelGGL(conv3x3_wino_kernel<1>, dim3((unsigned)grid), dim3(512), WN_LDS_BYTES, (hipStream_t)stream, c);
+        else hipLaunchKernelGGL(conv3x3_wino_kernel<2>, dim3((unsigned)grid), dim3(512), WN_LDS_BYTES, (hipStream_t)stream, c);
+        return tnr_check_launch("conv3x3_wino (statistics)");
+    }
+    if (wino_w16()) {
         hipLaunchKernelGGL(conv3x3_wino16_kernel, dim3((unsigned)grid), dim3(1024), WN_LDS_BYTES, (hipStream_t)stream, c);
         return tnr_check_launch("conv3x3_wino16");
     }
-    hipLaunchKernelGGL(conv3x3_wino_kernel, dim3((unsigned)grid), dim3(512), WN_LDS_BYTES, (hipStream_t)stream, c);
+    hipLaunchKernelGGL(conv3x3_wino_kernel<0>, dim3((unsigned)grid), dim3(512), WN_LDS_BYTES, (hipStream_t)stream, c);
     return tnr_check_launch("conv3x3_wino");
 }
diff --git a/trainner_amd/csrc/norm_loss_optim.hip b/trainner_amd/csrc/norm_loss_optim.hip
--- a/trainner_amd/csrc/norm_loss_optim.hip
+++ b/trainner_amd/csrc/norm_loss_optim.hip
@@ -657,6 +657,65 @@
     return tnr_check_launch("bn_train_bwd_z");
 }
 
+namespace {
+__global__ void __launch_bounds__(256) bn_fold_slots_kernel(const double *in, int slots, int per, int row, double *out, int nslab) {
+    const int64_t g = (int64_t)blockIdx.x * 256 + threadIdx.x;
+    if (g >= (int64_t)nslab * row) return;
+    const int b = (int)(g / row), j = (int)(g - (int64_t)b * row);
+    int q1 = (b + 1) * per;
+    if (q1 > slots) q1 = slots;
+    double s = 0;
+    for (int q = b * per; q < q1; ++q) s += in[(size_t)q * row + j];
+    out[g] = s;
+}
+
+inline const double *bn_fold_slots(const double *partial, int slots, int C, double *ws, int &nslab, hipStream_t s) {
+    nslab = slots;
+    if (slots <= RED_BLOCKS) return partial;
+    const int per = tnr_cdiv(slots, RED_BLOCKS);
+    nslab = tnr_cdiv(slots, per);
+    hipLaunchKernelGGL(bn_fold_slots_kernel, dim3((unsigned)tnr_cdiv64((int64_t)nslab * C * 2, 256)), dim3(256), 0, s, partial, slots, per,
+                       C * 2, ws, nslab);
+    return ws;
+}
+}
+
+extern "C" int tnr_bn_train_fwd_partials(const double *partial, int32_t slots, tnr_view z, tnr_view y, int64_t pixels, int32_t C,
+                                         const float *gamma, const float *beta, float *running_mean, float *running_var,
+                                         int64_t *num_batches, float momentum, float eps, float *save_mean, float *save_invstd,
+                                         double *stat64, int32_t act, float slope, void *ws, void *stream) {
+    TNR_REQUIRE(partial && slots > 0 && z.ptr && y.ptr && gamma && beta && save_mean && save_invstd && ws, "bn_fwd_partials: null pointer");
+    TNR_REQUIRE((C % 4) == 0 && C / 4 <= 256, "bn_fwd_partials: unsupported C %d", C);
+    hipStream_t s = (hipStream_t)stream;
+    int nslab;
+    const double *slabs = bn_fold_slots(partial, slots, C, (double *)ws, nslab, s);
+    hipLaunchKernelGGL(bn_fwd_finalize_kernel, dim3(tnr_cdiv(C, 32)), dim3(256), 0, s, slabs, nslab, C, pixels,
+                       running_mean, running_var, num_batches, momentum, eps, save_mean, save_invstd, stat64);
+    hipLaunchKernelGGL(bn_fwd_apply_kernel, dim3(grid_for(pixels * (C / 4))), dim3(256), 0, s, z.ptr, z.ctot, z.coff, y.ptr,
+                       y.ctot, y.coff, pixels, C, gamma, beta, save_mean, save_invstd, act, slope);
+    return tnr_check_launch("bn_train_fwd_partials");
+}
+
+extern "C" int tnr_bn_train_bwd_z_partials(const double *partial, int32_t slots, tnr_view gy, tnr_view z, tnr_view gz, int64_t pixels,
+                                           int32_t C, const float *gamma, const float *beta, const float *save_mean,
+                                           const float *save_invstd, float mslope, float *dgamma, float *dbeta, float acc_beta, void *ws,
+                                           void *stream) {
+    TNR_REQUIRE(partial && slots > 0 && gy.ptr && z.ptr && gz.ptr && gamma && beta && save_mean && save_invstd && ws,
+                "bn_bwd_z_partials: null pointer");
+    TNR_REQUIRE((C % 4) == 0 && C / 4 <= 256, "bn_bwd_z_partials: unsupported C %d", C);
+    TNR_REQUIRE((dgamma == nullptr) == (dbeta == nullptr), "bn_bwd_z_partials: dgamma and dbeta go together");
+    hipStream_t s = (hipStream_t)stream;
+    double *sums = (double *)ws + (size_t)RED_BLOCKS * C * 2;
+    int nslab;
+    const double *slabs = bn_fold_slots(partial, slots, C, (double *)ws, nslab, s);
+    hipLaunchKernelGGL(bn_bwd_finalize_kernel, dim3(tnr_cdiv(C, 32)), dim3(256), 0, s, slabs, nslab, C, save_invstd, sums,
+                       dgamma, dbeta, acc_beta);
+    hipLaunchKernelGGL(bn_bwd_apply_kernel<true>, dim3(grid_for(pixels * (C / 4))), dim3(256), 0, s, gy.ptr, gy.ctot, gy.coff,
+                       (const float *)nullptr, 0, 0, z.ptr, z.ctot, z.coff, gz.ptr, gz.ctot, gz.coff, pixels, C, gamma, save_mean,
+                       save_invstd, sums, mslope, beta);
+    return tnr_check_launch("bn_train_bwd_z_partials");
+}
+
 extern "C" int64_t tnr_instnorm_workspace_bytes(int32_t N, int32_t C) {
     return (int64_t)N * ((int64_t)RED_BLOCKS * C * 2 + 2 * (int64_t)C) * (int64_t)sizeof(double);
 }
diff --git a/trainner_amd/engine.py b/trainner_amd/engine.py
--- a/trainner_amd/engine.py
+++ b/trainner_amd/engine.py
@@ -31,7 +31,7 @@
         self.dirs = {False: (self.mode_f, ops.ConvLayer(k, s, cin, cout, False, ups, direct=self.i_f, c4=i_f4, col=i_fc)),
                      True: (self.mode_d, ops.ConvLayer(k, s, cin, cout, True, ups, direct=self.i_d, c4=i_d4, col=i_dc))}
 
-    def _run(self, dgrad, x, y, epi):
+    def _run(self, dgrad, x, y, epi, stats=None):
         mode, layer = self.dirs[dgrad]
         wp = self.packer.get(layer.direct)
         form = ops.conv_plan(x, wp, y, mode, epi, layer=layer)[0]
@@ -41,18 +41,20 @@
             ops.conv(x if x.C == 4 else ops.View(x.buf), self.packer.get(layer.c4), y, mode=ops.CONV_3x3_C4, **epi)
         elif form == "im2col":
             ops.conv_small(x, self.packer.get(layer.col), y, layer.k, layer.stride, **epi)
+        elif stats is not None:
+            ops.conv_stats(x, wp, y, stats, mode=mode, **epi)
         else:
             ops.conv(x, wp, y, mode=mode, **epi)
 
-    def fwd(self, x, y, **epi):
+    def fwd(self, x, y, stats=None, **epi):
         epi["bias"] = self.mod.bias
-        self._run(False, x, y, epi)
+        self._run(False, x, y, epi, stats)
 
     def fwd_shuffle2(self, x, y, **epi):
         return ops.conv_shuffle2(x, self.packer.get(self.i_f), y, layer=self.dirs[False][1], bias=self.mod.bias, **epi)
 
-    def dgrad(self, g, gx, **epi):
-        self._run(True, g, gx, epi)
+    def dgrad(self, g, gx, stats=None, **epi):
+        self._run(True, g, gx, epi, stats)
 
     def fwd_stage(self, x, y, fresh_from=None, **epi):
         return dict(x=x, wp=self.packer.get(self.i_f), y=y, mode=self.mode_f, bias=self.mod.bias, fresh_from=fresh_from, **epi)
diff --git a/trainner_amd/hip.py b/trainner_amd/hip.py
--- a/trainner_amd/hip.py
+++ b/trainner_amd/hip.py
@@ -37,6 +37,14 @@
     ]
 
 
+STATS_FWD, STATS_BWD = 1, 2
+
+
+class ConvStats(C.Structure):
+    _fields_ = [("mode", c_i), ("slots", c_i), ("partial", c_p), ("z", CView),
+                ("mean", c_p), ("invstd", c_p), ("gamma", c_p), ("beta", c_p), ("slope", c_f)]
+
+
 class WgradDesc(C.Structure):
     _fields_ = [
         ("x", CView), ("N", c_i), ("H", c_i), ("W", c_i), ("Cin", c_i),
@@ -71,6 +79,8 @@
     "tnr_pack_dense_dims": (c_i, [c_i, c_i, c_i, C.POINTER(c_i), C.POINTER(c_i), C.POINTER(c_l)]),
     "tnr_pack_dense_dgrad": (c_i, [c_p, c_i, c_l, c_p]),
     "tnr_conv_forward": (c_i, [C.POINTER(ConvDesc), c_p]),
+    "tnr_conv_stats_slots": (c_i, [C.POINTER(ConvDesc), c_i]),
+    "tnr_conv_forward_stats": (c_i, [C.POINTER(ConvDesc), C.POINTER(ConvStats), c_p]),
     "tnr_conv_workspace_bytes": (c_l, [C.POINTER(ConvDesc)]),
     "tnr_conv_wq_bytes": (c_l, [C.POINTER(ConvDesc)]),
     "tnr_conv_wq_pack": (c_i, [C.POINTER(ConvDesc), c_p, c_l, c_p]),
@@ -153,6 +163,8 @@
     "tnr_bn_replay_running": (c_i, [c_p, c_p, c_p, c_p, c_i, c_f, c_p]),
     "tnr_bn_train_bwd": (c_i, [CView, CView, CView, CView, c_l, c_i, c_p, c_p, c_p, c_f, c_p, c_p, c_f, c_p, c_p]),
     "tnr_bn_train_bwd_z": (c_i, [CView, CView, CView, c_l, c_i, c_p, c_p, c_p, c_p, c_f, c_p, c_p, c_f, c_p, c_p]),
+    "tnr_bn_train_fwd_partials": (c_i, [c_p, c_i, CView, CView, c_l, c_i, c_p, c_p, c_p, c_p, c_p, c_f, c_f, c_p, c_p, c_p, c_i, c_f, c_p, c_p]),
+    "tnr_bn_train_bwd_z_partials": (c_i, [c_p, c_i, CView, CView, CView, c_l, c_i, c_p, c_p, c_p, c_p, c_f, c_p, c_p, c_f, c_p, c_p]),
     "tnr_instnorm_workspace_bytes": (c_l, [c_i, c_i]),
     "tnr_instnorm_fwd": (c_i, [CView, CView, c_i, c_l, c_i, c_f, c_p, c_p, c_i, c_f, c_p, c_p]),
     "tnr_instnorm_bwd": (c_i, [CView, CView, CView, CView, c_i, c_l, c_i, c_p, c_p, c_f, c_p, c_p]),
diff --git a/trainner_amd/models/modules/architectures/discriminators.py b/trainner_amd/models/modules/architectures/discriminators.py
--- a/trainner_amd/models/modules/architectures/discriminators.py
+++ b/trainner_amd/models/modules/architectures/discriminators.py
@@ -58,13 +58,21 @@
                 acts.append((cur, None, y, None, None))
             else:
                 z = View(new_act(N, Ho, Ho, m.out_channels, dev))
-                conv.fwd(cur, z)
+                hook = ops.BnStats(ops.STATS_FWD) if (ops.BN_FUSED and ops.BN_FUSED_FWD and z.buf.is_cuda) else None
+                if hook is None:
+                    conv.fwd(cur, z)
+                else:
+                    conv.fwd(cur, z, stats=hook)
                 y = View(new_act(N, Ho, Ho, m.out_channels, dev))
                 mean = torch.empty(m.out_channels, dtype=torch.float32, device=dev)
                 invstd = torch.empty(m.out_channels, dtype=torch.float32, device=dev)
                 st = torch.empty(2 * m.out_channels, dtype=torch.float64, device=dev) if (save and self.memoize) else None
-                ops.bn_train_fwd(z, y, bn.weight, bn.bias, bn.running_mean, bn.running_var, bn.num_batches_tracked,
-                                 mean, invstd, momentum=bn.momentum, eps=bn.eps, act=act, slope=sl, stat64=st)
+                if hook is not None and hook.partial is not None:
+                    ops.bn_train_fwd_partials(hook, z, y, bn.weight, bn.bias, bn.running_mean, bn.running_var, bn.num_batches_tracked,
+                                              mean, invstd, momentum=bn.momentum, eps=bn.eps, act=act, slope=sl, stat64=st)
+                else:
+                    ops.bn_train_fwd(z, y, bn.weight, bn.bias, bn.running_mean, bn.running_var, bn.num_batches_tracked,
+                                     mean, invstd, momentum=bn.momentum, eps=bn.eps, act=act, slope=sl, stat64=st)
                 acts.append((cur, z, y, mean, invstd))
                 bn_stats.append((bn, st))
             cur = y
@@ -102,13 +110,18 @@
         sched = getattr(self, "_bucket_schedule", None) if W else None
         if sched is not None:
             sched.mark_done(l0.weight)
+        hook = None
         for li in range(len(self._ops) - 1, -1, -1):
             conv, bn = self._ops[li]
             xin, z, y, mean, invstd = acts[li]
             if bn is not None:
                 gz = View(new_act(N, y.H, y.W, y.C, dev))
-                ops.bn_train_bwd(gy, y, z, gz, bn.weight, mean, invstd, dgamma=bn.weight.grad if W else None,
-                                 dbeta=bn.bias.grad if W else None, mslope=sl, beta=bn.bias)
+                if hook is not None and hook.partial is not None:
+                    ops.bn_train_bwd_partials(hook, gy, z, gz, bn.weight, bn.bias, mean, invstd, dgamma=bn.weight.grad if W else None,
+                                              dbeta=bn.bias.grad if W else None, mslope=sl)
+                else:
+                    ops.bn_train_bwd(gy, y, z, gz, bn.weight, mean, invstd, dgamma=bn.weight.grad if W else None,
+                                     dbeta=bn.bias.grad if W else None, mslope=sl, beta=bn.bias)
             else:
                 gz = gy
             if W:
@@ -125,8 +138,13 @@
                 return gx
             prev_bn = self._ops[li - 1][1]
             gprev = View(new_act(N, xin.H, xin.W, xin.C, dev))
+            hook = None
             if prev_bn is None:
                 conv.dgrad(gz, gprev, mask=xin, m_slope=sl)
+            elif ops.BN_FUSED and ops.BN_FUSED_BWD and ops.BN_MASK_FROM_Z and gz.buf.is_cuda:
+                pz, pmean, pinv = acts[li - 1][1], acts[li - 1][3], acts[li - 1][4]
+                hook = ops.BnStats(ops.STATS_BWD, z=pz, mean=pmean, invstd=pinv, gamma=prev_bn.weight, beta=prev_bn.bias, slope=sl)
+                conv.dgrad(gz, gprev, stats=hook)
             else:
                 conv.dgrad(gz, gprev)
             gy = gprev
diff --git a/trainner_amd/ops.py b/trainner_amd/ops.py
--- a/trainner_amd/ops.py
+++ b/trainner_amd/ops.py
@@ -391,7 +391,21 @@
     return "tile", why
 
 
-def _conv_launch(x, wp, y, mode, wino, shuffle, epi, layer=None):
+_BN_FUSED = os.environ.get("TNR_BN_FUSED", "1").lower()
+BN_FUSED = _BN_FUSED != "0"
+BN_FUSED_FWD, BN_FUSED_BWD = _BN_FUSED != "bwd", _BN_FUSED != "fwd"
+STATS_FWD, STATS_BWD = hip.STATS_FWD, hip.STATS_BWD
+
+
+class BnStats:
+    __slots__ = ("mode", "z", "mean", "invstd", "gamma", "beta", "slope", "partial", "slots")
+
+    def __init__(self, mode, z=None, mean=None, invstd=None, gamma=None, beta=None, slope=0.2):
+        self.mode, self.z, self.mean, self.invstd, self.gamma, self.beta, self.slope = mode, z, mean, invstd, gamma, beta, slope
+        self.partial, self.slots = None, 0
+
+
+def _conv_launch(x, wp, y, mode, wino, shuffle, epi, layer=None, stats=None):
     d, said = None, {}
     while True:
         form, why = conv_plan(x, wp, y, mode, epi, shuffle, layer, wino, **said)
@@ -424,8 +438,19 @@
             said["stream_ok"] = False
         else:
             break
+    cs = None
+    if stats is not None and BN_FUSED and x.buf.is_cuda:
+        slots = lib.tnr_conv_stats_slots(C.byref(d), stats.mode)
+        if slots > 0:
+            part = WS.get("bn_slots@%x" % hip.stream(), slots * y.C * 16, x.buf.device)
+            cs = hip.ConvStats(stats.mode, slots, part.data_ptr(), cv(stats.z), hip.ptr(stats.mean), hip.ptr(stats.invstd), hip.ptr(stats.gamma),
+                               hip.ptr(stats.beta), stats.slope)
+            stats.partial, stats.slots = part, slots
     t0 = PROFILE.begin() if PROFILE is not None else None
-    hip.check(lib.tnr_conv_forward(C.byref(d), hip.stream()), "conv_forward")
+    if cs is not None:
+        hip.check(lib.tnr_conv_forward_stats(C.byref(d), C.byref(cs), hip.stream()), "conv_forward_stats")
+    else:
+        hip.check(lib.tnr_conv_forward(C.byref(d), hip.stream()), "conv_forward")
     if PROFILE is not None:
         fam, taps = _CONV_FAMILY[mode]
         PROFILE.end("conv_wino_3x3" if form == "wino" else fam, 2.0 * d.N * d.Ho * d.Wo * taps * min(x.C, wp.KinP) * d.Cout, t0, (x.C, d.Cout, d.Ho, wp.kind))
@@ -438,6 +463,10 @@
 
 def conv(x, wp, y, mode=CONV_3x3, wino=None, **epi):
     _conv_launch(x, wp, y, mode, wino, 0, epi)
+
+
+def conv_stats(x, wp, y, stats, mode=CONV_3x3, wino=None, **epi):
+    _conv_launch(x, wp, y, mode, wino, 0, epi, stats=stats)
 
 
 CHAIN_MAX = 6
@@ -971,6 +1000,16 @@
                                          hip.stream()), "bn_train_fwd")
 
 
+def bn_train_fwd_partials(stats, z, y, gamma, beta, running_mean, running_var, num_batches, save_mean, save_invstd,
+                          momentum=0.1, eps=1e-5, act=ACT_LRELU, slope=0.2, stat64=None):
+    lib = hip.load()
+    ws = WS.get("bn", lib.tnr_bn_workspace_bytes(z.C), z.buf.device)
+    hip.check(lib.tnr_bn_train_fwd_partials(stats.partial.data_ptr(), stats.slots, z.c(), y.c(), z.pixels, z.C, gamma.data_ptr(), beta.data_ptr(),
+                                            hip.ptr(running_mean), hip.ptr(running_var), hip.ptr(num_batches), momentum, eps,
+                                            save_mean.data_ptr(), save_invstd.data_ptr(), hip.ptr(stat64), act, slope, ws.data_ptr(),
+                                            hip.stream()), "bn_train_fwd_partials")
+
+
 def bn_replay_running(running_mean, running_var, num_batches, stat64, momentum=0.1):
     hip.check(hip.load().tnr_bn_replay_running(running_mean.data_ptr(), running_var.data_ptr(), hip.ptr(num_batches), stat64.data_ptr(),
                                                running_mean.numel(), momentum, hip.stream()), "bn_replay_running")
@@ -990,6 +1029,14 @@
     hip.check(lib.tnr_bn_train_bwd(gy.c(), y.c(), z.c(), gz.c(), z.pixels, z.C, gamma.data_ptr(),
                                    save_mean.data_ptr(), save_invstd.data_ptr(), mslope, hip.ptr(dgamma),
                                    hip.ptr(dbeta), acc_beta, ws.data_ptr(), hip.stream()), "bn_train_bwd")
+
+
+def bn_train_bwd_partials(stats, gy, z, gz, gamma, beta, save_mean, save_invstd, dgamma=None, dbeta=None, acc_beta=1.0, mslope=0.2):
+    lib = hip.load()
+    ws = WS.get("bn", lib.tnr_bn_workspace_bytes(z.C), z.buf.device)
+    hip.check(lib.tnr_bn_train_bwd_z_partials(stats.partial.data_ptr(), stats.slots, gy.c(), z.c(), gz.c(), z.pixels, z.C, gamma.data_ptr(),
+                                              beta.data_ptr(), save_mean.data_ptr(), save_invstd.data_ptr(), mslope, hip.ptr(dgamma),
+                                              hip.ptr(dbeta), acc_beta, ws.data_ptr(), hip.stream()), "bn_train_bwd_z_partials")
 
 
 def instnorm_fwd(z, y, save_mean, save_invstd, eps=1e-5, act=ACT_NONE, slope=0.0):
```

Result: no change. 75.00, median of 5 (+0.7%).
